# zhing2006/hala-renderer

Measured on AMD Instinct MI355X. Metric: Mrays/s, higher is better.
Workload: dtype f32

## Files before the change

### hala-renderer_amd/_abi.py

```python
import ctypes as C

INVALID_INDEX = 0xFFFFFFFF
MAX_CAMERA_COUNT = 8
MAX_LIGHT_COUNT = 32


class Vertex(C.Structure):
    _fields_ = [("position", C.c_float * 3), ("normal", C.c_float * 3),
                ("tangent", C.c_float * 3), ("tex_coord", C.c_float * 2)]


class GpuCamera(C.Structure):
    _fields_ = [("position", C.c_float * 3), ("_pad0", C.c_float),
                ("right", C.c_float * 3), ("_pad1", C.c_float),
                ("up", C.c_float * 3), ("_pad2", C.c_float),
                ("forward", C.c_float * 3), ("yfov", C.c_float),
                ("focal_distance_or_xmag", C.c_float), ("aperture_or_ymag", C.c_float),
                ("type", C.c_uint32), ("_pad3", C.c_uint32)]


class GpuLight(C.Structure):
    _fields_ = [("intensity", C.c_float * 3), ("_pad0", C.c_float),
                ("position", C.c_float * 3), ("_pad1", C.c_float),
                ("u", C.c_float * 3), ("_pad2", C.c_float),
# ... 51 lines not shown
class MeshDesc(C.Structure):
    _fields_ = [("primitives", C.POINTER(PrimitiveDesc)), ("primitive_count", C.c_uint32)]


class MaterialDesc(C.Structure):
    _fields_ = [("type", C.c_uint32), ("base_color", C.c_float * 3), ("opacity", C.c_float),
                ("emission", C.c_float * 3), ("anisotropic", C.c_float), ("metallic", C.c_float),
                ("roughness", C.c_float), ("subsurface", C.c_float), ("specular_tint", C.c_float),
                ("sheen", C.c_float), ("sheen_tint", C.c_float), ("clearcoat", C.c_float),
                ("clearcoat_roughness", C.c_float), ("clearcoat_tint", C.c_float * 3),
                ("specular_transmission", C.c_float), ("ior", C.c_float),
                ("medium_type", C.c_uint32), ("medium_color", C.c_float * 3),
                ("medium_density", C.c_float), ("medium_anisotropy", C.c_float),
                ("base_color_map_index", C.c_uint32), ("emission_map_index", C.c_uint32),
                ("normal_map_index", C.c_uint32), ("metallic_roughness_map_index", C.c_uint32)]


class LightDesc(C.Structure):
    _fields_ = [("color", C.c_float * 3), ("intensity", C.c_float), ("light_type", C.c_uint32),
                ("param0", C.c_float), ("param1", C.c_float)]


class CameraDesc(C.Structure):
    _fields_ = [("type", C.c_uint32), ("aspect", C.c_float), ("yfov", C.c_float), ("znear", C.c_float),
                ("zfar", C.c_float), ("focal_distance", C.c_float), ("aperture", C.c_float),
                ("xmag", C.c_float), ("ymag", C.c_float)]


class ImageDesc(C.Structure):
    _fields_ = [("format", C.c_uint32), ("width", C.c_uint32), ("height", C.c_uint32),
                ("data", C.c_void_p), ("num_of_bytes", C.c_size_t)]


class IndexPair(C.Structure):
    _fields_ = [("key", C.c_uint32), ("value", C.c_uint32)]


class SceneDesc(C.Structure):
    _fields_ = [("nodes", C.POINTER(NodeDesc)), ("node_count", C.c_uint32),
                ("meshes", C.POINTER(MeshDesc)), ("mesh_count", C.c_uint32),
                ("materials", C.POINTER(MaterialDesc)), ("material_count", C.c_uint32),
                ("lights", C.POINTER(LightDesc)), ("light_count", C.c_uint32),
                ("cameras", C.POINTER(CameraDesc)), ("camera_count", C.c_uint32),
                ("texture2image_mapping", C.POINTER(IndexPair)), ("texture_count", C.c_uint32),
                ("image2data_mapping", C.POINTER(IndexPair)), ("image_count", C.c_uint32),
                ("image_data", C.POINTER(ImageDesc)), ("image_data_count", C.c_uint32)]


class Ray(C.Structure):
    _fields_ = [("origin", C.c_float * 3), ("tmin", C.c_float), ("direction", C.c_float * 3), ("tmax", C.c_float)]


class Hit(C.Structure):
    _fields_ = [("t", C.c_float), ("u", C.c_float), ("v", C.c_float), ("prim", C.c_uint32)]


class RtInfo(C.Structure):
    _fields_ = [("width", C.c_uint32), ("height", C.c_uint32)]


class RtStatistics(C.Structure):
    _fields_ = [("total_frames", C.c_uint64), ("last_gpu_ms", C.c_double), ("rays_last_update", C.c_uint64),
                ("rays_total", C.c_uint64), ("traverse_ms_last_update", C.c_double),
                ("gpu_ms_total", C.c_double), ("traverse_closest_ms_total", C.c_double),
                ("traverse_shadow_ms_total", C.c_double), ("traverse_closest_launches", C.c_uint64),
                ("traverse_shadow_launches", C.c_uint64), ("updates_rendered", C.c_uint64),
                ("rays_closest_total", C.c_uint64), ("rays_shadow_total", C.c_uint64),
                ("nodes_closest_total", C.c_uint64), ("tris_closest_total", C.c_uint64),
                ("nodes_shadow_total", C.c_uint64), ("tris_shadow_total", C.c_uint64),
                ("rays_closest_counted", C.c_uint64), ("rays_shadow_counted", C.c_uint64),
                ("wave_steps_closest_total", C.c_uint64), ("leaf_passes_closest_total", C.c_uint64), ("leaf_lanes_closest_total", C.c_uint64),
                ("wave_steps_shadow_total", C.c_uint64), ("leaf_passes_shadow_total", C.c_uint64), ("leaf_lanes_shadow_total", C.c_uint64),
                ("traverse_primary_ms_total", C.c_double), ("traverse_primary_launches", C.c_uint64),
                ("nodes_primary_total", C.c_uint64), ("tris_primary_total", C.c_uint64), ("rays_primary_counted", C.c_uint64),
                ("rays_primary_total", C.c_uint64),
                ("rays_closest_timed", C.c_uint64), ("rays_primary_timed", C.c_uint64), ("rays_shadow_timed", C.c_uint64),
                ("shade_ms_total", C.c_double), ("shade_launches", C.c_uint64),
                ("traverse_fused_ms_total", C.c_double), ("traverse_fused_launches", C.c_uint64),
                ("rays_fused_closest_timed", C.c_uint64), ("rays_fused_shadow_timed", C.c_uint64)]


class BuildOptions(C.Structure):
    _fields_ = [("builder", C.c_uint32), ("ploc_tail", C.c_uint32), ("ploc_look_every", C.c_uint32),
                ("collapse_look_every", C.c_uint32), ("instancing", C.c_uint32), ("reserved", C.c_uint32 * 3)]


class BvhInfo(C.Structure):
    _fields_ = [("node_count", C.c_uint32), ("triangle_count", C.c_uint32), ("max_depth", C.c_uint32),
                ("lds_node_count", C.c_uint32), ("scene_min", C.c_float * 3), ("scene_max", C.c_float * 3),
                ("node_width", C.c_uint32), ("stored_triangle_count", C.c_uint32), ("instance_node_count", C.c_uint32),
                ("instance_ref_count", C.c_uint32), ("tree_bytes", C.c_uint64)]


class RtProgDescInfo(C.Structure):
    _fields_ = [("raygen_count", C.c_uint32), ("miss_count", C.c_uint32), ("hit_count", C.c_uint32),
                ("callable_count", C.c_uint32), ("push_constant_size", C.c_uint32),
                ("binding_count", C.c_uint32), ("ray_recursion_depth", C.c_uint32)]


class DenoiseParams(C.Structure):
    _fields_ = [("iterations", C.c_uint32), ("sigma_color", C.c_float), ("sigma_albedo", C.c_float),
                ("normal_power", C.c_uint32), ("demodulate", C.c_uint32), ("reserved", C.c_uint32 * 3)]


class AdaptiveParams(C.Structure):
    _fields_ = [("threshold", C.c_float), ("min_samples", C.c_uint32), ("interval", C.c_uint32), ("reserved", C.c_uint32 * 5)]


class AdaptiveStatus(C.Structure):
    _fields_ = [("enabled", C.c_uint32), ("active_blocks", C.c_uint32), ("total_blocks", C.c_uint32), ("active_pixels", C.c_uint32),
                ("samples", C.c_uint32), ("last_snapshot", C.c_uint32), ("reserved", C.c_uint32 * 2)]


class LightGroups(C.Structure):
    _fields_ = [("group_count", C.c_uint32), ("environment_group", C.c_uint32), ("light_count", C.c_uint32),
                ("material_count", C.c_uint32), ("light_group", C.POINTER(C.c_uint32)), ("material_group", C.POINTER(C.c_uint32))]


class CryptomatteDesc(C.Structure):
    _fields_ = [("layer_mask", C.c_uint32), ("material_name_count", C.c_uint32), ("material_names", C.POINTER(C.c_char_p)),
                ("reserved", C.c_uint32 * 2)]


class TemporalParams(C.Structure):
    _fields_ = [("max_history", C.c_float), ("tol", C.c_float), ("min_weight", C.c_float), ("reserved", C.c_uint32 * 5)]


PROTOTYPES = {
    "hala_denoise_default_params": ([C.POINTER(DenoiseParams)], None),
    "hala_rt_denoise": ([C.c_void_p, C.POINTER(DenoiseParams), C.POINTER(C.c_float)], C.c_int),
    "hala_rt_read_denoised": ([C.c_void_p, C.POINTER(C.c_float)], C.c_int),
    "hala_rt_get_denoised_buffer": ([C.c_void_p, C.POINTER(C.c_void_p), C.POINTER(C.c_size_t)], C.c_int),
    "hala_rt_save_denoised": ([C.c_void_p, C.c_char_p], C.c_int),
    "hala_denoise_images": ([C.c_int, C.POINTER(C.c_float), C.POINTER(C.c_float), C.POINTER(C.c_float), C.c_uint32, C.c_uint32,
                             C.POINTER(DenoiseParams), C.POINTER(C.c_float)], C.c_int),
    "hala_adaptive_default_params": ([C.POINTER(AdaptiveParams)], None),
    "hala_rt_set_adaptive_sampling": ([C.c_void_p, C.POINTER(AdaptiveParams)], C.c_int),
    "hala_rt_read_sample_counts": ([C.c_void_p, C.POINTER(C.c_uint32)], C.c_int),
    "hala_rt_get_adaptive_status": ([C.c_void_p, C.POINTER(AdaptiveStatus)], C.c_int),
    "hala_rt_set_views": ([C.c_void_p, C.POINTER(C.c_uint32), C.c_uint32], C.c_int),
    "hala_rt_read_view_image": ([C.c_void_p, C.c_uint32, C.c_int, C.POINTER(C.c_float)], C.c_int),
    "hala_rt_set_aovs": ([C.c_void_p, C.c_uint32], C.c_int),
    "hala_rt_set_light_groups": ([C.c_void_p, C.POINTER(LightGroups)], C.c_int),
    "hala_rt_read_light_group": ([C.c_void_p, C.c_uint32, C.c_uint32, C.POINTER(C.c_float)], C.c_int),
    "hala_rt_relight": ([C.c_void_p, C.c_uint32, C.POINTER(C.c_float), C.c_uint32], C.c_int),
    "hala_rt_read_relit": ([C.c_void_p, C.c_int, C.POINTER(C.c_float)], C.c_int),
    "hala_rt_get_relit_buffer": ([C.c_void_p, C.c_int, C.POINTER(C.c_void_p), C.POINTER(C.c_size_t)], C.c_int),
    "hala_rt_set_cryptomatte": ([C.c_void_p, C.POINTER(CryptomatteDesc)], C.c_int),
    "hala_rt_read_cryptomatte": ([C.c_void_p, C.c_uint32, C.c_uint32, C.POINTER(C.c_float)], C.c_int),
    "hala_rt_read_cryptomatte_records": ([C.c_void_p, C.c_uint32, C.c_uint32, C.POINTER(C.c_uint32)], C.c_int),
    "hala_rt_get_cryptomatte_manifest": ([C.c_void_p, C.c_uint32, C.c_char_p, C.c_size_t, C.POINTER(C.c_size_t)], C.c_int),
    "hala_rt_save_cryptomatte": ([C.c_void_p, C.c_uint32, C.c_char_p], C.c_int),
    "hala_cryptomatte_hash": ([C.c_char_p, C.POINTER(C.c_uint32), C.POINTER(C.c_uint32)], C.c_int),
    "hala_write_exr": ([C.c_char_p, C.c_uint32, C.c_uint32, C.c_uint32, C.POINTER(C.c_char_p), C.POINTER(C.POINTER(C.c_float)), C.c_uint32,
                        C.POINTER(C.c_char_p), C.POINTER(C.c_char_p)], C.c_int),
    "hala_temporal_default_params": ([C.POINTER(TemporalParams)], None),
    "hala_rt_set_temporal": ([C.c_void_p, C.POINTER(TemporalParams)], C.c_int),
    "hala_rt_temporal_capture": ([C.c_void_p], C.c_int),
    "hala_rt_temporal_resolve": ([C.c_void_p, C.POINTER(C.c_float)], C.c_int),
    "hala_rt_read_temporal": ([C.c_void_p, C.c_int, C.POINTER(C.c_float)], C.c_int),
    "hala_rt_get_temporal_buffer": ([C.c_void_p, C.c_int, C.POINTER(C.c_void_p), C.POINTER(C.c_size_t)], C.c_int),
    "hala_rt_denoise_temporal": ([C.c_void_p, C.POINTER(DenoiseParams), C.POINTER(C.c_float)], C.c_int),
}


import numpy as _np

RAY_DTYPE = _np.dtype([("origin", "<f4", 3), ("tmin", "<f4"), ("direction", "<f4", 3), ("tmax", "<f4")])
HIT_DTYPE = _np.dtype([("t", "<f4"), ("u", "<f4"), ("v", "<f4"), ("prim", "<u4")])
VERTEX_DTYPE = _np.dtype([("position", "<f4", 3), ("normal", "<f4", 3), ("tangent", "<f4", 3), ("tex_coord", "<f4", 2)])

EXPORTS = [
    "hala_last_error_message", "hala_rt_create", "hala_rt_destroy",
    "hala_rt_push_general_shader", "hala_rt_push_general_shader_with_file",
    "hala_rt_push_hit_shaders", "hala_rt_push_hit_shaders_with_file",
    "hala_rt_load_blue_noise_texture", "hala_rt_load_blue_noise_pixels", "hala_rt_set_scene", "hala_rt_set_envmap_pixels",
    "hala_rt_set_envmap_file", "hala_rt_set_ground_color", "hala_rt_set_sky_color",
    "hala_rt_set_env_intensity", "hala_rt_set_exposure_value", "hala_rt_commit", "hala_rt_set_build_options", "hala_rt_update", "hala_rt_update_batch",
    "hala_rt_render", "hala_rt_wait_idle", "hala_rt_save_images", "hala_rt_read_image",
    "hala_rt_get_info", "hala_rt_get_statistics", "hala_rt_set_counting", "hala_rt_set_launch_timing_period", "hala_rt_set_pass_fusion", "hala_rt_reset_accumulation", "hala_rt_get_global_uniform",
    "hala_rt_get_packed_cameras", "hala_rt_get_packed_lights", "hala_rt_get_packed_materials",
    "hala_rt_get_packed_primitives", "hala_rt_get_env_distribution", "hala_rt_get_texture_info",
    "hala_rt_read_texture_level", "hala_rt_sample_texture_host", "hala_rt_set_tile_shard",
    "hala_rt_tile_buffer", "hala_rt_get_stream", "hala_rt_scatter_gathered_tiles", "hala_rt_scatter_gathered_tiles_on_stream", "hala_rt_trace_rays",
    "hala_rt_trace_rays_host", "hala_rt_trace_rays_indirect", "hala_rt_get_bvh_info", "hala_rt_download_bvh", "hala_rt_download_instance_refs",
    "hala_rt_update_node_transform", "hala_rt_update_vertices", "hala_rt_update_material", "hala_rt_refit", "hala_envmap_build_distribution",
    "hala_tonemap_pixels", "hala_write_pfm", "hala_rtprog_parse_desc", "hala_version",
    "hala_scene_load_gltf", "hala_scene_get_desc", "hala_scene_free", "hala_load_float_image",
    "hala_rtprog_create", "hala_rtprog_destroy", "hala_rtprog_get_desc_info", "hala_rtprog_bind", "hala_rtprog_push_constants",
    "hala_rtprog_push_constants_f32", "hala_rtprog_trace_rays", "hala_rtprog_trace_rays_indirect",
    "hala_rt_comm_unique_id", "hala_rt_comm_init_rank", "hala_rt_comm_attach", "hala_rt_comm_destroy",
    "hala_rt_tile_allgather", "hala_rt_tile_allgather_begin", "hala_rt_tile_allgather_finish", "hala_rt_get_gathered_buffer",
    "hala_rt_tile_allgather_begin_external", "hala_rt_get_exchange_buffers",
    "hala_denoise_default_params", "hala_rt_denoise", "hala_rt_read_denoised", "hala_rt_get_denoised_buffer", "hala_rt_save_denoised",
    "hala_denoise_images",
    "hala_adaptive_default_params", "hala_rt_set_adaptive_sampling", "hala_rt_read_sample_counts", "hala_rt_get_adaptive_status",
    "hala_rt_set_views", "hala_rt_read_view_image", "hala_rt_set_aovs",
    "hala_rt_set_light_groups", "hala_rt_read_light_group", "hala_rt_relight", "hala_rt_read_relit", "hala_rt_get_relit_buffer",
    "hala_rt_set_cryptomatte", "hala_rt_read_cryptomatte", "hala_rt_read_cryptomatte_records", "hala_rt_get_cryptomatte_manifest",
    "hala_rt_save_cryptomatte", "hala_cryptomatte_hash", "hala_write_exr",
    "hala_temporal_default_params", "hala_rt_set_temporal", "hala_rt_temporal_capture", "hala_rt_temporal_resolve", "hala_rt_read_temporal",
    "hala_rt_get_temporal_buffer", "hala_rt_denoise_temporal",
]
```

### hala-renderer_amd/csrc/hala_types.h

```cpp
#pragma once
#include <hip/hip_vector_types.h>

#include <cstddef>
#include <cstdint>

#include "../../include/halart.h"

static_assert(sizeof(hala_vertex) == 44, "HalaVertex is 44 B (src/scene/vertex.rs:2-9)");
static_assert(sizeof(hala_gpu_camera) == 80, "gpu::HalaCamera is 80 B (src/scene/gpu/camera.rs:10-20)");
static_assert(offsetof(hala_gpu_camera, forward) == 48 && offsetof(hala_gpu_camera, yfov) == 60 && offsetof(hala_gpu_camera, type) == 72, "HalaCamera offsets");
static_assert(sizeof(hala_gpu_light) == 80, "gpu::HalaLight is 80 B (src/scene/gpu/light.rs:7-32)");
static_assert(offsetof(hala_gpu_light, v) == 48 && offsetof(hala_gpu_light, radius) == 60 && offsetof(hala_gpu_light, type) == 68, "HalaLight offsets");
static_assert(sizeof(hala_aabb) == 24, "HalaAABB is 24 B");
static_assert(sizeof(hala_gpu_material) == 144, "gpu::HalaMaterial is 144 B (src/scene/gpu/material.rs:6-48)");
static_assert(offsetof(hala_gpu_material, base_color) == 32 && offsetof(hala_gpu_material, ior) == 112 && offsetof(hala_gpu_material, type) == 140, "HalaMaterial offsets");
static_assert(sizeof(hala_gpu_mesh_data) == 96, "gpu::HalaMeshData is 96 B (src/scene/gpu/mesh.rs:32-39)");
static_assert(offsetof(hala_gpu_mesh_data, material_index) == 64 && offsetof(hala_gpu_mesh_data, vertices) == 72 && offsetof(hala_gpu_mesh_data, indices) == 80, "HalaMeshData offsets");
static_assert(sizeof(hala_global_uniform) == 112, "HalaGlobalUniform is 112 B (src/rt_renderer.rs:44-65)");
static_assert(offsetof(hala_global_uniform, resolution) == 32 && offsetof(hala_global_uniform, frame_index) == 48 && offsetof(hala_global_uniform, env_total_sum) == 68 && offsetof(hala_global_uniform, num_of_lights) == 96, "HalaGlobalUniform offsets");
static_assert(sizeof(hala_ray) == 32 && sizeof(hala_hit) == 16, "ray batch records");

namespace rt {

constexpr uint32_t kAbsent = 0xffffffffu;
constexpr float kTMax = 3.402823466e+38f;
constexpr float kNoNeePdf = 1e18f;

struct alignas(16) BvhNode4 {
  float pmin[3];
  uint32_t exps;
  uint32_t qlo[3];
  uint32_t qhi[3];
  uint32_t pad[2];
  uint32_t ref[4];
};
static_assert(sizeof(BvhNode4) == 64, "BVH4 node is 64 B");
constexpr uint32_t kLeafRef = 0x80000000u;
constexpr uint32_t kInstLeafTag = 0xF0000000u;
constexpr uint32_t kExitRef = 0xfffffffeu;
#if defined(__HIPCC__)
__host__ __device__
#endif
inline bool is_inst_leaf(uint32_t ref) { return (ref & kInstLeafTag) == kInstLeafTag && ref < kExitRef; }
struct alignas(64) InstRef {
  float r0[3], r1[3], r2[3], tr[3];
  uint32_t root;
  uint32_t gid_base;
  uint32_t shade_base;
  uint32_t inst;
};
static_assert(sizeof(InstRef) == 64, "instance reference is 64 B");
struct InstInfo {
  uint32_t first_tri;
  uint32_t shade_base;
  uint32_t instanced;
  uint32_t pad;
};

struct alignas(16) Tri {
  float v0[3]; uint32_t id;
  float e1[3]; uint32_t pad1;
  float e2[3]; uint32_t pad2;
};
static_assert(sizeof(Tri) == 48, "triangle is 48 B");

constexpr uint32_t kHitKindBits = 3;
#if defined(__HIPCC__)
__host__ __device__
#endif
inline uint32_t hit_encode(uint32_t id, uint32_t kind) { return (id << kHitKindBits) | (kind & 7u); }

struct alignas(128) ShadeTri {
  float gcross[3]; uint32_t inst;
  float n0[3];     uint32_t material;
  float n1[3];     uint32_t pad0;
  float n2[3];     uint32_t pad1;
  float uv[3][2];
  float tg[3][3];
  uint32_t pad2;
};
static_assert(sizeof(ShadeTri) == 128, "shading record is 128 B");

constexpr uint32_t kMaxMips = 16;
constexpr uint32_t kTexFloat = 0, kTexSrgb8 = 1, kTexUnorm8 = 2;
struct TexDesc {
  uint32_t width, height, mips, format;
  uint32_t mip_offset[kMaxMips];
};
#if defined(__HIPCC__)
__host__ __device__
#endif
inline uint32_t tex_tiled_index(uint32_t x, uint32_t y, uint32_t w) { return (((y >> 2) * ((w + 3u) >> 2) + (x >> 2)) << 4) + ((y & 3u) << 2) + (x & 3u); }
inline uint32_t tex_tiled_size(uint32_t w, uint32_t h) { return ((w + 3u) >> 2) * ((h + 3u) >> 2) * 16u; }
static_assert(sizeof(TexDesc) == 80, "texture descriptor is 80 B");

struct SceneView {
  const TexDesc* textures;
  const float4* tex_arena;
  const uint32_t* tex_arena8;
  const float* tex_lut;
  uint32_t texture_count;
  uint32_t shade_sort;
  const BvhNode4* nodes;
  const Tri* tris;
  const Tri* tris_any;
  const Tri* tris_by_id;
  const ShadeTri* shade_tris;
  const uint32_t* inst_first_tri;
  const hala_gpu_mesh_data* primitives;
  const hala_gpu_material* materials;
  const uint8_t* material_kind;
  const hala_gpu_light* lights;
  const hala_gpu_camera* cameras;
  const float* env_pixels;
  const float* env_marginal;
  const float* env_conditional;
  uint32_t node_count, tri_count, lds_nodes, lds_tris;
  const InstRef* inst_refs;
  const InstInfo* inst_info;
  uint32_t instance_count;
  uint32_t two_level;
  uint32_t any_translucent;
  uint32_t scatter_media;
  uint32_t simple_materials;
  float ray_eps;
  uint32_t staged;
};

constexpr uint32_t kShadeKindMiss = 0;
constexpr uint32_t kShadeKindFirst = 1;
constexpr uint32_t kShadeKindSpecial = 7;
constexpr uint32_t kShadeKinds = 9;
inline uint8_t shade_kind_of(const hala_gpu_material& m, uint32_t texture_count) {
  if (m.opacity < 1.0f || m.medium_type != 0u) return (uint8_t)kShadeKindSpecial;
  const bool tex = m.base_color_map_index < texture_count || m.normal_map_index < texture_count ||
                   m.metallic_roughness_map_index < texture_count || m.emission_map_index < texture_count;
  if (m.type == 1u && m.specular_transmission > 0.0f) return (uint8_t)(5u + (tex ? 1u : 0u));
  return (uint8_t)(kShadeKindFirst + (m.type == 1u ? 2u : 0u) + (tex ? 1u : 0u));
}

inline uint8_t any_class_of(const hala_gpu_material& m, bool base_map_has_alpha) {
  const bool medium = m.medium_type == 1u || m.medium_type == 2u;
  if (m.opacity == 0.0f) return medium ? 3 : 1;
  if (m.opacity < 1.0f || base_map_has_alpha) return medium ? 4 : 2;
  return 0;
}
constexpr uint32_t kAnyKeyLight = 0xA511E9B3u, kAnyKeyEnv = 0x63D83595u, kAnyKeyBatch = 0x5BD1E995u;

#ifndef RT_PIXEL_BLOCK
#define RT_PIXEL_BLOCK 8
#endif
constexpr uint32_t kPixelBlock = RT_PIXEL_BLOCK;
constexpr uint32_t kMaxViews = HALA_MAX_CAMERA_COUNT;
struct ViewConst {
  uint32_t camera;
  float tan_half, pixel_spread;
  uint32_t pad;
};
static_assert(sizeof(ViewConst) == 16, "view record is 16 B");
struct FrameConst {
  hala_global_uniform u;
  float aspect, tan_half;
  float pixel_spread;
  uint32_t width, height;
  uint32_t tile_size, tiles_x, tiles_y, world, rank, tiles_per_rank, perm_a, perm_b;
  uint32_t blocks_x;
  uint32_t pixel_slots;
  uint32_t samples;
  uint32_t slot_count;
  uint32_t views;
  uint32_t view_pixels;
  const ViewConst* view_table;
  const uint32_t* block_list;
};

constexpr uint32_t kMaxDepth = 64;
#ifndef RT_WORK_SHARDS
#define RT_WORK_SHARDS 16
#endif
constexpr uint32_t kWorkShards = RT_WORK_SHARDS;
constexpr uint32_t kWorkStride = 32;
constexpr uint32_t kWorkBatch = 128;
struct WorkCounters {
  uint32_t c[kWorkShards * kWorkStride];
// ... 60 lines not shown
```

### hala-renderer_amd/csrc/kernels.h

```cpp
#pragma once
#include <hip/hip_runtime.h>

#include <string>
#include <vector>

#include "hala_types.h"

namespace rt {

struct LaunchCfg {
  uint32_t persistent_blocks;
  uint2* spill;
  uint32_t refill;
  size_t smem;
};

enum class TreeForm { Large, Staged, TwoLevel };
inline TreeForm tree_form(const SceneView& sv) { return sv.staged ? TreeForm::Staged : (sv.two_level ? TreeForm::TwoLevel : TreeForm::Large); }

size_t traverse_fixed_lds_bytes(TreeForm tree);
uint32_t traverse_stack_lds_levels(TreeForm tree);
uint32_t traverse_max_leaf(TreeForm tree);
uint32_t traverse_stack_spill_levels();
uint32_t traverse_blocks_per_cu(size_t dynamic_lds_bytes, TreeForm tree);
void launch_trace_batch(const LaunchCfg& lc, const SceneView& sv, const hala_ray* rays, hala_hit* hits, const uint32_t* n_ptr,
                        uint32_t n_imm, WorkCounters* work, Control* ctl, bool any, bool count, bool account, hipStream_t s);
void launch_trace_shadow(const LaunchCfg& lc, const SceneView& sv, const Queues& q, const PathState& ps, Control* ctl, uint32_t depth,
                         uint32_t kind , bool count, hipStream_t s);
bool launch_trace_shadow_then_batch(const LaunchCfg& lc, const SceneView& sv, const Queues& q, const PathState& ps, Control* ctl, uint32_t depth,
                                    uint32_t kinds , bool with_closest, hipStream_t s);
void launch_trace_primary(const LaunchCfg& lc, const SceneView& sv, const FrameConst& fc, hala_hit* hits, WorkCounters* work, Control* ctl,
                          uint32_t n_account , bool count, hipStream_t s);
void launch_shade(const FrameConst& fc, const SceneView& sv, const Queues& q, const PathState& ps, Control* ctl, uint32_t depth, hipStream_t s);
void launch_resolve(const FrameConst& fc, const PathState& ps, float4* accum, float4* albedo, float4* normal, float4* final_img, float4* pos,
                    uint4* ids, float4* group_images, size_t group_stride, hipStream_t s);
struct RelightScales { float s[kMaxLightGroups][3]; };
void launch_relight(const hala_global_uniform& u, const float4* group_images, size_t group_stride, uint32_t group_count, const RelightScales& sc,
                    uint32_t n, float4* linear, float4* toned, hipStream_t s);
void launch_scatter_tiles(const FrameConst& fc, const float4* gathered, float4* full, hipStream_t s);
void launch_sample_texture(const SceneView& sv, uint32_t tex, const float* uvl, uint32_t n, float4* out, hipStream_t s);

void launch_mip_downsample(const float4* src, uint32_t sw, uint32_t sh, float4* dst, uint32_t dw, uint32_t dh, hipStream_t s);
void launch_tile8(const uint32_t* src, uint32_t w, uint32_t h, uint32_t* dst, hipStream_t s);
void launch_mip_downsample8(const uint32_t* src, uint32_t sw, uint32_t sh, uint32_t* dst, uint32_t dw, uint32_t dh, uint32_t format, const float* lut,
                            const float* thr, hipStream_t s);

struct BuildOptions {
  uint32_t builder = 0;
  uint32_t ploc_tail = 0;
  uint32_t ploc_look_every = 0;
  uint32_t collapse_look_every = 0;
};
struct BvhBuffers {
  const hala_gpu_mesh_data* primitives;
  const uint32_t* inst_first_tri;
  uint32_t instance_count;
  uint32_t tri_count;
  const uint32_t* gid_first = nullptr;
  const uint32_t* inst_index = nullptr;
  bool object_space = false;
  Tri* tris_by_id;
  Tri* tris;
  Tri* tris_any = nullptr;
  const uint8_t* material_any_class = nullptr;
  uint32_t material_count = 0;
  const uint8_t* material_kind = nullptr;
  ShadeTri* shade_tris;
  BvhNode4* nodes;
  void* topology = nullptr;
  BuildOptions opt;
  uint32_t node_count;
  uint32_t max_depth;
  uint32_t stack_need;
  float scene_min[3], scene_max[3];
};
std::string bvh_build(BvhBuffers& b, uint32_t leaf_max, hipStream_t s);
std::string bvh_refit(BvhBuffers& b, hipStream_t s);
std::string bvh_relocate(BvhBuffers& b, uint32_t node_offset, uint32_t tri_offset, hipStream_t s);
void bvh_free_topology(void* topology);

struct TlasItem { float mn[3], mx[3]; uint32_t ref, need; };
uint32_t tlas_build(const std::vector<TlasItem>& items, std::vector<BvhNode4>& out, uint32_t* levels, uint32_t* stack_need);

std::string envmap_build_distribution(const float4* d_rgba, uint32_t width, uint32_t height, float* d_total_sum, float* d_marginal,
                                      float* d_conditional, hipStream_t s);

}
```

### hala-renderer_amd/csrc/renderer.hip

```cpp
#include <hip/hip_runtime.h>

#include <algorithm>
#include <cmath>
#include <cstdio>
#include <cstring>
#include <map>
#include <memory>
#include <string>
#include <sys/stat.h>
#include <vector>

#include "adaptive.h"
#include "cryptomatte.h"
#include "denoise.h"
#include "dyn_api.h"
#include "hala_types.h"
#include "host_image.h"
#include "host_scene.h"
#include "host_util.h"
#include "kernels.h"
#include "temporal.h"

namespace rt { std::string decode_image_file_rgba8(const char* path, uint32_t* w, uint32_t* h, std::vector<uint8_t>* rgba); }

using namespace rt;

namespace {

constexpr uint32_t kLeafMax = 4;
constexpr uint32_t kLeafMaxStaged = 4;
constexpr size_t kLdsStageBudget = 40 * 1024;
constexpr uint32_t kRefillThreshold = 24;
constexpr int kStatRing = 16;
constexpr uint32_t kMaxSampleBatch = 16;

float h_sin_poly(float a) {
  float a2 = a * a;
  float p = -2.50521083854417187751e-8f;
  p = std::fmaf(p, a2, 2.75573192239858906526e-6f);
  p = std::fmaf(p, a2, -1.98412698412698412698e-4f);
  p = std::fmaf(p, a2, 8.33333333333333333333e-3f);
  p = std::fmaf(p, a2, -1.66666666666666666667e-1f);
  p = std::fmaf(p, a2, 1.0f);
  return a * p;
}
float h_cos_poly(float a) {
  float a2 = a * a;
  float p = 2.08767569878680989792e-9f;
  p = std::fmaf(p, a2, -2.75573192239858906526e-7f);
  p = std::fmaf(p, a2, 2.48015873015873015873e-5f);
  p = std::fmaf(p, a2, -1.38888888888888888889e-3f);
  p = std::fmaf(p, a2, 4.16666666666666666667e-2f);
  p = std::fmaf(p, a2, -0.5f);
  p = std::fmaf(p, a2, 1.0f);
  return p;
}
void h_sincos_rad(float a, float* s, float* c) {
  float t = a * 0.15915494309189533577f;
  t = t - std::floor(t);
  if (t >= 1.0f) t = 0.0f;
  float x = t * 4.0f;
  int q = (int)x;
  float f = x - (float)q;
  float ang = f * 1.57079632679489661923f;
  float sa = h_sin_poly(ang), ca = h_cos_poly(ang);
  switch (q & 3) {
    case 0: *s = sa; *c = ca; break;
    case 1: *s = ca; *c = -sa; break;
    case 2: *s = -sa; *c = -ca; break;
    default: *s = -ca; *c = sa; break;
  }
}

uint32_t gcd_u32(uint32_t a, uint32_t b) { while (b) { uint32_t t = a % b; a = b; b = t; } return a; }
uint32_t mod_inverse(uint32_t a, uint32_t n) {
  long long t = 0, nt = 1, r = n, nr = a % n;
  while (nr != 0) { long long q = r / nr; long long tmp = t - q * nt; t = nt; nt = tmp; tmp = r - q * nr; r = nr; nr = tmp; }
  if (t < 0) t += n;
  return (uint32_t)t;
}

struct TraceEvents {
  std::vector<hipEvent_t> ev;
  size_t used = 0;
  hipEvent_t frame_begin = nullptr, frame_end = nullptr;
  bool pending = false, counted = false;
  uint32_t samples = 1;
  uint32_t primary_pixels = 0;
  uint32_t shadow_launches = 0;
  unsigned long long fused_mask = 0, traced_mask = 0;
  QueueSizes* host_sizes = nullptr;
  Totals* host_totals = nullptr;
};

}

struct hala_rt_renderer {
  std::string name;
  uint32_t width = 0, height = 0;
  int device = 0;
  uint32_t max_depth = 0, rr_depth = 0;
  bool enable_tonemap = false, enable_aces = false, use_simple_aces = false;
  uint64_t max_frames = 0;
  hipStream_t stream = nullptr;
  uint32_t cu_count = 256;

  float ground[4] = {1.0f, 1.0f, 1.0f, 1.0f};
  float sky[4] = {0.5f, 0.7f, 1.0f, 1.0f};
  float env_intensity = 1.0f, exposure = 1.0f, env_rotation = 0.0f;

  uint32_t n_raygen = 0, n_miss = 0, n_callable = 0, n_hit = 0;
  DeviceArray<uint8_t> blue_noise;
  uint32_t blue_w = 0, blue_h = 0;

  bool has_scene = false, committed = false;
  HostScene hs;
  DeviceArray<hala_vertex> d_vertices;
  DeviceArray<uint32_t> d_indices;
  std::vector<size_t> prim_vertex_offset, prim_index_offset;
  DeviceArray<hala_gpu_camera> d_cameras;
  DeviceArray<hala_gpu_light> d_lights;
  DeviceArray<hala_gpu_material> d_materials;
  DeviceArray<uint8_t> d_material_kind;
  std::vector<uint8_t> material_kind;
  bool shade_sort = false, simple_materials = false, scatter_media = false;
  DeviceArray<hala_gpu_mesh_data> d_instances;
  DeviceArray<uint32_t> d_inst_first_tri;
  DeviceArray<float4> d_tex_arena;
  DeviceArray<uint32_t> d_tex_arena8;
  DeviceArray<float> d_srgb_lut, d_srgb_thr;
  DeviceArray<TexDesc> d_textures;
  std::vector<TexDesc> host_textures;

  BvhBuffers bvh{};
  struct Blas {
    BvhBuffers b{};
    uint32_t node_off = 0, tri_off = 0, node_cap = 0;
    bool object_space = false;
    uint32_t prim = 0;
    std::vector<uint32_t> insts;
    DeviceArray<hala_gpu_mesh_data> d_md;
    DeviceArray<uint32_t> d_first, d_gid, d_inst;
    ~Blas() { if (b.topology) bvh_free_topology(b.topology); }
  };
  std::vector<std::unique_ptr<Blas>> blas;
  bool two_level = false;
  uint32_t instancing_mode = 0;
  std::vector<uint8_t> inst_instanced;
  std::vector<int32_t> prim_blas;
  uint32_t tlas_capacity = 0, tlas_nodes = 0, stored_tris = 0;
  std::vector<InstRef> inst_refs;
  DeviceArray<InstRef> d_inst_refs;
  DeviceArray<InstInfo> d_inst_info;
  DeviceArray<Tri> d_tris_by_id, d_tris;
  DeviceArray<Tri> d_tris_any;
  DeviceArray<ShadeTri> d_shade_tris;
  DeviceArray<BvhNode4> d_nodes;
  uint32_t lds_nodes = 0, lds_tris = 0;
  bool staged = false;
  uint32_t leaf_max_built = 0;
  float ray_eps = 0.0f;
  DeviceArray<uint2> d_spill;
  LaunchCfg lcfg{};
  uint32_t fuse_mode = 1;

  bool has_env = false;
  uint32_t env_w = 0, env_h = 0;
  DeviceArray<float4> d_env;
  DeviceArray<float> d_env_total, d_marginal, d_conditional;
  float env_total_sum = 0.0f;

  uint32_t real_pixels = 0;
  uint32_t rank = 0, world = 1, tile_size = 32, tiles_x = 0, tiles_y = 0, tiles_per_rank = 0, perm_a_inv = 0, perm_b = 7;
  uint32_t slot_count = 0;
  uint32_t blocks_x = 0;
  size_t image_pixels() const { return world <= 1 ? (size_t)width * height : (size_t)slot_count; }
  uint32_t batch_capacity = 1;
  std::vector<uint32_t> views{0u};
  DeviceArray<ViewConst> d_views;
  std::vector<ViewConst> views_uploaded;
  uint32_t view_count() const { return (uint32_t)views.size(); }
  size_t image_alloc() const { return (size_t)slot_count + (size_t)(view_count() - 1) * image_pixels(); }

  DeviceArray<float4> img_local[6];
  DeviceArray<float4> img_full[6];
  bool full_valid[6] = {false, false, false, false, false, false};
  uint32_t aov_mask = 0;
  bool has_image(int which) const { return which >= 0 && (which < 4 || (which < 6 && ((aov_mask >> (which - 4)) & 1u))); }
  DeviceArray<float4> ps_aov_pos;
  DeviceArray<uint4> ps_aov_ids;
  DeviceArray<uint32_t> d_inst_node, d_light_node;
  uint32_t group_count = 0, env_group = 0;
  std::vector<uint32_t> light_group, material_group;
  DeviceArray<uint32_t> d_light_group, d_material_group;
  DeviceArray<P3> ps_groups;
  DeviceArray<float4> group_img;
  DeviceArray<float4> relit[2];
  bool relit_valid = false;
  uint32_t crypto_mask = 0;
  std::vector<std::string> crypto_material_names;
  DeviceArray<uint4> crypto_rec;
  std::vector<uint32_t> crypto_object, crypto_asset, crypto_material;
  DeviceArray<uint32_t> d_crypto_object, d_crypto_asset, d_crypto_material;
  bool crypto_tables = false;
  bool crypto_ready = false;
  size_t crypto_quads() const { return 4 * (size_t)__builtin_popcount(crypto_mask) * view_count() * slot_count; }
  bool wants_ids() const { return (aov_mask & 2u) || crypto_mask; }
  CryptoTables crypto_view() const {
    return CryptoTables{d_crypto_object.ptr, d_crypto_asset.ptr, d_crypto_material.ptr, (uint32_t)crypto_object.size(), (uint32_t)crypto_material.size(),
                        crypto_mask, slot_count};
  }
  DenoiseBuffers denoise;
  bool denoised = false;
  AdaptiveState adaptive;
  TemporalState temporal;
  DeviceArray<P3> ps_lr, ps_le, ps_alb, ps_nrm;
  DeviceArray<hala_ray> q_rays[2];
  DeviceArray<float4> q_state[2];
  DeviceArray<hala_hit> q_hits;
  DeviceArray<uint32_t> q_perm;
  DeviceArray<ShadowEntry> q_shadow[2];
  DeviceArray<Control> d_ctl;
  DeviceArray<WorkCounters> d_batch_work;

  uint64_t total_frames = 0;
  bool counting = false;
  hala_global_uniform last_uniform{};
  TraceEvents ring[kStatRing];
  int ring_pos = 0;
  bool vertices_dirty = false;
  bool materials_dirty_any = false;
  bool materials_dirty_any_refit = false;
  bool any_invisible = false;
  bool any_translucent = false;
  DeviceArray<uint8_t> d_material_any_class;
  std::vector<uint8_t> material_any_class;
  uint32_t launch_event_period = 0;
  unsigned long long update_counter = 0;
  hala_rt_statistics stats{};
  hipEvent_t scratch_event = nullptr;
  hipStream_t scratch_stream = nullptr;
  hipEvent_t batch_done = nullptr;
  ncclComm_t comm = nullptr;
  bool comm_owned = false;
  int comm_rank = 0, comm_world = 1;
  hipStream_t gather_stream = nullptr;
  DeviceArray<float4> gather_stage[6], gather_recv[6];
  hipEvent_t ev_rendered = nullptr, ev_staged = nullptr, ev_gathered = nullptr;
  uint32_t gather_pending = 0;
  int scratch_acquire(hipStream_t s) {
    if (scratch_event && scratch_stream != s) RT_HIP(hipStreamWaitEvent(s, scratch_event, 0));
    return HALA_OK;
  }
  hipStream_t tail_stream = nullptr;
  hipEvent_t ev_shaded = nullptr;
  hipEvent_t tail_done = nullptr;
  bool tail_open = false;
  uint32_t ctl_pos = 0;
  DeviceArray<uint2> d_spill_tail;
  int join_tail() {
    if (tail_open) RT_HIP(hipStreamWaitEvent(stream, tail_done, 0));
    tail_open = false;
    return HALA_OK;
  }

  ~hala_rt_renderer() {
    if (device >= 0) (void)hipSetDevice(device);
    if (stream) (void)hipStreamSynchronize(stream);
    if (tail_stream) (void)hipStreamSynchronize(tail_stream);
    for (auto& t : ring) {
      for (auto e : t.ev) (void)hipEventDestroy(e);
      if (t.frame_begin) (void)hipEventDestroy(t.frame_begin);
      if (t.frame_end) (void)hipEventDestroy(t.frame_end);
      if (t.host_totals) (void)hipHostFree(t.host_totals);
      if (t.host_sizes) (void)hipHostFree(t.host_sizes);
    }
    if (batch_done) (void)hipEventDestroy(batch_done);
    if (gather_stream) { (void)hipStreamSynchronize(gather_stream); (void)hipStreamDestroy(gather_stream); }
    for (hipEvent_t e : {ev_rendered, ev_staged, ev_gathered}) if (e) (void)hipEventDestroy(e);
    if (comm && comm_owned) { if (const RcclApi* api = rccl_api(nullptr)) (void)api->CommDestroy(comm); }
    for (auto& i : img_local) i.release();
    for (auto& i : img_full) i.release();
    if (bvh.topology) bvh_free_topology(bvh.topology);
    blas.clear();
    if (ev_shaded) (void)hipEventDestroy(ev_shaded);
    if (tail_stream) (void)hipStreamDestroy(tail_stream);
    if (stream) (void)hipStreamDestroy(stream);
  }

  SceneView view() const {
    SceneView sv{};
    sv.nodes = d_nodes.ptr; sv.tris = d_tris.ptr; sv.tris_any = any_invisible ? d_tris_any.ptr : d_tris.ptr; sv.tris_by_id = d_tris_by_id.ptr; sv.shade_tris = d_shade_tris.ptr;
    sv.inst_first_tri = d_inst_first_tri.ptr; sv.primitives = d_instances.ptr; sv.materials = d_materials.ptr; sv.material_kind = d_material_kind.ptr;
    sv.lights = d_lights.ptr; sv.cameras = d_cameras.ptr;
    sv.textures = d_textures.ptr; sv.tex_arena = d_tex_arena.ptr; sv.tex_arena8 = d_tex_arena8.ptr; sv.tex_lut = d_srgb_lut.ptr; sv.texture_count = (uint32_t)host_textures.size(); sv.shade_sort = shade_sort ? 1u : 0u; sv.simple_materials = simple_materials ? 1u : 0u; sv.scatter_media = scatter_media ? 1u : 0u; sv.any_translucent = any_translucent ? 1u : 0u;
    sv.env_pixels = reinterpret_cast<const float*>(d_env.ptr); sv.env_marginal = d_marginal.ptr; sv.env_conditional = d_conditional.ptr;
    sv.node_count = bvh.node_count; sv.tri_count = bvh.tri_count; sv.lds_nodes = lds_nodes; sv.lds_tris = lds_tris;
    sv.inst_refs = d_inst_refs.ptr; sv.inst_info = d_inst_info.ptr; sv.instance_count = (uint32_t)hs.instances.size(); sv.two_level = two_level ? 1u : 0u;
    sv.ray_eps = ray_eps;
    sv.staged = staged ? 1u : 0u;
    return sv;
  }
  Queues queues() const {
    Queues q{};
    q.rays[0] = q_rays[0].ptr; q.rays[1] = q_rays[1].ptr; q.state[0] = q_state[0].ptr; q.state[1] = q_state[1].ptr;
    q.hits = q_hits.ptr; q.perm = q_perm.ptr; q.shadow[0] = q_shadow[0].ptr; q.shadow[1] = q_shadow[1].ptr;
    return q;
  }
  PathState path_state() const {
    return PathState{ps_lr.ptr, ps_le.ptr, ps_alb.ptr, ps_nrm.ptr, (aov_mask & 1u) ? ps_aov_pos.ptr : nullptr, wants_ids() ? ps_aov_ids.ptr : nullptr,
                     d_inst_node.ptr, d_light_node.ptr,
                     group_count ? ps_groups.ptr : nullptr, group_count ? d_light_group.ptr : nullptr, group_count ? d_material_group.ptr : nullptr,
                     group_count, group_count ? (uint32_t)((size_t)slot_count * batch_capacity) : 0u, env_group};
  }

  ViewConst view_const(uint32_t cam, float height) const {
    ViewConst v{};
    float sn = 0.0f, cs = 1.0f;
    if (cam < hs.cameras.size()) h_sincos_rad(0.5f * hs.cameras[cam].yfov, &sn, &cs);
    v.camera = cam;
    v.tan_half = sn / cs;
    v.pixel_spread = 2.0f * v.tan_half / height;
    return v;
  }
  FrameConst frame_const(const hala_global_uniform& u, uint32_t samples = 1) const {
    FrameConst fc{};
    fc.u = u;
    fc.aspect = u.resolution[0] / u.resolution[1];
    const ViewConst v0 = view_const(views[0], u.resolution[1]);
    fc.tan_half = v0.tan_half;
    fc.pixel_spread = v0.pixel_spread;
    fc.views = view_count();
    fc.view_pixels = (uint32_t)image_pixels();
    fc.view_table = fc.views > 1u ? d_views.ptr : nullptr;
    fc.width = width; fc.height = height;
    fc.tile_size = tile_size; fc.tiles_x = tiles_x; fc.tiles_y = tiles_y; fc.world = world; fc.rank = rank; fc.blocks_x = blocks_x;
    fc.tiles_per_rank = tiles_per_rank; fc.perm_a = perm_a_inv; fc.perm_b = perm_b;
    fc.pixel_slots = slot_count; fc.samples = samples; fc.slot_count = slot_count * samples * fc.views;
    if (adaptive.enabled) {
      fc.block_list = adaptive.lists[adaptive.cur].ptr;
      fc.pixel_slots = adaptive.active_blocks * kPixelBlock * kPixelBlock;
      fc.slot_count = fc.pixel_slots * samples;
    }
    return fc;
  }

  void reset_accumulation() {
    total_frames = 0;
    for (bool& v : full_valid) v = false;
    adaptive.restart(width * height);
    crypto_ready = false;
  }
  uint32_t rendered_frames() const { return (uint32_t)std::min(total_frames, max_frames); }

  void resolve_slot(TraceEvents& t) {
    if (!t.pending) return;
    (void)hipEventSynchronize(t.frame_end);
    float ms = 0.0f;
    if (hipEventElapsedTime(&ms, t.frame_begin, t.frame_end) == hipSuccess) { stats.last_gpu_ms = ms; stats.gpu_ms_total += ms; }
    double tr[3] = {0.0, 0.0, 0.0}, sh = 0.0;
    unsigned long long rays[3] = {0, 0, 0}, launches[3] = {0, 0, 0};
    const QueueSizes* qs = t.host_sizes;
    for (size_t k = 0, depth = 0; k + 3 < t.used; k += 4, ++depth) {
      float m = 0.0f;
      const bool own_closest = depth == 0 || !((t.traced_mask >> depth) & 1ull);
      if (own_closest && hipEventElapsedTime(&m, t.ev[k], t.ev[k + 1]) == hipSuccess) {
        const unsigned long long n = depth == 0 ? (unsigned long long)t.primary_pixels * t.samples : qs->n_active[depth];
        tr[0] += m; rays[0] += n; launches[0] += 1;
        if (depth == 0) { stats.traverse_primary_ms_total += m; stats.traverse_primary_launches += 1; stats.rays_primary_timed += n; }
      }
      if (hipEventElapsedTime(&m, t.ev[k + 1], t.ev[k + 2]) == hipSuccess) sh += m;
      if (hipEventElapsedTime(&m, t.ev[k + 2], t.ev[k + 3]) == hipSuccess) {
        const unsigned long long ns = (unsigned long long)qs->n_shadow[0][depth] + qs->n_shadow[1][depth];
        if ((t.fused_mask >> depth) & 1ull) {
          tr[2] += m; launches[2] += 1;
          stats.rays_fused_shadow_timed += ns;
          if ((t.traced_mask >> (depth + 1)) & 1ull) stats.rays_fused_closest_timed += qs->n_active[depth + 1];
        } else { tr[1] += m; rays[1] += ns; }
// ... 192 lines not shown
    hs.instances[i].indices = reinterpret_cast<uint64_t>(r->d_indices.ptr + r->prim_index_offset[p]);
  }
  RT_HIP(r->d_cameras.upload(hs.cameras.data(), hs.cameras.size(), r->stream));
  RT_HIP(r->d_lights.upload(hs.lights.data(), hs.lights.size(), r->stream));
  RT_HIP(r->d_materials.upload(hs.gpu_materials.data(), hs.gpu_materials.size(), r->stream));
  {
    std::vector<uint8_t> kind(hs.gpu_materials.size());
    for (size_t i = 0; i < kind.size(); ++i) kind[i] = shade_kind_of(hs.gpu_materials[i], (uint32_t)hs.texture_image.size());
    RT_HIP(r->d_material_kind.upload(kind.data(), kind.size(), r->stream));
    r->material_kind = kind;
    uint32_t seen = 0;
    for (uint8_t k : kind) seen |= 1u << k;
    r->shade_sort = (seen & (seen - 1u)) != 0u;
    r->scatter_media = false;
    for (const auto& m : hs.gpu_materials) r->scatter_media = r->scatter_media || m.medium_type == 2u;
    r->simple_materials = seen == (1u << kShadeKindFirst);
  }
  RT_HIP(r->d_instances.upload(hs.instances.data(), hs.instances.size(), r->stream));
  RT_HIP(r->d_inst_first_tri.upload(hs.inst_first_tri.data(), hs.inst_first_tri.size(), r->stream));
  RT_HIP(r->d_inst_node.upload(hs.instance_node.data(), hs.instance_node.size(), r->stream));
  RT_HIP(r->d_light_node.upload(hs.light_node.data(), hs.light_node.size(), r->stream));
  RT_HIP(hipStreamSynchronize(r->stream));
  return HALA_OK;
}

int upload_textures(hala_rt_renderer* r) {
  const HostScene& hs = r->hs;
  std::vector<TexDesc> img_desc(hs.images.size());
  size_t total_f = 0, total_8 = 0, largest_8 = 0;
  for (size_t k = 0; k < hs.images.size(); ++k) {
    TexDesc& td = img_desc[k];
    memset(&td, 0, sizeof(td));
    td.width = hs.images[k].width; td.height = hs.images[k].height; td.format = hs.images[k].format;
    uint32_t m = std::max(td.width, td.height), p2 = 1, lg = 0;
    while (p2 < m) { p2 <<= 1; ++lg; }
    td.mips = std::min<uint32_t>(lg + 1, kMaxMips);
    size_t& total = td.format == kTexFloat ? total_f : total_8;
    for (uint32_t l = 0; l < td.mips; ++l) {
      if (total > 0xffffffffull) RT_FAIL("The texture arena exceeds 2^32 texels.");
      td.mip_offset[l] = (uint32_t)total;
      const uint32_t lw = std::max(1u, td.width >> l), lh = std::max(1u, td.height >> l);
      total += td.format == kTexFloat ? (size_t)lw * lh : (size_t)tex_tiled_size(lw, lh);
    }
    if (td.format != kTexFloat) largest_8 = std::max(largest_8, (size_t)td.width * td.height);
  }
  RT_HIP(r->d_tex_arena.resize(total_f));
  RT_HIP(r->d_tex_arena8.resize(total_8));
  if (total_8) RT_HIP(hipMemsetAsync(r->d_tex_arena8.ptr, 0, total_8 * 4, r->stream));
  const float* lut = srgb_decode_lut();
  float thr[256];
  for (int k = 0; k < 255; ++k) thr[k] = (lut[k] + lut[k + 1]) * 0.5f;
  thr[255] = 3.402823466e+38f;
  float lut512[512];
  for (int k = 0; k < 256; ++k) { lut512[k] = lut[k]; lut512[256 + k] = (float)k / 255.0f; }
  RT_HIP(r->d_srgb_lut.upload(lut512, 512, r->stream));
  RT_HIP(r->d_srgb_thr.upload(thr, 256, r->stream));
  DeviceArray<uint32_t> staging;
  RT_HIP(staging.resize(largest_8));
  for (size_t k = 0; k < hs.images.size(); ++k) {
    const TexDesc& td = img_desc[k];
    if (td.format == kTexFloat) {
      RT_HIP(hipMemcpyAsync(r->d_tex_arena.ptr + td.mip_offset[0], hs.images[k].rgba.data(), (size_t)td.width * td.height * 16, hipMemcpyHostToDevice, r->stream));
      for (uint32_t l = 1; l < td.mips; ++l)
        launch_mip_downsample(r->d_tex_arena.ptr + td.mip_offset[l - 1], std::max(1u, td.width >> (l - 1)), std::max(1u, td.height >> (l - 1)),
                              r->d_tex_arena.ptr + td.mip_offset[l], std::max(1u, td.width >> l), std::max(1u, td.height >> l), r->stream);
    } else {
      RT_HIP(hipMemcpyAsync(staging.ptr, hs.images[k].rgba8.data(), (size_t)td.width * td.height * 4, hipMemcpyHostToDevice, r->stream));
      launch_tile8(staging.ptr, td.width, td.height, r->d_tex_arena8.ptr + td.mip_offset[0], r->stream);
      for (uint32_t l = 1; l < td.mips; ++l)
        launch_mip_downsample8(r->d_tex_arena8.ptr + td.mip_offset[l - 1], std::max(1u, td.width >> (l - 1)), std::max(1u, td.height >> (l - 1)),
                               r->d_tex_arena8.ptr + td.mip_offset[l], std::max(1u, td.width >> l), std::max(1u, td.height >> l), td.format,
                               r->d_srgb_lut.ptr, r->d_srgb_thr.ptr, r->stream);
    }
  }
  std::vector<TexDesc> tex(hs.texture_image.size());
  for (size_t i = 0; i < tex.size(); ++i) tex[i] = img_desc[hs.texture_image[i]];
  RT_HIP(r->d_textures.upload(tex.data(), tex.size(), r->stream));
  RT_HIP(hipStreamSynchronize(r->stream));
  RT_HIP(hipGetLastError());
  r->host_textures = tex;
  return HALA_OK;
}

int configure_traversal(hala_rt_renderer* r) {
  const size_t nb = (size_t)r->bvh.node_count * 64, tb = (size_t)r->bvh.tri_count * 48;
  r->staged = !r->two_level && nb + tb <= kLdsStageBudget;
  r->lds_nodes = r->staged ? r->bvh.node_count : 0u;
  r->lds_tris = r->staged ? r->bvh.tri_count : 0u;
  const TreeForm tree = tree_form(r->view());
  if (r->leaf_max_built > traverse_max_leaf(tree)) RT_FAIL("The BVH was built with larger leaves than the traversal variant for its size accepts.");
  const size_t smem = (size_t)r->lds_nodes * 64 + (size_t)r->lds_tris * 48 + traverse_fixed_lds_bytes(tree);
  const uint32_t per_cu = traverse_blocks_per_cu(smem, tree);
  if (per_cu == 0) RT_FAIL("The traversal kernel does not fit on a compute unit with the requested LDS staging.");
  r->lcfg.persistent_blocks = r->cu_count * std::min(per_cu, 8u);
  r->lcfg.smem = smem;
  r->lcfg.spill = nullptr;
  r->lcfg.refill = r->staged ? 64u : kRefillThreshold;
  if (r->two_level || r->bvh.stack_need > traverse_stack_lds_levels(tree)) {
    if (r->two_level || r->bvh.stack_need > traverse_stack_lds_levels(tree) + traverse_stack_spill_levels()) {
      std::vector<BvhNode4> nodes(r->bvh.node_count);
      RT_HIP(hipMemcpy(nodes.data(), r->d_nodes.ptr, nodes.size() * sizeof(BvhNode4), hipMemcpyDeviceToHost));
      std::vector<uint32_t> need(nodes.size(), 0u);
      for (size_t i = nodes.size(); i-- > 0;) {
        uint32_t inner = 0, deepest = 0;
        for (uint32_t ref : nodes[i].ref) {
          if (ref == kAbsent) continue;
          if (is_inst_leaf(ref)) {
            const uint32_t k = ref & 0x0fffffffu;
            ++inner;
            if (k < r->inst_refs.size() && r->inst_refs[k].root < need.size()) deepest = std::max(deepest, 4u + need[r->inst_refs[k].root]);
            continue;
          }
          if (ref & kLeafRef) continue;
          ++inner;
          if (ref < need.size()) deepest = std::max(deepest, need[ref]);
        }
        need[i] = inner ? inner - 1u + deepest : 0u;
      }
      r->bvh.stack_need = need.empty() ? 1u : std::max(1u, need[0]);
    }
    if (r->bvh.stack_need > traverse_stack_lds_levels(tree) + traverse_stack_spill_levels())
      RT_FAIL("The BVH is deeper than the traversal stack supports (" + std::to_string(r->bvh.max_depth) + " levels, " + std::to_string(r->bvh.stack_need) + " stack entries).");
    RT_HIP(r->d_spill.resize((size_t)r->lcfg.persistent_blocks * 256 * traverse_stack_spill_levels()));
    RT_HIP(r->d_spill_tail.resize(r->d_spill.count));
    r->lcfg.spill = r->d_spill.ptr;
  }
  const float ex = r->bvh.scene_max[0] - r->bvh.scene_min[0], ey = r->bvh.scene_max[1] - r->bvh.scene_min[1], ez = r->bvh.scene_max[2] - r->bvh.scene_min[2];
  r->ray_eps = std::sqrt(std::fmaf(ez, ez, std::fmaf(ey, ey, ex * ex))) * 1e-5f;
  return HALA_OK;
}

int attach_any_triangles(hala_rt_renderer* r) {
  const HostScene& hs = r->hs;
  std::vector<uint8_t> cls(hs.gpu_materials.size());
  r->any_invisible = false; r->any_translucent = false;
  for (size_t i = 0; i < cls.size(); ++i) {
    const hala_gpu_material& m = hs.gpu_materials[i];
    const bool cutout = m.base_color_map_index < hs.texture_image.size() && hs.images[hs.texture_image[m.base_color_map_index]].has_alpha;
    cls[i] = any_class_of(m, cutout);
    r->any_invisible = r->any_invisible || cls[i] != 0;
    r->any_translucent = r->any_translucent || cls[i] >= 2;
  }
  r->material_any_class = cls;
  RT_HIP(r->d_material_any_class.upload(cls.data(), cls.size(), r->stream));
  if (r->any_invisible) RT_HIP(r->d_tris_any.resize(r->two_level ? r->stored_tris : r->hs.triangle_count));
  r->bvh.tris_any = r->any_invisible ? r->d_tris_any.ptr : nullptr;
  r->bvh.material_any_class = r->d_material_any_class.ptr;
  r->bvh.material_kind = r->d_material_kind.ptr;
  r->bvh.material_count = (uint32_t)r->hs.gpu_materials.size();
  return HALA_OK;
}

static float h_dot3(const float* a, const float* b) { return std::fmaf(a[2], b[2], std::fmaf(a[1], b[1], a[0] * b[0])); }
static void h_cross3(const float* a, const float* b, float* o) {
  o[0] = std::fmaf(a[1], b[2], -(a[2] * b[1])); o[1] = std::fmaf(a[2], b[0], -(a[0] * b[2])); o[2] = std::fmaf(a[0], b[1], -(a[1] * b[0]));
}
static bool world_to_object(const float* m, InstRef* o) {
  const float c0[3] = {m[0], m[1], m[2]}, c1[3] = {m[4], m[5], m[6]}, c2[3] = {m[8], m[9], m[10]};
  float k0[3], k1[3], k2[3];
  h_cross3(c1, c2, k0); h_cross3(c2, c0, k1); h_cross3(c0, c1, k2);
  const float det = h_dot3(c0, k0);
  if (!(det != 0.0f) || !std::isfinite(det)) return false;
  const float inv = 1.0f / det;
  for (int k = 0; k < 3; ++k) { o->r0[k] = k0[k] * inv; o->r1[k] = k1[k] * inv; o->r2[k] = k2[k] * inv; o->tr[k] = m[12 + k]; }
  for (int k = 0; k < 3; ++k)
    if (!std::isfinite(o->r0[k]) || !std::isfinite(o->r1[k]) || !std::isfinite(o->r2[k]) || !std::isfinite(o->tr[k])) return false;
// ... 304 lines not shown
  return HALA_OK;
}

int hala_rt_load_blue_noise_pixels(hala_rt_renderer* r, const uint8_t* rgba8, uint32_t width, uint32_t height);
int hala_rt_load_blue_noise_texture(hala_rt_renderer* r, const char* path) {
  if (!r) RT_FAIL("The renderer handle is null!");
  if (!path || !*path || file_stem(path).empty()) RT_FAIL("The file name is none!");
  uint32_t w = 0, h = 0;
  std::vector<uint8_t> px;
  std::string e;
  try { e = rt::decode_image_file_rgba8(path, &w, &h, &px); }
  catch (const std::exception& ex) { e = std::string("Failed to open image \"") + path + "\": " + ex.what(); }
  if (!e.empty()) RT_FAIL(e);
  return hala_rt_load_blue_noise_pixels(r, px.data(), w, h);
}
int hala_rt_load_blue_noise_pixels(hala_rt_renderer* r, const uint8_t* rgba8, uint32_t width, uint32_t height) {
  if (ensure_device(r) != HALA_OK) return HALA_ERR;
  if (!rgba8 || !width || !height) RT_FAIL("The blue noise texture is empty!");
  RT_HIP(r->blue_noise.upload(rgba8, (size_t)width * height * 4, r->stream));
  RT_HIP(hipStreamSynchronize(r->stream));
  r->blue_w = width; r->blue_h = height;
  return HALA_OK;
}

int hala_rt_set_scene(hala_rt_renderer* r, const hala_scene_desc* scene) {
  RtRange range("halart::set_scene");
  if (ensure_device(r) != HALA_OK) return HALA_ERR;
  RT_HIP(hipStreamSynchronize(r->stream));
  r->has_scene = false; r->committed = false;
  r->temporal.drop_history();
  const std::string e = r->hs.assign(scene);
  if (!e.empty()) RT_FAIL(e);
  if (upload_packed(r) != HALA_OK) return HALA_ERR;
  if (upload_textures(r) != HALA_OK) return HALA_ERR;
  r->has_scene = true;
  return HALA_OK;
}

int hala_rt_set_envmap_pixels(hala_rt_renderer* r, const float* pixels, uint32_t channels, uint32_t width, uint32_t height, float rotation_degrees) {
  if (ensure_device(r) != HALA_OK) return HALA_ERR;
  RT_HIP(hipStreamSynchronize(r->stream));
  return install_envmap(r, pixels, channels, width, height, rotation_degrees, nullptr, nullptr, nullptr);
}

int hala_rt_set_envmap_file(hala_rt_renderer* r, const char* path, float rotation_degrees) {
  if (ensure_device(r) != HALA_OK) return HALA_ERR;
  if (!path || !*path) RT_FAIL("The file name is none!");
  HostImage img;
  const std::string e = load_float_image(path, &img);
  if (!e.empty()) RT_FAIL(e);
  RT_HIP(hipStreamSynchronize(r->stream));
  const std::string cache = "./out/" + file_stem(path) + ".dist_cache";
  const size_t W = img.width, H = img.height;
  std::vector<float> blob(1 + H + W * H);
  FILE* f = fopen(cache.c_str(), "rb");
  if (f) {
    const size_t got = fread(blob.data(), 4, blob.size(), f);
    fclose(f);
    if (got != blob.size()) RT_FAIL("Failed to read from file.");
    return install_envmap(r, img.pixels.data(), img.channels, img.width, img.height, rotation_degrees, &blob[0], &blob[1], &blob[1 + H]);
  }
  if (install_envmap(r, img.pixels.data(), img.channels, img.width, img.height, rotation_degrees, nullptr, nullptr, nullptr) != HALA_OK) return HALA_ERR;
  blob[0] = r->env_total_sum;
  RT_HIP(hipMemcpy(&blob[1], r->d_marginal.ptr, H * 4, hipMemcpyDeviceToHost));
  RT_HIP(hipMemcpy(&blob[1 + H], r->d_conditional.ptr, W * H * 4, hipMemcpyDeviceToHost));
  f = fopen(cache.c_str(), "wb");
  if (!f) RT_FAIL("Failed to create file \"" + cache + "\".");
  const size_t put = fwrite(blob.data(), 4, blob.size(), f);
  if (fclose(f) != 0 || put != blob.size()) RT_FAIL("Failed to write to file.");
  return HALA_OK;
}

void hala_rt_set_ground_color(hala_rt_renderer* r, const float rgba[4]) { if (r && rgba) memcpy(r->ground, rgba, 16); }
void hala_rt_set_sky_color(hala_rt_renderer* r, const float rgba[4]) { if (r && rgba) memcpy(r->sky, rgba, 16); }
void hala_rt_set_env_intensity(hala_rt_renderer* r, float v) { if (r) r->env_intensity = v; }
void hala_rt_set_exposure_value(hala_rt_renderer* r, float v) { if (r) r->exposure = v; }

int hala_rt_commit(hala_rt_renderer* r) {
  RtRange range("halart::commit");
  if (ensure_device(r) != HALA_OK) return HALA_ERR;
  if (!r->has_scene) RT_FAIL("The scene in GPU is none!");
  if (r->hs.cameras.empty()) RT_FAIL("The scene has no camera.");
  if (r->hs.instances.empty()) RT_FAIL("The scene has no mesh primitive.");
  if (build_bvh(r) != HALA_OK) return HALA_ERR;
  r->committed = true;
  r->crypto_tables = false;
  r->temporal.drop_history();
  r->reset_accumulation();
  return HALA_OK;
}

int hala_rt_set_build_options(hala_rt_renderer* r, const hala_rt_build_options* o) {
  if (!r) RT_FAIL("The renderer handle is null!");
  if (!o) RT_FAIL("The build options are null!");
  if (o->builder > 3u || o->ploc_tail > 2u || o->instancing > 2u) RT_FAIL("Invalid build options.");
  for (uint32_t v : o->reserved) if (v != 0u) RT_FAIL("Invalid build options (reserved fields must be 0).");
  r->instancing_mode = o->instancing;
  r->bvh.opt.builder = o->builder; r->bvh.opt.ploc_tail = o->ploc_tail;
  r->bvh.opt.ploc_look_every = o->ploc_look_every; r->bvh.opt.collapse_look_every = o->collapse_look_every;
  return HALA_OK;
}

static int update_impl(hala_rt_renderer* r, uint32_t frames) {
  RtRange range("halart::update");
  if (ensure_device(r, false) != HALA_OK) return HALA_ERR;
  if (!r->committed) RT_FAIL("The pipeline is none!");
  const uint32_t V = r->view_count();
  for (uint32_t v = 0; v < V; ++v)
    if (r->views[v] >= r->hs.cameras.size())
      RT_FAIL("hala_rt_update: view " + std::to_string(v) + " renders camera " + std::to_string(r->views[v]) + ", but the committed scene has " +
              std::to_string(r->hs.cameras.size()) + " camera(s) (hala_rt_set_views).");
  if (r->group_count && (r->hs.lights.size() > r->light_group.size() || r->hs.gpu_materials.size() > r->material_group.size()))
    RT_FAIL("hala_rt_update: the light groups cover " + std::to_string(r->light_group.size()) + " light(s) and " + std::to_string(r->material_group.size()) +
            " material(s), but the committed scene has " + std::to_string(r->hs.lights.size()) + " and " + std::to_string(r->hs.gpu_materials.size()) +
            " (hala_rt_set_light_groups).");
  const uint64_t first = r->total_frames;
  r->total_frames += frames;
  if (first >= r->max_frames) return HALA_OK;
  const uint32_t samples = (uint32_t)std::min<uint64_t>(frames, r->max_frames - first);
  if (samples * V > r->batch_capacity) {
    if (r->join_tail() != HALA_OK) return HALA_ERR;
    RT_HIP(hipStreamSynchronize(r->stream));
    if (alloc_wavefront(r, samples * V) != HALA_OK) return HALA_ERR;
  }
  if (r->crypto_mask && crypto_prepare(r) != HALA_OK) return HALA_ERR;
  if (V > 1u) {
    std::vector<ViewConst> table(V);
    for (uint32_t v = 0; v < V; ++v) table[v] = r->view_const(r->views[v], (float)r->height);
    if (table.size() != r->views_uploaded.size() || memcmp(table.data(), r->views_uploaded.data(), V * sizeof(ViewConst)) != 0) {
      if (r->join_tail() != HALA_OK) return HALA_ERR;
      RT_HIP(hipStreamSynchronize(r->stream));
      RT_HIP(r->d_views.upload(table.data(), V, r->stream));
      RT_HIP(hipStreamSynchronize(r->stream));
      r->views_uploaded = table;
    }
  }
  hala_global_uniform u{};
  memcpy(u.ground_color, r->ground, 16); memcpy(u.sky_color, r->sky, 16);
  u.resolution[0] = (float)r->width; u.resolution[1] = (float)r->height;
  u.max_depth = r->max_depth; u.rr_depth = r->rr_depth;
  u.frame_index = (uint32_t)first;
  u.camera_index = r->views[0];
  u.env_type = r->has_env ? 1u : 0u;
  u.env_map_width = r->has_env ? r->env_w : 0; u.env_map_height = r->has_env ? r->env_h : 0;
  u.env_total_sum = r->has_env ? r->env_total_sum : 0.0f;
  u.env_rotation = r->env_rotation / 360.0f;
  u.env_intensity = r->env_intensity; u.exposure_value = r->exposure;
  u.enable_tonemap = r->enable_tonemap; u.enable_aces = r->enable_aces; u.use_simple_aces = r->use_simple_aces;
  u.num_of_lights = (uint32_t)r->hs.lights.size();
  r->last_uniform = u;
  r->last_uniform.frame_index = (uint32_t)(first + samples - 1);
  AdaptiveState& ad = r->adaptive;
  if (ad.enabled && first == 0 && (r->join_tail() != HALA_OK || adaptive_begin(ad, r->stream) != hipSuccess)) RT_FAIL("hala_rt_update: the adaptive sampling state could not be reset.");
  if (ad.enabled && ad.active_blocks == 0) {
    for (int k = 0; k < kStatRing; ++k) r->resolve_slot(r->ring[(r->ring_pos + k) % kStatRing]);
    r->stats.rays_last_update = 0;
    return HALA_OK;
  }
  const uint32_t primary_pixels = (ad.enabled ? ad.active_pixels : r->real_pixels) * V;

  TraceEvents& te = r->ring[r->ring_pos];
  r->ring_pos = (r->ring_pos + 1) % kStatRing;
  r->resolve_slot(te);
  if (!te.frame_begin) { RT_HIP(hipEventCreate(&te.frame_begin)); RT_HIP(hipEventCreate(&te.frame_end)); RT_HIP(hipHostMalloc(reinterpret_cast<void**>(&te.host_totals), sizeof(Totals), hipHostMallocDefault)); }
  te.used = 0; te.counted = r->counting; te.shadow_launches = 0; te.fused_mask = 0; te.traced_mask = 0;

  te.samples = samples;
  te.primary_pixels = primary_pixels;
  const FrameConst fc = r->frame_const(u, samples);
  const SceneView sv = r->view();
  const Queues q = r->queues();
  const PathState ps = r->path_state();
  Control* ctl = r->d_ctl.ptr + r->ctl_pos;
  r->ctl_pos ^= 1u;
  const hipStream_t s = r->stream;
  const bool timed = r->launch_event_period == 1u || (r->launch_event_period > 1u && (r->update_counter % r->launch_event_period) == 0u);
  r->update_counter++;
  const bool split_tail = !timed && !r->counting;
  if (!split_tail && r->join_tail() != HALA_OK) return HALA_ERR;
  if (!r->tail_open && r->scratch_acquire(s) != HALA_OK) return HALA_ERR;
// ... 737 lines not shown
  if (e == hipSuccess && gpu_ms) e = hipEventRecord(ev[1], r->stream);
  if (e == hipSuccess && gpu_ms) e = hipEventSynchronize(ev[1]);
  if (e == hipSuccess && gpu_ms) e = hipEventElapsedTime(gpu_ms, ev[0], ev[1]);
  for (hipEvent_t x : ev) if (x) (void)hipEventDestroy(x);
  if (e != hipSuccess) RT_FAIL(std::string("hala_rt_denoise_temporal: ") + hipGetErrorString(e));
  r->denoised = true;
  return HALA_OK;
}

int hala_rt_set_launch_timing_period(hala_rt_renderer* r, uint32_t period) {
  if (!r) RT_FAIL("The renderer handle is null!");
  r->launch_event_period = period;
  r->update_counter = 0;
  return HALA_OK;
}
int hala_rt_set_pass_fusion(hala_rt_renderer* r, uint32_t mode) {
  if (!r) RT_FAIL("The renderer handle is null!");
  if (mode > 2u) RT_FAIL("Invalid pass fusion mode.");
  r->fuse_mode = mode;
  return HALA_OK;
}
int hala_rt_set_counting(hala_rt_renderer* r, int enable) {
  if (!r) RT_FAIL("The renderer handle is null!");
  r->counting = enable != 0;
  return HALA_OK;
}
int hala_rt_get_global_uniform(hala_rt_renderer* r, hala_global_uniform* out) {
  if (!r || !out) RT_FAIL("The renderer handle is null!");
  *out = r->last_uniform;
  return HALA_OK;
}

#define RT_READBACK(dev, T, dst, cap, cnt)                                                               \
  do {                                                                                                     \
    *(cnt) = (uint32_t)(dev).count;                                                                        \
    const size_t _n = std::min<size_t>((cap), (dev).count);                                                \
    if ((dst) && _n) RT_HIP(hipMemcpy((dst), (dev).ptr, _n * sizeof(T), hipMemcpyDeviceToHost));           \
  } while (0)

int hala_rt_get_packed_cameras(hala_rt_renderer* r, hala_gpu_camera* dst, uint32_t capacity, uint32_t* count) {
  if (ensure_device(r) != HALA_OK) return HALA_ERR;
  if (!r->has_scene || !count) RT_FAIL("The scene in GPU is none!");
  RT_READBACK(r->d_cameras, hala_gpu_camera, dst, capacity, count);
  return HALA_OK;
}
int hala_rt_get_packed_lights(hala_rt_renderer* r, hala_gpu_light* dst, hala_aabb* bb, uint32_t capacity, uint32_t* count) {
  if (ensure_device(r) != HALA_OK) return HALA_ERR;
  if (!r->has_scene || !count) RT_FAIL("The scene in GPU is none!");
  RT_READBACK(r->d_lights, hala_gpu_light, dst, capacity, count);
  if (bb) memcpy(bb, r->hs.light_aabbs.data(), std::min<size_t>(capacity, r->hs.light_aabbs.size()) * sizeof(hala_aabb));
  return HALA_OK;
}
int hala_rt_get_packed_materials(hala_rt_renderer* r, hala_gpu_material* dst, uint32_t capacity, uint32_t* count) {
  if (ensure_device(r) != HALA_OK) return HALA_ERR;
  if (!r->has_scene || !count) RT_FAIL("The scene in GPU is none!");
  RT_READBACK(r->d_materials, hala_gpu_material, dst, capacity, count);
  return HALA_OK;
}
int hala_rt_get_packed_primitives(hala_rt_renderer* r, hala_gpu_mesh_data* dst, float* t3x4, uint32_t capacity, uint32_t* count) {
  if (ensure_device(r) != HALA_OK) return HALA_ERR;
  if (!r->has_scene || !count) RT_FAIL("The scene in GPU is none!");
  RT_READBACK(r->d_instances, hala_gpu_mesh_data, dst, capacity, count);
  if (t3x4) memcpy(t3x4, r->hs.instance_3x4.data(), std::min<size_t>(capacity, r->hs.instances.size()) * 12 * sizeof(float));
  return HALA_OK;
}
int hala_rt_get_env_distribution(hala_rt_renderer* r, float* total_sum, float* marginal, float* conditional) {
  if (ensure_device(r) != HALA_OK) return HALA_ERR;
  if (!r->has_env) RT_FAIL("The environment map is none!");
  if (total_sum) *total_sum = r->env_total_sum;
  if (marginal) RT_HIP(hipMemcpy(marginal, r->d_marginal.ptr, (size_t)r->env_h * 4, hipMemcpyDeviceToHost));
  if (conditional) RT_HIP(hipMemcpy(conditional, r->d_conditional.ptr, (size_t)r->env_w * r->env_h * 4, hipMemcpyDeviceToHost));
  return HALA_OK;
}

int hala_rt_get_texture_info(hala_rt_renderer* r, uint32_t texture, uint32_t* width, uint32_t* height, uint32_t* mips) {
  if (!r) RT_FAIL("The renderer handle is null!");
  if (!r->has_scene || texture >= r->host_textures.size()) RT_FAIL("The texture does not exist.");
  const TexDesc& td = r->host_textures[texture];
  if (width) *width = td.width;
  if (height) *height = td.height;
  if (mips) *mips = td.mips;
  return HALA_OK;
}
int hala_rt_read_texture_level(hala_rt_renderer* r, uint32_t texture, uint32_t level, float* dst_rgba32f) {
  if (ensure_device(r) != HALA_OK) return HALA_ERR;
  if (!r->has_scene || texture >= r->host_textures.size() || !dst_rgba32f) RT_FAIL("The texture does not exist.");
  const TexDesc& td = r->host_textures[texture];
  if (level >= td.mips) RT_FAIL("The mip level does not exist.");
  const uint32_t lw = std::max(1u, td.width >> level), lh = std::max(1u, td.height >> level);
  const size_t n = (size_t)lw * lh;
  if (td.format == kTexFloat) {
    RT_HIP(hipMemcpy(dst_rgba32f, r->d_tex_arena.ptr + td.mip_offset[level], n * 16, hipMemcpyDeviceToHost));
    return HALA_OK;
  }
  std::vector<uint32_t> tiled(tex_tiled_size(lw, lh));
  RT_HIP(hipMemcpy(tiled.data(), r->d_tex_arena8.ptr + td.mip_offset[level], tiled.size() * 4, hipMemcpyDeviceToHost));
  const float* lut = srgb_decode_lut();
  for (uint32_t y = 0; y < lh; ++y)
    for (uint32_t x = 0; x < lw; ++x) {
      const uint32_t t = tiled[tex_tiled_index(x, y, lw)];
      float* o = dst_rgba32f + ((size_t)y * lw + x) * 4;
      for (int c = 0; c < 3; ++c) { const uint32_t b = (t >> (8 * c)) & 0xffu; o[c] = td.format == kTexSrgb8 ? lut[b] : (float)b / 255.0f; }
      o[3] = (float)(t >> 24) / 255.0f;
    }
  return HALA_OK;
}
int hala_rt_sample_texture_host(hala_rt_renderer* r, uint32_t texture, const float* uv_lod, uint32_t count, float* dst_rgba32f) {
  if (ensure_device(r) != HALA_OK) return HALA_ERR;
  if (!r->has_scene || texture >= r->host_textures.size()) RT_FAIL("The texture does not exist.");
  if (!count) return HALA_OK;
  if (!uv_lod || !dst_rgba32f) RT_FAIL("Invalid argument.");
  DeviceArray<float> d_in;
  DeviceArray<float4> d_out;
  RT_HIP(d_in.upload(uv_lod, (size_t)count * 3, r->stream));
  RT_HIP(d_out.resize(count));
  launch_sample_texture(r->view(), texture, d_in.ptr, count, d_out.ptr, r->stream);
  RT_HIP(hipMemcpyAsync(dst_rgba32f, d_out.ptr, (size_t)count * 16, hipMemcpyDeviceToHost, r->stream));
  RT_HIP(hipStreamSynchronize(r->stream));
  RT_HIP(hipGetLastError());
  return HALA_OK;
}

int hala_rt_tile_allgather_finish(hala_rt_renderer* r);
int hala_rt_set_tile_shard(hala_rt_renderer* r, uint32_t rank, uint32_t world, uint32_t tile_size) {
  if (ensure_device(r) != HALA_OK) return HALA_ERR;
  if (world == 0 || rank >= world) RT_FAIL("Invalid rank / world size.");
  if (tile_size == 0 || tile_size > 256) RT_FAIL("Invalid tile size.");
  if (world > 1 && r->adaptive.enabled) RT_FAIL("Adaptive sampling is on: a sharded frame cannot use it (hala_rt_set_adaptive_sampling(r, NULL) first).");
  if (world > 1 && r->view_count() > 1u) RT_FAIL("The renderer has several views: a sharded frame renders one (hala_rt_set_views with one camera first).");
  if (world > 1 && r->group_count) RT_FAIL("Light groups are on: a sharded frame cannot use them (hala_rt_set_light_groups(r, NULL) first).");
  if (world > 1 && r->crypto_mask) RT_FAIL("Cryptomatte is on: a sharded frame cannot use it (hala_rt_set_cryptomatte(r, NULL) first).");
  if (world > 1 && r->temporal.enabled) RT_FAIL("Temporal reprojection is on: a sharded frame cannot use it (hala_rt_set_temporal(r, NULL) first).");
  if (r->gather_pending && hala_rt_tile_allgather_finish(r) != HALA_OK) return HALA_ERR;
  if (r->comm && ((uint32_t)r->comm_rank != rank || (uint32_t)r->comm_world != world))
    RT_FAIL("The renderer holds a communicator for rank " + std::to_string(r->comm_rank) + " of " + std::to_string(r->comm_world) +
            ": call hala_rt_comm_destroy before changing the tile shard.");
  RT_HIP(hipStreamSynchronize(r->stream));
  if (r->gather_stream) RT_HIP(hipStreamSynchronize(r->gather_stream));
  r->rank = rank; r->world = world; r->tile_size = tile_size;
  r->temporal.drop_history();
  compute_tiling(r);
  if (alloc_frame_buffers(r) != HALA_OK) return HALA_ERR;
  RT_HIP(hipStreamSynchronize(r->stream));
  r->reset_accumulation();
  return HALA_OK;
}
int hala_rt_tile_buffer(hala_rt_renderer* r, int which, void** d_ptr, size_t* bytes) {
  if (!r || !r->has_image(which) || !d_ptr || !bytes) RT_FAIL("Invalid argument.");
  *d_ptr = r->img_local[which].ptr;
  *bytes = r->image_pixels() * sizeof(float4);
  return HALA_OK;
}
int hala_rt_get_stream(hala_rt_renderer* r, void** hip_stream) {
  if (!hip_stream) RT_FAIL("Invalid argument.");
  if (ensure_device(r) != HALA_OK) return HALA_ERR;
  *hip_stream = static_cast<void*>(r->stream);
  return HALA_OK;
}
int hala_rt_scatter_gathered_tiles_on_stream(hala_rt_renderer* r, int which, const void* d_gathered, size_t bytes, void* hip_stream) {
  if (ensure_device(r) != HALA_OK) return HALA_ERR;
  if (!r->has_image(which) || !d_gathered) RT_FAIL("Invalid argument.");
  if (r->world <= 1) RT_FAIL("The renderer is not sharded.");
  if (bytes != r->image_pixels() * r->world * sizeof(float4)) RT_FAIL("The gathered buffer has the wrong size.");
  RT_HIP(r->img_full[which].resize((size_t)r->width * r->height));
  hala_global_uniform u = r->last_uniform;
  const FrameConst fc = r->frame_const(u);
// ... 199 lines not shown
  RT_HIP(hipStreamSynchronize(r->stream));
  return HALA_OK;
}

int hala_rt_get_bvh_info(hala_rt_renderer* r, hala_bvh_info* out) {
  if (!r || !out) RT_FAIL("The renderer handle is null!");
  if (!r->committed) RT_FAIL("The top level acceleration structure is none!");
  out->node_count = r->bvh.node_count; out->triangle_count = r->hs.triangle_count; out->max_depth = r->bvh.max_depth; out->lds_node_count = r->lds_nodes;
  out->node_width = 4u;
  out->stored_triangle_count = r->stored_tris; out->instance_node_count = r->two_level ? r->tlas_nodes : 0u;
  out->instance_ref_count = r->two_level ? (uint32_t)r->inst_refs.size() : 0u;
  out->tree_bytes = (uint64_t)r->d_nodes.bytes() + r->d_tris.bytes() + r->d_tris_any.bytes() + r->d_shade_tris.bytes() + r->d_inst_refs.bytes() + r->d_inst_info.bytes();
  memcpy(out->scene_min, r->bvh.scene_min, 12); memcpy(out->scene_max, r->bvh.scene_max, 12);
  return HALA_OK;
}
int hala_rt_download_bvh(hala_rt_renderer* r, void* nodes_64B, void* triangles_48B) {
  if (ensure_device(r) != HALA_OK) return HALA_ERR;
  if (!r->committed) RT_FAIL("The top level acceleration structure is none!");
  RT_HIP(hipStreamSynchronize(r->stream));
  if (nodes_64B) RT_HIP(hipMemcpy(nodes_64B, r->d_nodes.ptr, (size_t)r->bvh.node_count * 64, hipMemcpyDeviceToHost));
  if (triangles_48B && r->bvh.tri_count) {
    RT_HIP(hipMemcpy(triangles_48B, r->d_tris.ptr, (size_t)r->bvh.tri_count * 48, hipMemcpyDeviceToHost));
    Tri* t = static_cast<Tri*>(triangles_48B);
    for (uint32_t i = 0; i < r->bvh.tri_count; ++i) t[i].pad2 = 0u;
  }
  return HALA_OK;
}

int hala_rt_download_instance_refs(hala_rt_renderer* r, void* refs_64B, uint32_t capacity, uint32_t* count) {
  if (!r || !count) RT_FAIL("Invalid argument.");
  if (!r->committed) RT_FAIL("The top level acceleration structure is none!");
  *count = r->two_level ? (uint32_t)r->inst_refs.size() : 0u;
  if (refs_64B && r->two_level) memcpy(refs_64B, r->inst_refs.data(), std::min<size_t>(capacity, r->inst_refs.size()) * sizeof(InstRef));
  return HALA_OK;
}
int hala_rt_update_node_transform(hala_rt_renderer* r, uint32_t node_index, const float local_transform[16]) {
  if (!r || !local_transform) RT_FAIL("Invalid argument.");
  if (!r->committed) RT_FAIL("The top level acceleration structure is none!");
  if (node_index >= r->hs.nodes.size()) RT_FAIL("The node does not exist.");
  memcpy(r->hs.nodes[node_index].local.m, local_transform, 64);
  return HALA_OK;
}
int hala_rt_update_vertices(hala_rt_renderer* r, uint32_t mesh_index, uint32_t primitive_index, const hala_vertex* vertices, uint32_t vertex_count) {
  if (!r || !vertices) RT_FAIL("Invalid argument.");
  if (ensure_device(r) != HALA_OK) return HALA_ERR;
  if (!r->committed) RT_FAIL("The top level acceleration structure is none!");
  if (mesh_index + 1u >= r->hs.mesh_first_prim.size()) RT_FAIL("The mesh does not exist.");
  const uint32_t first = r->hs.mesh_first_prim[mesh_index], end = r->hs.mesh_first_prim[mesh_index + 1u];
  if (primitive_index >= end - first) RT_FAIL("The primitive does not exist.");
  HostPrimitive& p = r->hs.prims[first + primitive_index];
  if (vertex_count != p.vertices.size()) RT_FAIL("The vertex count differs from the primitive's (" + std::to_string(p.vertices.size()) + "): refit keeps the topology, use set_scene + commit.");
  for (uint32_t k = 0; k < vertex_count; ++k)
    if (!std::isfinite(vertices[k].position[0]) || !std::isfinite(vertices[k].position[1]) || !std::isfinite(vertices[k].position[2])) RT_FAIL("Vertex position is not finite.");
  memcpy(p.vertices.data(), vertices, (size_t)vertex_count * sizeof(hala_vertex));
  RT_HIP(hipStreamSynchronize(r->stream));
  r->vertices_dirty = true;
  if (r->temporal.enabled)
    for (size_t i = 0; i < r->hs.instance_prim.size() && i < r->temporal.inst_marked.size(); ++i)
      if (r->hs.instance_prim[i] == first + primitive_index) { r->temporal.inst_marked[i] = 1; r->temporal.table_dirty = true; }
  if (vertex_count) RT_HIP(hipMemcpyAsync(r->d_vertices.ptr + r->prim_vertex_offset[first + primitive_index], p.vertices.data(), (size_t)vertex_count * sizeof(hala_vertex), hipMemcpyHostToDevice, r->stream));
  return HALA_OK;
}
int hala_rt_update_material(hala_rt_renderer* r, uint32_t material_index, const hala_material_desc* material) {
  if (!r || !material) RT_FAIL("Invalid argument.");
  if (!r->committed) RT_FAIL("The top level acceleration structure is none!");
  if (material_index >= r->hs.materials.size()) RT_FAIL("The material does not exist.");
  if (material->type > 1u) RT_FAIL("Invalid material type.");
  if (r->hs.materials[material_index].opacity == 0.0f || material->opacity == 0.0f) r->materials_dirty_any = true;
  r->hs.materials[material_index] = *material;
  if (r->temporal.enabled && material_index < r->temporal.mat_marked.size()) { r->temporal.mat_marked[material_index] = 1; r->temporal.table_dirty = true; }
  return HALA_OK;
}
int hala_rt_refit(hala_rt_renderer* r) {
  RtRange range("halart::refit");
  if (ensure_device(r) != HALA_OK) return HALA_ERR;
  if (!r->committed) RT_FAIL("The top level acceleration structure is none!");
  RT_HIP(hipStreamSynchronize(r->stream));
  const std::vector<hala_gpu_mesh_data> before = r->hs.instances;
  const std::vector<uint8_t> kinds_before = r->material_kind;
  r->hs.update_node_hierarchies();
  const std::string e = r->hs.pack();
  if (!e.empty()) RT_FAIL(e);
  if (upload_packed(r, false) != HALA_OK) return HALA_ERR;
  r->bvh.primitives = r->d_instances.ptr; r->bvh.inst_first_tri = r->d_inst_first_tri.ptr;
  const bool had_invisible = r->any_invisible;
  const std::vector<uint8_t> classes_before = r->material_any_class;
  if (attach_any_triangles(r) != HALA_OK) return HALA_ERR;
  if (classes_before != r->material_any_class) r->materials_dirty_any = true;
  bool geometry_moved = r->vertices_dirty || r->materials_dirty_any || had_invisible != r->any_invisible || before.size() != r->hs.instances.size() ||
                        kinds_before != r->material_kind;
  r->materials_dirty_any_refit = r->materials_dirty_any;
  r->materials_dirty_any = false;
  for (size_t i = 0; i < before.size() && !geometry_moved; ++i) geometry_moved = memcmp(before[i].transform, r->hs.instances[i].transform, 64) != 0;
  std::vector<uint8_t> flags;
  classify_instances(r, &flags);
  if (flags != r->inst_instanced) {
    if (build_bvh(r) != HALA_OK) return HALA_ERR;
    r->vertices_dirty = false;
  } else if (r->two_level) {
    const bool content = r->vertices_dirty || r->materials_dirty_any_refit || had_invisible != r->any_invisible || kinds_before != r->material_kind;
    r->bvh.tris_any = r->any_invisible ? r->d_tris_any.ptr : nullptr;
    for (auto& bl : r->blas) {
      bool moved = content;
      if (!bl->object_space)
        for (uint32_t i : bl->insts) moved = moved || memcmp(before[i].transform, r->hs.instances[i].transform, 64) != 0;
      if (moved && blas_build_or_refit(r, *bl, true) != HALA_OK) return HALA_ERR;
    }
    if (build_instance_levels(r) != HALA_OK) return HALA_ERR;
    if (configure_traversal(r) != HALA_OK) return HALA_ERR;
    r->vertices_dirty = false;
  } else if (geometry_moved) {
    const std::string e2 = bvh_refit(r->bvh, r->stream);
    if (!e2.empty()) RT_FAIL(e2);
    if (configure_traversal(r) != HALA_OK) return HALA_ERR;
    r->vertices_dirty = false;
  }
  r->crypto_tables = false;
  r->temporal.table_dirty = true;
  r->reset_accumulation();
  return HALA_OK;
}

int hala_envmap_build_distribution(int device_ordinal, const float* rgba32f, uint32_t width, uint32_t height, float* total_sum, float* marginal, float* conditional) {
  if (!rgba32f || !total_sum || !marginal || !conditional || !width || !height) RT_FAIL("Invalid argument.");
  int count = 0;
  if (hipGetDeviceCount(&count) != hipSuccess || count <= 0) RT_FAIL("No HIP device is available: libhalart has no CPU path.");
  RT_HIP(hipSetDevice(device_ordinal));
  DeviceArray<float4> d_px;
  DeviceArray<float> d_total, d_m, d_c;
  const size_t n = (size_t)width * height;
  RT_HIP(d_px.upload(reinterpret_cast<const float4*>(rgba32f), n, nullptr));
  RT_HIP(d_total.resize(1)); RT_HIP(d_m.resize(height)); RT_HIP(d_c.resize(n));
  const std::string e = envmap_build_distribution(d_px.ptr, width, height, d_total.ptr, d_m.ptr, d_c.ptr, nullptr);
  if (!e.empty()) RT_FAIL(e);
  RT_HIP(hipMemcpy(total_sum, d_total.ptr, 4, hipMemcpyDeviceToHost));
  RT_HIP(hipMemcpy(marginal, d_m.ptr, (size_t)height * 4, hipMemcpyDeviceToHost));
  RT_HIP(hipMemcpy(conditional, d_c.ptr, n * 4, hipMemcpyDeviceToHost));
  return HALA_OK;
}

void hala_tonemap_pixels(float* rgba32f, size_t pixel_count, int enable_tonemap, int enable_aces, int use_simple_aces) {
  if (rgba32f) tonemap_pixels(rgba32f, pixel_count, enable_tonemap, enable_aces, use_simple_aces);
}
int hala_cryptomatte_hash(const char* name, uint32_t* raw, uint32_t* id) {
  if (!name) RT_FAIL("The name is null!");
  const uint32_t h = murmur3_32(name, strlen(name), 0u);
  if (raw) *raw = h;
  if (id) *id = crypto_id(h);
  return HALA_OK;
}
int hala_write_exr(const char* path, uint32_t width, uint32_t height, uint32_t channel_count, const char* const* channel_names,
                   const float* const* planes, uint32_t attribute_count, const char* const* attr_names, const char* const* attr_values) {
  const std::string e = write_exr(path, width, height, channel_count, channel_names, planes, attribute_count, attr_names, attr_values);
  if (!e.empty()) RT_FAIL(e);
  return HALA_OK;
}
int hala_write_pfm(const char* path, const float* rgba32f, uint32_t width, uint32_t height) {
  if (!path || !rgba32f) RT_FAIL("Invalid argument.");
  const std::string e = write_pfm(path, rgba32f, width, height);
  if (!e.empty()) RT_FAIL(e);
  return HALA_OK;
}

int hala_load_float_image(const char* path, uint32_t* width, uint32_t* height, uint32_t* channels, float* dst, size_t capacity_floats) {
  if (!path || !width || !height || !channels) RT_FAIL("Invalid argument.");
  HostImage img;
// ... 118 lines not shown
```

### hala-renderer_amd/csrc/shading.h

```cpp
#pragma once
#include <hip/hip_runtime.h>

#include "hala_types.h"
#include "rt_math.h"

namespace rt {

RT_DI bool slot_to_pixel(const FrameConst& fc, uint32_t slot, uint32_t* px, uint32_t* py) {
  if (fc.world <= 1u) {
    if (kPixelBlock == 0u) {
      *py = slot / fc.width;
      *px = slot - *py * fc.width;
      return true;
    }
    constexpr uint32_t kB = kPixelBlock ? kPixelBlock : 1u, kB2 = kB * kB;
    uint32_t blk = slot / kB2;
    const uint32_t within = slot - blk * kB2;
    if (fc.block_list) blk = fc.block_list[blk];
    const uint32_t ly = within / kB, lx = within - ly * kB;
    const uint32_t by = blk / fc.blocks_x, bx = blk - by * fc.blocks_x;
    *px = bx * kB + lx;
    *py = by * kB + ly;
    return *px < fc.width && *py < fc.height;
  }
// ... 359 lines not shown
    }
    s.dist = kTMax;
    s.le = inten;
    s.valid = true;
  } else if (l.type == 3u) {
    f3 u = ld3(l.u), v = ld3(l.v);
    f3 pt = madd3(v, r2, madd3(u, r1, pos));
    f3 n = normalize3(cross3(u, v));
    f3 to = pt - P;
    float d2 = dot3(to, to);
    if (!(d2 > 0.0f)) return s;
    float dist = sqrtf(d2);
    s.wi = to * (1.0f / dist);
    float cosl = -dot3(s.wi, n);
    if (!(cosl > 0.0f)) return s;
    s.dist = dist; s.le = inten; s.pdf = d2 / (l.area * cosl); s.delta = false; s.valid = true;
  } else if (l.type == 4u) {
    float z = 1.0f - 2.0f * r1;
    float rr = sqrtf(maxf(0.0f, 1.0f - z * z));
    float sp, cp;
    sincos_2pi(r2, &sp, &cp);
    f3 nl = mk3(rr * cp, rr * sp, z);
    f3 pt = madd3(nl, l.radius, pos);
    f3 to = pt - P;
    float d2 = dot3(to, to);
    if (!(d2 > 0.0f)) return s;
    float dist = sqrtf(d2);
    s.wi = to * (1.0f / dist);
    float cosl = -dot3(s.wi, nl);
    if (!(cosl > 0.0f)) return s;
    s.dist = dist; s.le = inten; s.pdf = d2 / (l.area * cosl); s.delta = false; s.valid = true;
  }
  return s;
}
RT_DI float intersect_light(const hala_gpu_light& l, f3 o, f3 d, float* pdf) {
  f3 pos = ld3(l.position);
  if (l.type == 3u) {
    f3 u = ld3(l.u), v = ld3(l.v);
    f3 n = normalize3(cross3(u, v));
    float dn = dot3(d, n);
    if (!(dn < 0.0f)) return -1.0f;
    float t = dot3(pos - o, n) / dn;
    if (!(t > 0.0f)) return -1.0f;
    f3 hp = madd3(d, t, o) - pos;
    float a = dot3(hp, u) / dot3(u, u), b = dot3(hp, v) / dot3(v, v);
    if (!(a >= 0.0f && a <= 1.0f && b >= 0.0f && b <= 1.0f)) return -1.0f;
    *pdf = (t * t) / (l.area * (-dn));
    return t;
  }
  if (l.type == 4u) {
    f3 oc = o - pos;
    float b = dot3(oc, d);
    float c = dot3(oc, oc) - l.radius * l.radius;
    float disc = b * b - c;
    if (!(disc > 0.0f)) return -1.0f;
    float t = -b - sqrtf(disc);
    if (!(t > 0.0f)) return -1.0f;
    f3 nl = (madd3(d, t, o) - pos) * (1.0f / l.radius);
    float cosl = -dot3(d, nl);
    if (!(cosl > 0.0f)) return -1.0f;
    *pdf = (t * t) / (l.area * cosl);
    return t;
  }
  return -1.0f;
}

RT_DI f3 transform_normal(const float* m, f3 n) {
  f3 c0 = mk3(m[0], m[1], m[2]), c1 = mk3(m[4], m[5], m[6]), c2 = mk3(m[8], m[9], m[10]);
  f3 k0 = cross3(c1, c2), k1 = cross3(c2, c0), k2 = cross3(c0, c1);
  float det = dot3(c0, k0);
  f3 r = mk3(__fmaf_rn(k2.x, n.z, __fmaf_rn(k1.x, n.y, k0.x * n.x)), __fmaf_rn(k2.y, n.z, __fmaf_rn(k1.y, n.y, k0.y * n.x)),
             __fmaf_rn(k2.z, n.z, __fmaf_rn(k1.z, n.y, k0.z * n.x)));
  return det < 0.0f ? -r : r;
}

RT_DI float log2_approx(float x) {
  const uint32_t b = __float_as_uint(x);
  const float e = (float)((int)((b >> 23) & 255u) - 127);
  const float m = __uint_as_float((b & 0x007fffffu) | 0x3f800000u);
  return e + (m - 1.0f);
}
constexpr uint32_t kTexLutEntries = 512;
template <typename LUT>
RT_DI float4 tex8_fetch(LUT lut, const uint32_t* base, uint32_t format, int x, int y, int w) {
  const uint32_t t = base[tex_tiled_index((uint32_t)x, (uint32_t)y, (uint32_t)w)];
  const uint32_t o = format == kTexSrgb8 ? 0u : 256u;
  return make_float4(lut[o + (t & 0xffu)], lut[o + ((t >> 8) & 0xffu)], lut[o + ((t >> 16) & 0xffu)], lut[256u + (t >> 24)]);
}
template <typename LUT>
RT_DI float4 tex_bilinear(const SceneView& sv, LUT lut, const TexDesc& td, uint32_t level, float u, float v) {
  const int w = max((int)(td.width >> level), 1), h = max((int)(td.height >> level), 1);
  const float x = u * (float)w - 0.5f, y = v * (float)h - 0.5f;
  const float x0 = floorf(x), y0 = floorf(y);
  const float fx = x - x0, fy = y - y0;
  const int ix0 = wrapi((int)x0, w), iy0 = wrapi((int)y0, h);
  const int ix1 = wrap_next(ix0, w), iy1 = wrap_next(iy0, h);
  float4 c00, c10, c01, c11;
  if (td.format == kTexFloat) {
    const float4* base = sv.tex_arena + td.mip_offset[level];
    c00 = base[(size_t)iy0 * w + ix0]; c10 = base[(size_t)iy0 * w + ix1];
    c01 = base[(size_t)iy1 * w + ix0]; c11 = base[(size_t)iy1 * w + ix1];
  } else {
    const uint32_t* base = sv.tex_arena8 + td.mip_offset[level];
    c00 = tex8_fetch(lut, base, td.format, ix0, iy0, w); c10 = tex8_fetch(lut, base, td.format, ix1, iy0, w);
    c01 = tex8_fetch(lut, base, td.format, ix0, iy1, w); c11 = tex8_fetch(lut, base, td.format, ix1, iy1, w);
  }
  const float gx = 1.0f - fx, gy = 1.0f - fy;
  float4 r;
  r.x = (c00.x * gx + c10.x * fx) * gy + (c01.x * gx + c11.x * fx) * fy;
  r.y = (c00.y * gx + c10.y * fx) * gy + (c01.y * gx + c11.y * fx) * fy;
  r.z = (c00.z * gx + c10.z * fx) * gy + (c01.z * gx + c11.z * fx) * fy;
  r.w = (c00.w * gx + c10.w * fx) * gy + (c01.w * gx + c11.w * fx) * fy;
  return r;
}
template <typename LUT>
RT_DI float4 tex_sample(const SceneView& sv, LUT lut, uint32_t tex, float u, float v, float lod) {
  const TexDesc& td = sv.textures[tex];
  const float top = (float)(td.mips - 1u);
  lod = lod < 0.0f ? 0.0f : (lod > top ? top : lod);
  const float l0 = floorf(lod);
  const float fl = lod - l0;
  const uint32_t level = (uint32_t)l0;
  float4 a = tex_bilinear(sv, lut, td, level, u, v);
  if (fl > 0.0f && level + 1u < td.mips) {
    const float4 b = tex_bilinear(sv, lut, td, level + 1u, u, v);
    const float g = 1.0f - fl;
    a.x = a.x * g + b.x * fl; a.y = a.y * g + b.y * fl; a.z = a.z * g + b.z * fl; a.w = a.w * g + b.w * fl;
  }
  return a;
}
RT_DI float tex_lod(const SceneView& sv, uint32_t tex, float lod_base) {
  const TexDesc& td = sv.textures[tex];
  return lod_base + 0.5f * log2_approx((float)td.width * (float)td.height);
}

RT_DI uint32_t instance_of(const SceneView& sv, uint32_t gid) {
  uint32_t lo = 0, hi = sv.instance_count;
  while (hi - lo > 1u) {
    const uint32_t mid = (lo + hi) >> 1;
    if (sv.inst_info[mid].first_tri <= gid) lo = mid; else hi = mid;
  }
  return lo;
}
RT_DI uint32_t hit_record_of(const SceneView& sv, uint32_t gid, uint32_t shade_base_flagged, uint32_t local) {
  if (shade_base_flagged >> 31) return (shade_base_flagged & 0x7fffffffu) + local;
  const InstInfo ii = sv.inst_info[instance_of(sv, gid)];
  return ii.shade_base + (gid - ii.first_tri);
}
RT_DI float hit_alpha(const SceneView& sv, uint32_t prim, float u, float v) {
  const float4* sp = reinterpret_cast<const float4*>(sv.shade_tris + prim);
  const uint32_t material = __float_as_uint(sp[1].w);
  const hala_gpu_material& m = sv.materials[material];
  float alpha = m.opacity;
  const uint32_t tex = m.base_color_map_index;
  if (tex < sv.texture_count) {
    const float4 s4 = sp[4], s5 = sp[5];
    const float w0 = 1.0f - u - v;
    const float tu = __fmaf_rn(s5.x, v, __fmaf_rn(s4.z, u, s4.x * w0));
    const float tv = __fmaf_rn(s5.y, v, __fmaf_rn(s4.w, u, s4.y * w0));
    alpha = alpha * tex_bilinear(sv, sv.tex_lut, sv.textures[tex], 0u, tu, tv).w;
  }
  return alpha;
}
RT_DI bool any_hit_event(const SceneView& sv, uint32_t key, uint32_t prim, uint32_t rec, uint32_t flag, float t, float det, float u, float v, uint32_t q[3]) {
  q[0] = q[1] = q[2] = 0u;
  if (flag & 1u) {
    const float x = (float)(pcg_hash(key + prim * 0x9E3779B1u) >> 8) * (1.0f / 16777216.0f);
    if (x < hit_alpha(sv, rec, u, v)) return true;
  }
  if (flag & 2u) {
    const uint32_t material = __float_as_uint(reinterpret_cast<const float4*>(sv.shade_tris + rec)[1].w);
    const hala_gpu_material& m = sv.materials[material];
#pragma unroll
    for (int c = 0; c < 3; ++c) {
      const float sigma = m.medium_type == 1u ? m.medium_density * (1.0f - m.medium_color[c]) : m.medium_density;
      const uint32_t v32 = (uint32_t)(int32_t)floorf(minf(t * sigma, 4096.0f) * 65536.0f + 0.5f);
      q[c] = det < 0.0f ? v32 : 0u - v32;
    }
  }
  return false;
}
RT_DI f3 any_transmittance(const uint32_t tau[3]) {
  float r[3];
#pragma unroll
  for (int c = 0; c < 3; ++c) {
    const int32_t qv = (int32_t)tau[c];
    r[c] = qv > 0 ? exp_neg_poly(-((float)qv * (1.0f / 65536.0f))) : 1.0f;
  }
  return mk3(r[0], r[1], r[2]);
}

struct Surface {
  f3 P, ns, ng;
  MatView mat;
  f3 absorb, glow;
  float sigma, hg;
  f3 scol;
  uint32_t inst, material;
};
RT_DI f3 transform_vector(const float* m, f3 p) {
  return mk3(__fmaf_rn(m[8], p.z, __fmaf_rn(m[4], p.y, m[0] * p.x)), __fmaf_rn(m[9], p.z, __fmaf_rn(m[5], p.y, m[1] * p.x)),
             __fmaf_rn(m[10], p.z, __fmaf_rn(m[6], p.y, m[2] * p.x)));
}
template <bool SIMPLE, typename LUT>
RT_DI Surface make_surface(const SceneView& sv, LUT lut, float pixel_spread, f3 o, f3 d, float t, float u, float v, uint32_t prim) {
  Surface sf;
  uint32_t rec = prim, inst_tl = 0;
  bool instanced = false;
  if (sv.two_level) {
    inst_tl = instance_of(sv, prim);
    const InstInfo ii = sv.inst_info[inst_tl];
    rec = ii.shade_base + (prim - ii.first_tri);
    instanced = ii.instanced != 0u;
  }
  const float4* sp = reinterpret_cast<const float4*>(sv.shade_tris + rec);
  const float4 s0 = sp[0], s1 = sp[1], s2 = sp[2], s3 = sp[3];
  const uint32_t inst = sv.two_level ? inst_tl : __float_as_uint(s0.w), material = __float_as_uint(s1.w);
  const hala_gpu_mesh_data& md = sv.primitives[inst];
  sf.inst = inst; sf.material = material;
  float w0 = 1.0f - u - v;
  f3 nl = madd3(mk3(s3.x, s3.y, s3.z), v, madd3(mk3(s2.x, s2.y, s2.z), u, mk3(s1.x, s1.y, s1.z) * w0));
  sf.ns = normalize3(transform_normal(md.transform, nl));
  f3 gcross = mk3(s0.x, s0.y, s0.z);
  if (instanced) gcross = transform_normal(md.transform, gcross);
  sf.ng = normalize3(gcross);
  sf.P = madd3(d, t, o);
  const hala_gpu_material& m = sv.materials[material];
  sf.mat.base = ld3(m.base_color);
  sf.mat.emission = ld3(m.emission);
  sf.mat.ax = m.ax; sf.mat.ay = m.ay; sf.mat.type = SIMPLE ? 0u : m.type;
  sf.mat.metallic = m.metallic; sf.mat.roughness = m.roughness; sf.mat.specular_tint = m.specular_tint;
  sf.mat.sheen = m.sheen; sf.mat.sheen_tint = m.sheen_tint; sf.mat.clearcoat = m.clearcoat;
  sf.mat.clearcoat_roughness = m.clearcoat_roughness; sf.mat.ior = m.ior;
  sf.mat.trans = 0.0f; sf.mat.eta = m.ior; sf.mat.opacity = SIMPLE ? 1.0f : m.opacity;
  const uint32_t nt = sv.texture_count;
  const bool has_base = !SIMPLE && m.base_color_map_index < nt, has_nrm = !SIMPLE && m.normal_map_index < nt;
  const bool has_mr = !SIMPLE && m.metallic_roughness_map_index < nt, has_em = !SIMPLE && m.emission_map_index < nt;
  if (has_base || has_nrm || has_mr || has_em) {
    const float4 s4 = sp[4], s5 = sp[5], s6 = sp[6], s7 = sp[7];
    struct VA { float tex_coord[2]; };
    const VA a = {{s4.x, s4.y}}, b = {{s4.z, s4.w}}, c = {{s5.x, s5.y}};
    const float tu = __fmaf_rn(c.tex_coord[0], v, __fmaf_rn(b.tex_coord[0], u, a.tex_coord[0] * w0));
    const float tv = __fmaf_rn(c.tex_coord[1], v, __fmaf_rn(b.tex_coord[1], u, a.tex_coord[1] * w0));
    const float du1 = b.tex_coord[0] - a.tex_coord[0], dv1 = b.tex_coord[1] - a.tex_coord[1];
    const float du2 = c.tex_coord[0] - a.tex_coord[0], dv2 = c.tex_coord[1] - a.tex_coord[1];
    const float uv_area = fabsf(du1 * dv2 - dv1 * du2);
    const float world_area = sqrtf(dot3(gcross, gcross));
    const float cosi = maxf(fabsf(dot3(d, sf.ng)), 0.1f);
    const float foot = t * pixel_spread / cosi;
    const float ratio = foot * foot * uv_area / world_area;
    const float lod_base = (ratio > 0.0f && ratio < 3.0e38f) ? 0.5f * log2_approx(ratio) : 0.0f;
    if (has_base) {
      const float4 s = tex_sample(sv, lut, m.base_color_map_index, tu, tv, tex_lod(sv, m.base_color_map_index, lod_base));
      sf.mat.base = sf.mat.base * mk3(s.x, s.y, s.z);
      sf.mat.opacity = sf.mat.opacity * s.w;
    }
    if (has_em) {
      const float4 s = tex_sample(sv, lut, m.emission_map_index, tu, tv, tex_lod(sv, m.emission_map_index, lod_base));
      sf.mat.emission = sf.mat.emission * mk3(s.x, s.y, s.z);
    }
    if (has_mr) {
      const float4 s = tex_sample(sv, lut, m.metallic_roughness_map_index, tu, tv, tex_lod(sv, m.metallic_roughness_map_index, lod_base));
      sf.mat.metallic = sf.mat.metallic * s.z;
      if (m.type == 1u) {
        const float rl = sqrtf(m.roughness) * s.y;
        const float r2 = rl * rl;
        const float aspect = sqrtf(1.0f - clampf(m.anisotropic, 0.0f, 1.0f) * 0.9f);
        sf.mat.roughness = r2;
        sf.mat.ax = maxf(0.001f, r2 / aspect);
        sf.mat.ay = maxf(0.001f, r2 * aspect);
      }
    }
    if (has_nrm) {
      const float4 s = tex_sample(sv, lut, m.normal_map_index, tu, tv, tex_lod(sv, m.normal_map_index, lod_base));
      const f3 tl = madd3(mk3(s7.x, s7.y, s7.z), v, madd3(mk3(s6.y, s6.z, s6.w), u, mk3(s5.z, s5.w, s6.x) * w0));
      f3 tw = transform_vector(md.transform, tl);
      tw = tw - sf.ns * dot3(sf.ns, tw);
      const float tl2 = dot3(tw, tw);
      if (tl2 > 0.0f) {
        tw = tw * (1.0f / sqrtf(tl2));
        const f3 bw = cross3(sf.ns, tw);
        const f3 nts = mk3(s.x * 2.0f - 1.0f, s.y * 2.0f - 1.0f, s.z * 2.0f - 1.0f);
        const f3 nn = to_world(nts, tw, bw, sf.ns);
        const float nn2 = dot3(nn, nn);
        if (nn2 > 0.0f) sf.ns = nn * (1.0f / sqrtf(nn2));
      }
    }
  }
  if (!SIMPLE && m.type == 1u) sf.mat.trans = m.specular_transmission * (1.0f - sf.mat.metallic);
  if (dot3(sf.ns, sf.ng) < 0.0f) sf.ng = -sf.ng;
  sf.absorb = splat3(1.0f); sf.glow = splat3(0.0f);
  sf.sigma = 0.0f; sf.hg = 0.0f; sf.scol = splat3(1.0f);
  if (dot3(sf.ng, d) > 0.0f) {
    sf.ns = -sf.ns; sf.ng = -sf.ng;
    sf.mat.eta = 1.0f / sf.mat.ior;
    const float dt = m.medium_density * t;
    if (SIMPLE) {
    } else if (m.medium_type == 1u)
      sf.absorb = mk3(exp_neg_poly(-(dt * (1.0f - m.medium_color[0]))), exp_neg_poly(-(dt * (1.0f - m.medium_color[1]))),
                      exp_neg_poly(-(dt * (1.0f - m.medium_color[2]))));
    else if (m.medium_type == 3u)
      sf.glow = mk3(m.medium_color[0] * dt, m.medium_color[1] * dt, m.medium_color[2] * dt);
    else if (m.medium_type == 2u) {
      sf.sigma = m.medium_density; sf.hg = m.medium_anisotropy; sf.scol = mk3(m.medium_color[0], m.medium_color[1], m.medium_color[2]);
    }
  }
  return sf;
}

RT_DI float fold_mean(float mean_old, float x, uint32_t frame_index) {
  if (frame_index == 0u) return x;
  return (mean_old * (float)frame_index + x) / (float)(frame_index + 1u);
}

RT_DI f3 clamp01(f3 c) { return mk3(clampf(c.x, 0.0f, 1.0f), clampf(c.y, 0.0f, 1.0f), clampf(c.z, 0.0f, 1.0f)); }
RT_DI f3 mat3_mul(f3 c0, f3 c1, f3 c2, f3 v) {
  return mk3(c0.x * v.x + c1.x * v.y + c2.x * v.z, c0.y * v.x + c1.y * v.y + c2.y * v.z, c0.z * v.x + c1.z * v.y + c2.z * v.z);
}
RT_DI f3 tonemap_select(f3 color, uint32_t enable_tonemap, uint32_t enable_aces, uint32_t use_simple_aces) {
  if (!enable_tonemap) return color;
  if (enable_aces) {
    if (use_simple_aces) {
      const float A = 2.51f, B = 0.03f, Y = 2.43f, D = 0.59f, E = 0.14f;
      f3 num = color * (color * A + splat3(B));
      f3 den = color * (color * Y + splat3(D)) + splat3(E);
      return clamp01(mk3(num.x / den.x, num.y / den.y, num.z / den.z));
    }
    f3 c = mat3_mul(mk3(0.59719f, 0.07600f, 0.02840f), mk3(0.35458f, 0.90834f, 0.13383f), mk3(0.04823f, 0.01566f, 0.83777f), color);
    f3 a = c * (c + splat3(0.0245786f)) - splat3(0.000090537f);
    f3 b = c * (c * 0.983729f + splat3(0.432951f)) + splat3(0.238081f);
    c = mk3(a.x / b.x, a.y / b.y, a.z / b.z);
    c = mat3_mul(mk3(1.60475f, -0.10208f, -0.00327f), mk3(-0.53108f, 1.10813f, -0.07276f), mk3(-0.07367f, -0.00605f, 1.07602f), c);
    return clamp01(c);
  }
  float dd = 1.0f + luminance(color) / 1.5f;
  f3 n = color * 1.0f;
  return mk3(n.x / dd, n.y / dd, n.z / dd);
}

}
```

### hala-renderer_amd/csrc/texture.hip

```cpp
#include <hip/hip_runtime.h>

#include "kernels.h"
#include "rt_math.h"

namespace rt {

__global__ void __launch_bounds__(256) k_mip_downsample(const float4* __restrict__ src, uint32_t sw, uint32_t sh, float4* __restrict__ dst,
                                                         uint32_t dw, uint32_t dh) {
  const uint32_t i = blockIdx.x * blockDim.x + threadIdx.x;
  if (i >= dw * dh) return;
  const uint32_t y = i / dw, x = i - y * dw;
  const uint32_t x0 = min(2u * x, sw - 1u), x1 = min(2u * x + 1u, sw - 1u);
  const uint32_t y0 = min(2u * y, sh - 1u), y1 = min(2u * y + 1u, sh - 1u);
  const float4 a = src[(size_t)y0 * sw + x0], b = src[(size_t)y0 * sw + x1];
  const float4 c = src[(size_t)y1 * sw + x0], d = src[(size_t)y1 * sw + x1];
  float4 r;
  r.x = ((a.x + b.x) + (c.x + d.x)) * 0.25f;
  r.y = ((a.y + b.y) + (c.y + d.y)) * 0.25f;
  r.z = ((a.z + b.z) + (c.z + d.z)) * 0.25f;
  r.w = ((a.w + b.w) + (c.w + d.w)) * 0.25f;
  dst[i] = r;
}

__global__ void __launch_bounds__(256) k_tile8(const uint32_t* __restrict__ src, uint32_t w, uint32_t h, uint32_t* __restrict__ dst) {
  const uint32_t i = blockIdx.x * blockDim.x + threadIdx.x;
  if (i >= w * h) return;
  const uint32_t y = i / w, x = i - y * w;
  dst[tex_tiled_index(x, y, w)] = src[i];
}
RT_DI float4 tex8_decode(uint32_t t, uint32_t format, const float* __restrict__ lut) {
  const uint32_t r = t & 0xffu, g = (t >> 8) & 0xffu, b = (t >> 16) & 0xffu, a = t >> 24;
  if (format == kTexSrgb8) return make_float4(lut[r], lut[g], lut[b], (float)a / 255.0f);
  return make_float4((float)r / 255.0f, (float)g / 255.0f, (float)b / 255.0f, (float)a / 255.0f);
}
RT_DI uint32_t tex8_encode_unorm(float x) { const float v = floorf(x * 255.0f + 0.5f); return (uint32_t)(v < 0.0f ? 0.0f : (v > 255.0f ? 255.0f : v)); }
RT_DI uint32_t tex8_encode_srgb(float x, const float* __restrict__ thr) {
  uint32_t lo = 0, hi = 255;
  while (lo < hi) {
    const uint32_t mid = (lo + hi) >> 1;
    if (thr[mid] < x) lo = mid + 1u; else hi = mid;
  }
  return lo;
}
__global__ void __launch_bounds__(256) k_mip_downsample8(const uint32_t* __restrict__ src, uint32_t sw, uint32_t sh, uint32_t* __restrict__ dst, uint32_t dw,
                                                          uint32_t dh, uint32_t format, const float* __restrict__ lut, const float* __restrict__ thr) {
  const uint32_t i = blockIdx.x * blockDim.x + threadIdx.x;
  if (i >= dw * dh) return;
  const uint32_t y = i / dw, x = i - y * dw;
  const uint32_t x0 = min(2u * x, sw - 1u), x1 = min(2u * x + 1u, sw - 1u);
  const uint32_t y0 = min(2u * y, sh - 1u), y1 = min(2u * y + 1u, sh - 1u);
  const float4 a = tex8_decode(src[tex_tiled_index(x0, y0, sw)], format, lut), b = tex8_decode(src[tex_tiled_index(x1, y0, sw)], format, lut);
  const float4 c = tex8_decode(src[tex_tiled_index(x0, y1, sw)], format, lut), d = tex8_decode(src[tex_tiled_index(x1, y1, sw)], format, lut);
  const float r4[4] = {((a.x + b.x) + (c.x + d.x)) * 0.25f, ((a.y + b.y) + (c.y + d.y)) * 0.25f, ((a.z + b.z) + (c.z + d.z)) * 0.25f,
                       ((a.w + b.w) + (c.w + d.w)) * 0.25f};
  uint32_t out = tex8_encode_unorm(r4[3]) << 24;
#pragma unroll
  for (int k = 0; k < 3; ++k) out |= (format == kTexSrgb8 ? tex8_encode_srgb(r4[k], thr) : tex8_encode_unorm(r4[k])) << (8 * k);
  dst[tex_tiled_index(x, y, dw)] = out;
}
void launch_tile8(const uint32_t* src, uint32_t w, uint32_t h, uint32_t* dst, hipStream_t s) {
  hipLaunchKernelGGL(k_tile8, dim3((w * h + 255u) / 256u), dim3(256), 0, s, src, w, h, dst);
}
void launch_mip_downsample8(const uint32_t* src, uint32_t sw, uint32_t sh, uint32_t* dst, uint32_t dw, uint32_t dh, uint32_t format, const float* lut,
                            const float* thr, hipStream_t s) {
  hipLaunchKernelGGL(k_mip_downsample8, dim3((dw * dh + 255u) / 256u), dim3(256), 0, s, src, sw, sh, dst, dw, dh, format, lut, thr);
}

void launch_mip_downsample(const float4* src, uint32_t sw, uint32_t sh, float4* dst, uint32_t dw, uint32_t dh, hipStream_t s) {
  const uint32_t n = dw * dh;
  hipLaunchKernelGGL(k_mip_downsample, dim3((n + 255u) / 256u), dim3(256), 0, s, src, sw, sh, dst, dw, dh);
}

}
```

### hala-renderer_amd/renderer.py

```python
import ctypes as C
import os

import numpy as np

from . import _abi as A


class HalaRenderer:

    RAYGEN, MISS, CALLABLE = 0, 1, 2

    def __init__(self, name, width, height, max_depth, rr_depth, enable_tonemap, enable_aces, use_simple_aces,
                 max_frames, device_ordinal=0):
        from . import check, load_library
        self._lib = load_library()
        self._check = check
        self._h = C.c_void_p()
        check(self._lib.hala_rt_create(name.encode(), C.c_uint32(width), C.c_uint32(height), C.c_int(device_ordinal),
                                       C.c_uint32(max_depth), C.c_uint32(rr_depth), C.c_int(bool(enable_tonemap)),
                                       C.c_int(bool(enable_aces)), C.c_int(bool(use_simple_aces)),
                                       C.c_uint64(max_frames), C.byref(self._h)))
        self.width, self.height = width, height

    def close(self):
        if getattr(self, "_h", None) is not None and self._h:
            self._lib.hala_rt_destroy(self._h)
            self._h = None

    def __del__(self):
        try:
            self.close()
        except Exception:
            pass

    def __enter__(self):
        return self

    def __exit__(self, *exc):
        self.close()

    def push_general_shader(self, code: bytes, stage, group_type=None, debug_name=""):
        self._check(self._lib.hala_rt_push_general_shader(self._h, code, C.c_size_t(len(code)), C.c_int(stage), debug_name.encode()))

    def push_general_shader_with_file(self, file_path, stage, group_type=None, debug_name=""):
        self._check(self._lib.hala_rt_push_general_shader_with_file(self._h, os.fsencode(file_path), C.c_int(stage), debug_name.encode()))

    def push_hit_shaders(self, closest_code=None, any_hit_code=None, intersection_code=None, debug_name=""):
        def arg(b):
            return (b, C.c_size_t(len(b))) if b else (None, C.c_size_t(0))
        c, a, i = arg(closest_code), arg(any_hit_code), arg(intersection_code)
        self._check(self._lib.hala_rt_push_hit_shaders(self._h, c[0], c[1], a[0], a[1], i[0], i[1], debug_name.encode()))

    def push_hit_shaders_with_file(self, closest_hit_path=None, any_hit_path=None, intersection_path=None, debug_name=""):
        enc = lambda p: os.fsencode(p) if p else None
        self._check(self._lib.hala_rt_push_hit_shaders_with_file(self._h, enc(closest_hit_path), enc(any_hit_path), enc(intersection_path), debug_name.encode()))

    def load_blue_noise_texture(self, path_or_rgba8):
        if isinstance(path_or_rgba8, (str, bytes, os.PathLike)):
            self._check(self._lib.hala_rt_load_blue_noise_texture(self._h, os.fsencode(path_or_rgba8)))
            return
        px = np.ascontiguousarray(path_or_rgba8, dtype=np.uint8)
        self._check(self._lib.hala_rt_load_blue_noise_pixels(self._h, px.ctypes.data_as(C.POINTER(C.c_uint8)), C.c_uint32(px.shape[1]), C.c_uint32(px.shape[0])))

    def set_scene(self, scene_in_cpu):
        if hasattr(scene_in_cpu, "desc_ptr"):
            self._check(self._lib.hala_rt_set_scene(self._h, scene_in_cpu.desc_ptr()))
            return
        holder = scene_in_cpu.to_desc()
        self._check(self._lib.hala_rt_set_scene(self._h, holder.ptr()))
        self._scene = scene_in_cpu

    def set_envmap(self, path_or_pixels, rotation=0.0):
        if isinstance(path_or_pixels, (str, bytes, os.PathLike)):
            self._check(self._lib.hala_rt_set_envmap_file(self._h, os.fsencode(path_or_pixels), C.c_float(rotation)))
            return
        px = np.ascontiguousarray(path_or_pixels, dtype=np.float32)
        h, w, ch = px.shape
        self._check(self._lib.hala_rt_set_envmap_pixels(self._h, px.ctypes.data_as(C.POINTER(C.c_float)), C.c_uint32(ch), C.c_uint32(w), C.c_uint32(h), C.c_float(rotation)))

    def set_ground_color(self, color):
        self._lib.hala_rt_set_ground_color(self._h, (C.c_float * 4)(*color))

    def set_sky_color(self, color):
        self._lib.hala_rt_set_sky_color(self._h, (C.c_float * 4)(*color))

    def set_env_intensity(self, intensity):
        self._lib.hala_rt_set_env_intensity(self._h, C.c_float(intensity))

    def set_exposure_value(self, exposure_value):
        self._lib.hala_rt_set_exposure_value(self._h, C.c_float(exposure_value))

    def commit(self):
        self._check(self._lib.hala_rt_commit(self._h))

    BUILDERS = {None: 0, "auto": 0, "sah": 1, "ploc": 2, "lbvh": 3}

    def set_build_options(self, builder=None, ploc_tail=0, ploc_look_every=0, collapse_look_every=0, instancing=None):
        o = A.BuildOptions(builder=self.BUILDERS[builder], ploc_tail=ploc_tail, ploc_look_every=ploc_look_every, collapse_look_every=collapse_look_every,
                           instancing=0 if instancing is None else (2 if instancing else 1))
        self._check(self._lib.hala_rt_set_build_options(self._h, C.byref(o)))

    def update(self, delta_time=0.0, width=None, height=None, ui_fn=None):
        self._check(self._lib.hala_rt_update(self._h, C.c_double(delta_time), C.c_uint32(width or self.width), C.c_uint32(height or self.height)))

    def update_batch(self, frames: int):
        self._check(self._lib.hala_rt_update_batch(self._h, C.c_uint32(frames)))

    def render(self):
        self._check(self._lib.hala_rt_render(self._h))

    def wait_idle(self):
        self._check(self._lib.hala_rt_wait_idle(self._h))

    def save_images(self, path):
        self._check(self._lib.hala_rt_save_images(self._h, os.fsencode(path)))

    def info(self):
        i = A.RtInfo()
        self._check(self._lib.hala_rt_get_info(self._h, C.byref(i)))
        return i

    def statistics(self):
        s = A.RtStatistics()
        self._check(self._lib.hala_rt_get_statistics(self._h, C.byref(s)))
        return s

    def reset_accumulation(self):
        self._check(self._lib.hala_rt_reset_accumulation(self._h))

    def set_counting(self, enable: bool):
        self._check(self._lib.hala_rt_set_counting(self._h, C.c_int(bool(enable))))

    def set_pass_fusion(self, mode):
        self._check(self._lib.hala_rt_set_pass_fusion(self._h, C.c_uint32(mode)))

    def set_launch_timing_period(self, period):
        self._check(self._lib.hala_rt_set_launch_timing_period(self._h, C.c_uint32(period)))

    ACCUM, ALBEDO, NORMAL, FINAL, POSITION, IDS = 0, 1, 2, 3, 4, 5
    IMAGE_NAMES = ("accum", "albedo", "normal", "final", "position", "ids")

    def read_image(self, which=0, view=0) -> np.ndarray:
        if isinstance(which, str):
            which = self.IMAGE_NAMES.index(which)
        out = np.empty((self.height, self.width, 4), dtype=np.float32)
        dst = out.ctypes.data_as(C.POINTER(C.c_float))
        if view == 0:
            self._check(self._lib.hala_rt_read_image(self._h, C.c_int(which), dst))
        else:
            self._check(self._lib.hala_rt_read_view_image(self._h, C.c_uint32(view), C.c_int(which), dst))
        return out

    def set_views(self, cameras):
        idx = [int(c) for c in cameras]
        arr = (C.c_uint32 * max(len(idx), 1))(*idx)
        self._check(self._lib.hala_rt_set_views(self._h, arr, C.c_uint32(len(idx))))

    def set_aovs(self, position=False, ids=False):
        self._check(self._lib.hala_rt_set_aovs(self._h, C.c_uint32((1 if position else 0) | (2 if ids else 0))))

    def read_ids(self, view=0) -> np.ndarray:
        return self.read_image(self.IDS, view=view).view(np.uint32)

    def set_light_groups(self, lights=None, environment=0, materials=None, group_count=None):
        if lights is None and materials is None and group_count is None and environment == 0:
            self._check(self._lib.hala_rt_set_light_groups(self._h, None))
            self.light_group_count = 0
            return
        n_lights = len(self.packed_lights()[0])
        if isinstance(lights, dict):
            scene = getattr(self, "_scene", None)
            if scene is None or not hasattr(scene, "nodes"):
                raise ValueError("set_light_groups: a dict of light node names needs the HalaScene given to set_scene")
            from .scene import INVALID
            names = [nd.name for nd in scene.nodes if nd.light_index != INVALID]
            unknown = set(lights) - set(names)
            if unknown:
                raise ValueError(f"set_light_groups: no light node named {sorted(unknown)}")
            lg = [int(lights.get(nm, 0)) for nm in names[:n_lights]]
        else:
            lg = [int(x) for x in (lights if lights is not None else [0] * n_lights)]
        used = max(lg + [int(environment)]) + 1
# ... 102 lines not shown
        p = temporal_default_params(max_history=max_history, tol=tol, min_weight=min_weight)
        self._check(self._lib.hala_rt_set_temporal(self._h, C.byref(p)))

    def temporal_capture(self):
        self._check(self._lib.hala_rt_temporal_capture(self._h))

    def temporal_resolve(self, timed=False):
        ms = C.c_float(0.0)
        self._check(self._lib.hala_rt_temporal_resolve(self._h, C.byref(ms) if timed else None))
        return ms.value if timed else None

    def read_temporal(self, which=0) -> np.ndarray:
        if isinstance(which, str):
            which = ("temporal", "motion").index(which)
        out = np.empty((self.height, self.width, 4), dtype=np.float32)
        self._check(self._lib.hala_rt_read_temporal(self._h, C.c_int(which), out.ctypes.data_as(C.POINTER(C.c_float))))
        return out

    def temporal_buffer(self, which=0):
        p = C.c_void_p(); n = C.c_size_t()
        self._check(self._lib.hala_rt_get_temporal_buffer(self._h, C.c_int(which), C.byref(p), C.byref(n)))
        return p.value, n.value

    def denoise_temporal(self, iterations=None, sigma_color=None, sigma_albedo=None, normal_power=None, demodulate=True, timed=False):
        p = denoise_default_params(iterations=iterations, sigma_color=sigma_color, sigma_albedo=sigma_albedo,
                                   normal_power=normal_power, demodulate=demodulate)
        ms = C.c_float(0.0)
        self._check(self._lib.hala_rt_denoise_temporal(self._h, C.byref(p), C.byref(ms) if timed else None))
        return ms.value if timed else None

    def set_adaptive_sampling(self, threshold, min_samples=None, interval=None):
        if threshold is None:
            self._check(self._lib.hala_rt_set_adaptive_sampling(self._h, None))
            return
        p = adaptive_default_params(threshold=threshold, min_samples=min_samples, interval=interval)
        self._check(self._lib.hala_rt_set_adaptive_sampling(self._h, C.byref(p)))

    def read_sample_counts(self) -> np.ndarray:
        out = np.empty((self.height, self.width), dtype=np.uint32)
        self._check(self._lib.hala_rt_read_sample_counts(self._h, out.ctypes.data_as(C.POINTER(C.c_uint32))))
        return out

    def adaptive_status(self) -> A.AdaptiveStatus:
        s = A.AdaptiveStatus()
        self._check(self._lib.hala_rt_get_adaptive_status(self._h, C.byref(s)))
        return s

    def global_uniform(self) -> A.GlobalUniform:
        u = A.GlobalUniform()
        self._check(self._lib.hala_rt_get_global_uniform(self._h, C.byref(u)))
        return u

    def packed_cameras(self):
        buf = (A.GpuCamera * A.MAX_CAMERA_COUNT)(); n = C.c_uint32()
        self._check(self._lib.hala_rt_get_packed_cameras(self._h, buf, C.c_uint32(A.MAX_CAMERA_COUNT), C.byref(n)))
        return list(buf[:n.value])

    def packed_lights(self):
        buf = (A.GpuLight * A.MAX_LIGHT_COUNT)(); bb = (A.Aabb * A.MAX_LIGHT_COUNT)(); n = C.c_uint32()
        self._check(self._lib.hala_rt_get_packed_lights(self._h, buf, bb, C.c_uint32(A.MAX_LIGHT_COUNT), C.byref(n)))
        return list(buf[:n.value]), list(bb[:n.value])

    def packed_materials(self, capacity=4096):
        buf = (A.GpuMaterial * capacity)(); n = C.c_uint32()
        self._check(self._lib.hala_rt_get_packed_materials(self._h, buf, C.c_uint32(capacity), C.byref(n)))
        return list(buf[:min(n.value, capacity)])

    def packed_primitives(self, capacity=65536):
        buf = (A.GpuMeshData * capacity)(); t = np.zeros((capacity, 12), dtype=np.float32); n = C.c_uint32()
        self._check(self._lib.hala_rt_get_packed_primitives(self._h, buf, t.ctypes.data_as(C.POINTER(C.c_float)), C.c_uint32(capacity), C.byref(n)))
        k = min(n.value, capacity)
        return list(buf[:k]), t[:k]

    def env_distribution(self, width, height):
        total = C.c_float(); marg = np.empty(height, dtype=np.float32); cond = np.empty((height, width), dtype=np.float32)
        self._check(self._lib.hala_rt_get_env_distribution(self._h, C.byref(total), marg.ctypes.data_as(C.POINTER(C.c_float)), cond.ctypes.data_as(C.POINTER(C.c_float))))
        return total.value, marg, cond

    def texture_info(self, texture):
        w, h, m = C.c_uint32(), C.c_uint32(), C.c_uint32()
        self._check(self._lib.hala_rt_get_texture_info(self._h, C.c_uint32(texture), C.byref(w), C.byref(h), C.byref(m)))
        return w.value, h.value, m.value

    def read_texture_level(self, texture, level):
        w, h, _ = self.texture_info(texture)
        lw, lh = max(1, w >> level), max(1, h >> level)
        out = np.empty((lh, lw, 4), dtype=np.float32)
        self._check(self._lib.hala_rt_read_texture_level(self._h, C.c_uint32(texture), C.c_uint32(level), out.ctypes.data_as(C.POINTER(C.c_float))))
        return out

    def sample_texture(self, texture, uv_lod):
        q = np.ascontiguousarray(uv_lod, dtype=np.float32).reshape(-1, 3)
        out = np.empty((q.shape[0], 4), dtype=np.float32)
        self._check(self._lib.hala_rt_sample_texture_host(self._h, C.c_uint32(texture), q.ctypes.data_as(C.POINTER(C.c_float)), C.c_uint32(q.shape[0]),
                                                          out.ctypes.data_as(C.POINTER(C.c_float))))
        return out

    def trace_rays_host(self, rays: np.ndarray, mode=0, count_steps=False):
        rays = np.ascontiguousarray(rays, dtype=A.RAY_DTYPE)
        hits = np.empty(rays.shape[0], dtype=A.HIT_DTYPE)
        ctr = (C.c_uint64 * 2)(0, 0)
        self._check(self._lib.hala_rt_trace_rays_host(self._h, C.c_void_p(rays.ctypes.data), C.c_void_p(hits.ctypes.data), C.c_uint32(rays.shape[0]), C.c_int(mode), ctr if count_steps else None))
        return (hits, (ctr[0], ctr[1])) if count_steps else hits

    def trace_rays(self, d_rays: int, d_hits: int, count: int, mode=0, d_counters: int = 0, stream: int = 0):
        self._check(self._lib.hala_rt_trace_rays(self._h, C.c_void_p(d_rays), C.c_void_p(d_hits), C.c_uint32(count), C.c_int(mode), C.c_void_p(d_counters), C.c_void_p(stream)))

    def bvh_info(self) -> A.BvhInfo:
        i = A.BvhInfo()
        self._check(self._lib.hala_rt_get_bvh_info(self._h, C.byref(i)))
        return i

    def download_bvh(self):
        i = self.bvh_info()
        nodes = np.empty(i.node_count * 16, dtype=np.uint32)
        tris = np.empty(max(i.stored_triangle_count, 1) * 12, dtype=np.uint32)
        self._check(self._lib.hala_rt_download_bvh(self._h, C.c_void_p(nodes.ctypes.data), C.c_void_p(tris.ctypes.data)))
        return nodes, tris[: i.stored_triangle_count * 12]

    def download_instance_refs(self):
        n = C.c_uint32(0)
        self._check(self._lib.hala_rt_download_instance_refs(self._h, None, C.c_uint32(0), C.byref(n)))
        refs = np.empty((max(n.value, 1), 16), dtype=np.uint32)
        self._check(self._lib.hala_rt_download_instance_refs(self._h, C.c_void_p(refs.ctypes.data), C.c_uint32(n.value), C.byref(n)))
        return refs[: n.value]

    def update_node_transform(self, node_index, local_transform):
        m = np.asarray(local_transform, dtype=np.float32)
        self._check(self._lib.hala_rt_update_node_transform(self._h, C.c_uint32(node_index), (C.c_float * 16)(*m.T.reshape(-1).tolist())))

    def update_vertices(self, mesh_index, primitive_index, vertices):
        v = np.ascontiguousarray(vertices, dtype=A.VERTEX_DTYPE)
        self._check(self._lib.hala_rt_update_vertices(self._h, C.c_uint32(mesh_index), C.c_uint32(primitive_index), C.c_void_p(v.ctypes.data), C.c_uint32(v.shape[0])))

    def update_material(self, material_index, material):
        from .scene import fill_material_desc
        d = A.MaterialDesc()
        fill_material_desc(d, material)
        self._check(self._lib.hala_rt_update_material(self._h, C.c_uint32(material_index), C.byref(d)))

    def refit(self):
        self._check(self._lib.hala_rt_refit(self._h))

    def set_tile_shard(self, rank, world, tile_size=32):
        self._check(self._lib.hala_rt_set_tile_shard(self._h, C.c_uint32(rank), C.c_uint32(world), C.c_uint32(tile_size)))

    def stream_handle(self):
        p = C.c_void_p()
        self._check(self._lib.hala_rt_get_stream(self._h, C.byref(p)))
        return p.value or 0

    def tile_buffer(self, which=0):
        p = C.c_void_p(); n = C.c_size_t()
        self._check(self._lib.hala_rt_tile_buffer(self._h, C.c_int(which), C.byref(p), C.byref(n)))
        return p.value, n.value

    @staticmethod
    def comm_unique_id() -> bytes:
        from . import check, load_library
        buf = (C.c_uint8 * 128)()
        check(load_library().hala_rt_comm_unique_id(buf))
        return bytes(buf)

    def comm_init_rank(self, unique_id: bytes, rank: int, world: int):
        self._check(self._lib.hala_rt_comm_init_rank(self._h, (C.c_uint8 * 128)(*unique_id), C.c_uint32(rank), C.c_uint32(world)))

# ... 108 lines not shown
```

### include/halart.h

```cpp
#ifndef HALART_H
#define HALART_H

#include <stddef.h>
#include <stdint.h>

#ifdef __cplusplus
extern "C" {
#endif

#define HALA_OK 0
#define HALA_ERR 1

#define HALA_INVALID_INDEX 0xffffffffu
#define HALA_MAX_CAMERA_COUNT 8
#define HALA_MAX_LIGHT_COUNT 32


typedef struct hala_vertex {
  float position[3];
  float normal[3];
  float tangent[3];
  float tex_coord[2];
} hala_vertex;

// ... 152 lines not shown
  float znear;
  float zfar;
  float focal_distance;
  float aperture;
  float xmag;
  float ymag;
} hala_camera_desc;

#define HALA_FORMAT_R8G8B8A8_UNORM 0
#define HALA_FORMAT_R8G8B8A8_SRGB 1
#define HALA_FORMAT_R32G32B32A32_SFLOAT 2
#define HALA_FORMAT_B8G8R8A8_UNORM 3
typedef struct hala_image_desc {
  uint32_t format;
  uint32_t width;
  uint32_t height;
  const void* data;
  size_t num_of_bytes;
} hala_image_desc;

typedef struct hala_index_pair {
  uint32_t key;
  uint32_t value;
} hala_index_pair;

typedef struct hala_scene_desc {
  const hala_node_desc* nodes;         uint32_t node_count;
  const hala_mesh_desc* meshes;        uint32_t mesh_count;
  const hala_material_desc* materials; uint32_t material_count;
  const hala_light_desc* lights;       uint32_t light_count;
  const hala_camera_desc* cameras;     uint32_t camera_count;
  const hala_index_pair* texture2image_mapping; uint32_t texture_count;
  const hala_index_pair* image2data_mapping;    uint32_t image_count;
  const hala_image_desc* image_data;   uint32_t image_data_count;
} hala_scene_desc;

typedef struct hala_scene hala_scene;
int hala_scene_load_gltf(const char* path, hala_scene** out);
const hala_scene_desc* hala_scene_get_desc(const hala_scene* scene);
void hala_scene_free(hala_scene* scene);

const char* hala_last_error_message(void);

typedef struct hala_rt_renderer hala_rt_renderer;

int hala_rt_create(const char* name, uint32_t width, uint32_t height, int device_ordinal,
                   uint32_t max_depth, uint32_t rr_depth, int enable_tonemap, int enable_aces,
                   int use_simple_aces, uint64_t max_frames, hala_rt_renderer** out);
void hala_rt_destroy(hala_rt_renderer* r);

int hala_rt_push_general_shader(hala_rt_renderer* r, const void* code, size_t code_size, int stage,
                                const char* debug_name);
int hala_rt_push_general_shader_with_file(hala_rt_renderer* r, const char* file_path, int stage,
                                          const char* debug_name);
int hala_rt_push_hit_shaders(hala_rt_renderer* r, const void* closest_hit, size_t closest_hit_size,
                             const void* any_hit, size_t any_hit_size, const void* intersection,
                             size_t intersection_size, const char* debug_name);
int hala_rt_push_hit_shaders_with_file(hala_rt_renderer* r, const char* closest_hit_path,
                                       const char* any_hit_path, const char* intersection_path,
                                       const char* debug_name);

int hala_rt_load_blue_noise_texture(hala_rt_renderer* r, const char* path);
int hala_rt_load_blue_noise_pixels(hala_rt_renderer* r, const uint8_t* rgba8, uint32_t width,
                                   uint32_t height);

int hala_rt_set_scene(hala_rt_renderer* r, const hala_scene_desc* scene);

int hala_rt_set_envmap_pixels(hala_rt_renderer* r, const float* pixels, uint32_t channels,
                              uint32_t width, uint32_t height, float rotation_degrees);
int hala_rt_set_envmap_file(hala_rt_renderer* r, const char* path, float rotation_degrees);

void hala_rt_set_ground_color(hala_rt_renderer* r, const float rgba[4]);
void hala_rt_set_sky_color(hala_rt_renderer* r, const float rgba[4]);
void hala_rt_set_env_intensity(hala_rt_renderer* r, float intensity);
void hala_rt_set_exposure_value(hala_rt_renderer* r, float exposure_value);

int hala_rt_commit(hala_rt_renderer* r);
typedef struct hala_rt_build_options {
  uint32_t builder;
  uint32_t ploc_tail;
  uint32_t ploc_look_every;
  uint32_t collapse_look_every;
  uint32_t instancing;
  uint32_t reserved[3];
} hala_rt_build_options;
int hala_rt_set_build_options(hala_rt_renderer* r, const hala_rt_build_options* options);

int hala_rt_update(hala_rt_renderer* r, double delta_time, uint32_t width, uint32_t height);
int hala_rt_update_batch(hala_rt_renderer* r, uint32_t frames);
int hala_rt_render(hala_rt_renderer* r);
int hala_rt_wait_idle(hala_rt_renderer* r);

int hala_rt_save_images(hala_rt_renderer* r, const char* path);

int hala_rt_read_image(hala_rt_renderer* r, int which, float* dst_rgba32f);

int hala_rt_set_views(hala_rt_renderer* r, const uint32_t* camera_indices, uint32_t count);
int hala_rt_read_view_image(hala_rt_renderer* r, uint32_t view, int which, float* dst_rgba32f);

int hala_rt_set_aovs(hala_rt_renderer* r, uint32_t mask);

typedef struct hala_light_groups {
  uint32_t group_count;
  uint32_t environment_group;
  uint32_t light_count;
  uint32_t material_count;
  const uint32_t* light_group;
  const uint32_t* material_group;
} hala_light_groups;
int hala_rt_set_light_groups(hala_rt_renderer* r, const hala_light_groups* g);
int hala_rt_read_light_group(hala_rt_renderer* r, uint32_t view, uint32_t group, float* dst_rgba32f);
int hala_rt_relight(hala_rt_renderer* r, uint32_t view, const float* rgb_scales, uint32_t group_count);
int hala_rt_read_relit(hala_rt_renderer* r, int which, float* dst_rgba32f);
int hala_rt_get_relit_buffer(hala_rt_renderer* r, int which, void** d_ptr, size_t* bytes);

typedef struct hala_cryptomatte_desc {
  uint32_t layer_mask;
  uint32_t material_name_count;
  const char* const* material_names;
  uint32_t reserved[2];
} hala_cryptomatte_desc;
int hala_rt_set_cryptomatte(hala_rt_renderer* r, const hala_cryptomatte_desc* d);
int hala_rt_read_cryptomatte(hala_rt_renderer* r, uint32_t view, uint32_t layer, float* dst);
int hala_rt_read_cryptomatte_records(hala_rt_renderer* r, uint32_t view, uint32_t layer, uint32_t* dst);
int hala_rt_get_cryptomatte_manifest(hala_rt_renderer* r, uint32_t layer, char* dst, size_t capacity, size_t* length);
int hala_rt_save_cryptomatte(hala_rt_renderer* r, uint32_t view, const char* path);

typedef struct hala_rt_info {
  uint32_t width;
  uint32_t height;
} hala_rt_info;
typedef struct hala_rt_statistics {
  uint64_t total_frames;
  double last_gpu_ms;
  uint64_t rays_last_update;
  uint64_t rays_total;
  double traverse_ms_last_update;
  double gpu_ms_total;
  double traverse_closest_ms_total;
  double traverse_shadow_ms_total;
  uint64_t traverse_closest_launches;
  uint64_t traverse_shadow_launches;
  uint64_t updates_rendered;
  uint64_t rays_closest_total;
  uint64_t rays_shadow_total;
  uint64_t nodes_closest_total, tris_closest_total, nodes_shadow_total, tris_shadow_total;
  uint64_t rays_closest_counted, rays_shadow_counted;
  uint64_t wave_steps_closest_total, leaf_passes_closest_total, leaf_lanes_closest_total;
  uint64_t wave_steps_shadow_total, leaf_passes_shadow_total, leaf_lanes_shadow_total;
  double traverse_primary_ms_total;
  uint64_t traverse_primary_launches;
  uint64_t nodes_primary_total, tris_primary_total, rays_primary_counted;
  uint64_t rays_primary_total;
  uint64_t rays_closest_timed, rays_primary_timed, rays_shadow_timed;
  double shade_ms_total;
  uint64_t shade_launches;
  double traverse_fused_ms_total;
  uint64_t traverse_fused_launches;
  uint64_t rays_fused_closest_timed, rays_fused_shadow_timed;
} hala_rt_statistics;
int hala_rt_get_info(hala_rt_renderer* r, hala_rt_info* out);
int hala_rt_get_statistics(hala_rt_renderer* r, hala_rt_statistics* out);
int hala_rt_reset_accumulation(hala_rt_renderer* r);
int hala_rt_set_counting(hala_rt_renderer* r, int enable);
int hala_rt_set_launch_timing_period(hala_rt_renderer* r, uint32_t period);
int hala_rt_set_pass_fusion(hala_rt_renderer* r, uint32_t mode);
int hala_rt_get_global_uniform(hala_rt_renderer* r, hala_global_uniform* out);

int hala_rt_get_packed_cameras(hala_rt_renderer* r, hala_gpu_camera* dst, uint32_t capacity, uint32_t* count);
int hala_rt_get_packed_lights(hala_rt_renderer* r, hala_gpu_light* dst, hala_aabb* dst_aabbs, uint32_t capacity, uint32_t* count);
int hala_rt_get_packed_materials(hala_rt_renderer* r, hala_gpu_material* dst, uint32_t capacity, uint32_t* count);
int hala_rt_get_packed_primitives(hala_rt_renderer* r, hala_gpu_mesh_data* dst, float* dst_instance_3x4, uint32_t capacity, uint32_t* count);
int hala_rt_get_env_distribution(hala_rt_renderer* r, float* total_sum, float* marginal, float* conditional);

int hala_rt_get_texture_info(hala_rt_renderer* r, uint32_t texture, uint32_t* width, uint32_t* height, uint32_t* mips);
int hala_rt_read_texture_level(hala_rt_renderer* r, uint32_t texture, uint32_t level, float* dst_rgba32f);
int hala_rt_sample_texture_host(hala_rt_renderer* r, uint32_t texture, const float* uv_lod, uint32_t count, float* dst_rgba32f);

int hala_rt_set_tile_shard(hala_rt_renderer* r, uint32_t rank, uint32_t world, uint32_t tile_size);
int hala_rt_tile_buffer(hala_rt_renderer* r, int which, void** d_ptr, size_t* bytes);
int hala_rt_get_stream(hala_rt_renderer* r, void** hip_stream);
int hala_rt_scatter_gathered_tiles(hala_rt_renderer* r, int which, const void* d_gathered, size_t bytes);

#define HALA_COMM_UNIQUE_ID_BYTES 128
int hala_rt_comm_unique_id(void* out_128_bytes);
int hala_rt_comm_init_rank(hala_rt_renderer* r, const void* unique_id_128_bytes, uint32_t rank, uint32_t world);
int hala_rt_comm_attach(hala_rt_renderer* r, void* nccl_comm);
int hala_rt_comm_destroy(hala_rt_renderer* r);
int hala_rt_tile_allgather(hala_rt_renderer* r, uint32_t aov_mask);
int hala_rt_tile_allgather_begin(hala_rt_renderer* r, uint32_t aov_mask);
int hala_rt_tile_allgather_finish(hala_rt_renderer* r);
int hala_rt_get_gathered_buffer(hala_rt_renderer* r, int which, void** d_ptr, size_t* bytes);
int hala_rt_tile_allgather_begin_external(hala_rt_renderer* r, uint32_t aov_mask);
int hala_rt_get_exchange_buffers(hala_rt_renderer* r, int which, void** d_staged, size_t* staged_bytes, void** d_receive, size_t* receive_bytes,
                                 void** hip_stream);
int hala_rt_scatter_gathered_tiles_on_stream(hala_rt_renderer* r, int which, const void* d_gathered, size_t bytes, void* hip_stream);

typedef struct hala_ray {
  float origin[3];
  float tmin;
  float direction[3];
  float tmax;
} hala_ray;

typedef struct hala_hit {
  float t;
  float u;
  float v;
  uint32_t prim;
} hala_hit;

int hala_rt_trace_rays(hala_rt_renderer* r, const hala_ray* d_rays, hala_hit* d_hits, uint32_t count,
                       int mode, uint64_t* d_counters, void* hip_stream);
int hala_rt_trace_rays_indirect(hala_rt_renderer* r, const hala_ray* d_rays, hala_hit* d_hits,
                                const uint32_t* d_indirect, int mode, void* hip_stream);
int hala_rt_trace_rays_host(hala_rt_renderer* r, const hala_ray* rays, hala_hit* hits, uint32_t count,
                            int mode, uint64_t counters[2]);

typedef struct hala_bvh_info {
  uint32_t node_count;
  uint32_t triangle_count;
  uint32_t max_depth;
  uint32_t lds_node_count;
  float scene_min[3];
  float scene_max[3];
  uint32_t node_width;
  uint32_t stored_triangle_count;
  uint32_t instance_node_count;
  uint32_t instance_ref_count;
  uint64_t tree_bytes;
} hala_bvh_info;
int hala_rt_get_bvh_info(hala_rt_renderer* r, hala_bvh_info* out);
int hala_rt_download_bvh(hala_rt_renderer* r, void* nodes_64B, void* triangles_48B);
int hala_rt_download_instance_refs(hala_rt_renderer* r, void* refs_64B, uint32_t capacity, uint32_t* count);
int hala_rt_update_node_transform(hala_rt_renderer* r, uint32_t node_index, const float local_transform[16]);
int hala_rt_update_vertices(hala_rt_renderer* r, uint32_t mesh_index, uint32_t primitive_index, const hala_vertex* vertices,
                            uint32_t vertex_count);
int hala_rt_update_material(hala_rt_renderer* r, uint32_t material_index, const hala_material_desc* material);
int hala_rt_refit(hala_rt_renderer* r);

typedef struct hala_denoise_params {
  uint32_t iterations;
  float sigma_color;
  float sigma_albedo;
  uint32_t normal_power;
  uint32_t demodulate;
  uint32_t reserved[3];
} hala_denoise_params;
void hala_denoise_default_params(hala_denoise_params* out);
int hala_rt_denoise(hala_rt_renderer* r, const hala_denoise_params* p, float* gpu_ms);
int hala_rt_read_denoised(hala_rt_renderer* r, float* dst_rgba32f);
int hala_rt_get_denoised_buffer(hala_rt_renderer* r, void** d_ptr, size_t* bytes);
int hala_rt_save_denoised(hala_rt_renderer* r, const char* path);
int hala_denoise_images(int device_ordinal, const float* color, const float* albedo, const float* normal, uint32_t width,
                        uint32_t height, const hala_denoise_params* p, float* dst);

typedef struct hala_adaptive_status {
  uint32_t enabled, active_blocks, total_blocks, active_pixels;
  uint32_t samples;
// ... 68 lines not shown
```

### rust/hala-renderer-halart/src/lib.rs

```rust
#![allow(non_camel_case_types)]

use std::ffi::{CStr, CString};
use std::os::raw::{c_char, c_int, c_void};
use std::path::Path;

pub mod sys {
  use super::*;

  #[repr(C)] pub struct hala_rt_renderer { _private: [u8; 0] }

  #[repr(C)] #[derive(Clone, Copy)]
  pub struct hala_vertex { pub position: [f32; 3], pub normal: [f32; 3], pub tangent: [f32; 3], pub tex_coord: [f32; 2] }

  #[repr(C)] pub struct hala_node_desc {
    pub name: *const c_char, pub parent: i32, pub local_transform: [f32; 16],
    pub mesh_index: u32, pub camera_index: u32, pub light_index: u32,
  }
  #[repr(C)] pub struct hala_primitive_desc {
    pub indices: *const u32, pub index_count: u32, pub vertices: *const hala_vertex, pub vertex_count: u32, pub material_index: u32,
  }
  #[repr(C)] pub struct hala_mesh_desc { pub primitives: *const hala_primitive_desc, pub primitive_count: u32 }
  #[repr(C)] pub struct hala_material_desc {
    pub type_: u32, pub base_color: [f32; 3], pub opacity: f32, pub emission: [f32; 3], pub anisotropic: f32, pub metallic: f32,
    pub roughness: f32, pub subsurface: f32, pub specular_tint: f32, pub sheen: f32, pub sheen_tint: f32, pub clearcoat: f32,
    pub clearcoat_roughness: f32, pub clearcoat_tint: [f32; 3], pub specular_transmission: f32, pub ior: f32,
    pub medium_type: u32, pub medium_color: [f32; 3], pub medium_density: f32, pub medium_anisotropy: f32,
    pub base_color_map_index: u32, pub emission_map_index: u32, pub normal_map_index: u32, pub metallic_roughness_map_index: u32,
  }
  #[repr(C)] pub struct hala_light_desc { pub color: [f32; 3], pub intensity: f32, pub light_type: u32, pub param0: f32, pub param1: f32 }
  #[repr(C)] pub struct hala_camera_desc {
    pub type_: u32, pub aspect: f32, pub yfov: f32, pub znear: f32, pub zfar: f32, pub focal_distance: f32, pub aperture: f32, pub xmag: f32, pub ymag: f32,
  }
  #[repr(C)] pub struct hala_light_groups {
    pub group_count: u32, pub environment_group: u32, pub light_count: u32, pub material_count: u32,
    pub light_group: *const u32, pub material_group: *const u32,
  }
  #[repr(C)] pub struct hala_cryptomatte_desc {
    pub layer_mask: u32, pub material_name_count: u32, pub material_names: *const *const c_char, pub reserved: [u32; 2],
  }
  #[repr(C)] pub struct hala_image_desc { pub format: u32, pub width: u32, pub height: u32, pub data: *const c_void, pub num_of_bytes: usize }
  #[repr(C)] pub struct hala_index_pair { pub key: u32, pub value: u32 }
  #[repr(C)] pub struct hala_scene_desc {
    pub nodes: *const hala_node_desc, pub node_count: u32,
    pub meshes: *const hala_mesh_desc, pub mesh_count: u32,
    pub materials: *const hala_material_desc, pub material_count: u32,
    pub lights: *const hala_light_desc, pub light_count: u32,
    pub cameras: *const hala_camera_desc, pub camera_count: u32,
    pub texture2image_mapping: *const hala_index_pair, pub texture_count: u32,
    pub image2data_mapping: *const hala_index_pair, pub image_count: u32,
    pub image_data: *const hala_image_desc, pub image_data_count: u32,
  }
  #[repr(C)] #[derive(Clone, Copy)] pub struct hala_ray { pub origin: [f32; 3], pub tmin: f32, pub direction: [f32; 3], pub tmax: f32 }
  #[repr(C)] #[derive(Clone, Copy)] pub struct hala_hit { pub t: f32, pub u: f32, pub v: f32, pub prim: u32 }
  #[repr(C)] #[derive(Default)] pub struct hala_rt_info { pub width: u32, pub height: u32 }

  #[repr(C)] #[derive(Default, Clone, Copy)]
  pub struct hala_rt_build_options { pub builder: u32, pub ploc_tail: u32, pub ploc_look_every: u32, pub collapse_look_every: u32, pub instancing: u32, pub reserved: [u32; 3] }
  #[repr(C)] pub struct hala_scene { _private: [u8; 0] }
  #[repr(C)] pub struct hala_rtprog { _private: [u8; 0] }
  extern "C" {
    pub fn hala_last_error_message() -> *const c_char;
    pub fn hala_rt_create(name: *const c_char, width: u32, height: u32, device_ordinal: c_int, max_depth: u32, rr_depth: u32,
                          enable_tonemap: c_int, enable_aces: c_int, use_simple_aces: c_int, max_frames: u64, out: *mut *mut hala_rt_renderer) -> c_int;
    pub fn hala_rt_destroy(r: *mut hala_rt_renderer);
    pub fn hala_rt_push_general_shader(r: *mut hala_rt_renderer, code: *const c_void, code_size: usize, stage: c_int, debug_name: *const c_char) -> c_int;
    pub fn hala_rt_push_general_shader_with_file(r: *mut hala_rt_renderer, file_path: *const c_char, stage: c_int, debug_name: *const c_char) -> c_int;
    pub fn hala_rt_push_hit_shaders_with_file(r: *mut hala_rt_renderer, closest: *const c_char, any: *const c_char, isect: *const c_char, debug_name: *const c_char) -> c_int;
    pub fn hala_rt_load_blue_noise_pixels(r: *mut hala_rt_renderer, rgba8: *const u8, width: u32, height: u32) -> c_int;
    pub fn hala_rt_set_scene(r: *mut hala_rt_renderer, scene: *const hala_scene_desc) -> c_int;
    pub fn hala_rt_set_envmap_file(r: *mut hala_rt_renderer, path: *const c_char, rotation_degrees: f32) -> c_int;
    pub fn hala_rt_set_envmap_pixels(r: *mut hala_rt_renderer, pixels: *const f32, channels: u32, width: u32, height: u32, rotation_degrees: f32) -> c_int;
    pub fn hala_rt_set_ground_color(r: *mut hala_rt_renderer, rgba: *const f32);
    pub fn hala_rt_set_sky_color(r: *mut hala_rt_renderer, rgba: *const f32);
    pub fn hala_rt_set_env_intensity(r: *mut hala_rt_renderer, intensity: f32);
    pub fn hala_rt_set_exposure_value(r: *mut hala_rt_renderer, exposure_value: f32);
    pub fn hala_rt_commit(r: *mut hala_rt_renderer) -> c_int;
    pub fn hala_rt_update(r: *mut hala_rt_renderer, delta_time: f64, width: u32, height: u32) -> c_int;
    pub fn hala_rt_update_batch(r: *mut hala_rt_renderer, frames: u32) -> c_int;
    pub fn hala_rt_render(r: *mut hala_rt_renderer) -> c_int;
    pub fn hala_rt_wait_idle(r: *mut hala_rt_renderer) -> c_int;
    pub fn hala_rt_save_images(r: *mut hala_rt_renderer, path: *const c_char) -> c_int;
    pub fn hala_rt_get_info(r: *mut hala_rt_renderer, out: *mut hala_rt_info) -> c_int;
    pub fn hala_rt_trace_rays(r: *mut hala_rt_renderer, d_rays: *const hala_ray, d_hits: *mut hala_hit, count: u32, mode: c_int,
                              d_counters: *mut u64, hip_stream: *mut c_void) -> c_int;
    pub fn hala_rt_trace_rays_indirect(r: *mut hala_rt_renderer, d_rays: *const hala_ray, d_hits: *mut hala_hit, d_indirect: *const u32,
                                       mode: c_int, hip_stream: *mut c_void) -> c_int;
    pub fn hala_rt_update_node_transform(r: *mut hala_rt_renderer, node_index: u32, local_transform: *const f32) -> c_int;
    pub fn hala_rt_update_material(r: *mut hala_rt_renderer, material_index: u32, material: *const hala_material_desc) -> c_int;
    pub fn hala_rt_update_vertices(r: *mut hala_rt_renderer, mesh_index: u32, primitive_index: u32, vertices: *const hala_vertex, vertex_count: u32) -> c_int;
    pub fn hala_rt_refit(r: *mut hala_rt_renderer) -> c_int;
    pub fn hala_rt_load_blue_noise_texture(r: *mut hala_rt_renderer, path: *const c_char) -> c_int;
    pub fn hala_rt_set_tile_shard(r: *mut hala_rt_renderer, rank: u32, world: u32, tile_size: u32) -> c_int;
    pub fn hala_rt_comm_unique_id(out_128_bytes: *mut u8) -> c_int;
    pub fn hala_rt_comm_init_rank(r: *mut hala_rt_renderer, unique_id_128_bytes: *const u8, rank: u32, world: u32) -> c_int;
    pub fn hala_rt_comm_attach(r: *mut hala_rt_renderer, nccl_comm: *mut c_void) -> c_int;
    pub fn hala_rt_comm_destroy(r: *mut hala_rt_renderer) -> c_int;
    pub fn hala_rt_tile_allgather(r: *mut hala_rt_renderer, aov_mask: u32) -> c_int;
    pub fn hala_rt_tile_allgather_begin(r: *mut hala_rt_renderer, aov_mask: u32) -> c_int;
    pub fn hala_rt_tile_allgather_finish(r: *mut hala_rt_renderer) -> c_int;
    pub fn hala_rtprog_create(r: *mut hala_rt_renderer, desc_json: *const c_char, debug_name: *const c_char, out: *mut *mut hala_rtprog) -> c_int;
    pub fn hala_rtprog_destroy(p: *mut hala_rtprog);
    pub fn hala_rtprog_bind(p: *mut hala_rtprog, d_rays: *const hala_ray, d_hits: *mut hala_hit) -> c_int;
    pub fn hala_rtprog_push_constants(p: *mut hala_rtprog, offset: u32, data: *const c_void, len: usize) -> c_int;
    pub fn hala_rtprog_push_constants_f32(p: *mut hala_rtprog, offset: u32, data: *const f32, count: usize) -> c_int;
    pub fn hala_rtprog_trace_rays(p: *mut hala_rtprog, width: u32, height: u32, depth: u32, hip_stream: *mut c_void) -> c_int;
    pub fn hala_rtprog_trace_rays_indirect(p: *mut hala_rtprog, d_indirect: *const u32, hip_stream: *mut c_void) -> c_int;
    pub fn hala_rt_tile_buffer(r: *mut hala_rt_renderer, which: c_int, d_ptr: *mut *mut c_void, bytes: *mut usize) -> c_int;
    pub fn hala_rt_scatter_gathered_tiles(r: *mut hala_rt_renderer, which: c_int, d_gathered: *const c_void, bytes: usize) -> c_int;
    pub fn hala_rt_scatter_gathered_tiles_on_stream(r: *mut hala_rt_renderer, which: c_int, d_gathered: *const c_void, bytes: usize, hip_stream: *mut c_void) -> c_int;
    pub fn hala_rt_get_stream(r: *mut hala_rt_renderer, hip_stream: *mut *mut c_void) -> c_int;
    pub fn hala_rt_set_launch_timing_period(r: *mut hala_rt_renderer, period: u32) -> c_int;
    pub fn hala_rt_set_pass_fusion(r: *mut hala_rt_renderer, mode: u32) -> c_int;
    pub fn hala_rt_set_build_options(r: *mut hala_rt_renderer, options: *const hala_rt_build_options) -> c_int;
    pub fn hala_rt_tile_allgather_begin_external(r: *mut hala_rt_renderer, aov_mask: u32) -> c_int;
    pub fn hala_rt_get_exchange_buffers(r: *mut hala_rt_renderer, which: c_int, d_staged: *mut *mut c_void, staged_bytes: *mut usize,
                                        d_receive: *mut *mut c_void, receive_bytes: *mut usize, hip_stream: *mut *mut c_void) -> c_int;
    pub fn hala_rt_set_aovs(r: *mut hala_rt_renderer, mask: u32) -> c_int;
    pub fn hala_rt_set_light_groups(r: *mut hala_rt_renderer, g: *const hala_light_groups) -> c_int;
    pub fn hala_rt_read_light_group(r: *mut hala_rt_renderer, view: u32, group: u32, dst_rgba32f: *mut f32) -> c_int;
    pub fn hala_rt_relight(r: *mut hala_rt_renderer, view: u32, rgb_scales: *const f32, group_count: u32) -> c_int;
    pub fn hala_rt_read_relit(r: *mut hala_rt_renderer, which: c_int, dst_rgba32f: *mut f32) -> c_int;
    pub fn hala_rt_get_relit_buffer(r: *mut hala_rt_renderer, which: c_int, d_ptr: *mut *mut c_void, bytes: *mut usize) -> c_int;
    pub fn hala_rt_set_cryptomatte(r: *mut hala_rt_renderer, d: *const hala_cryptomatte_desc) -> c_int;
    pub fn hala_rt_read_cryptomatte(r: *mut hala_rt_renderer, view: u32, layer: u32, dst: *mut f32) -> c_int;
    pub fn hala_rt_read_cryptomatte_records(r: *mut hala_rt_renderer, view: u32, layer: u32, dst: *mut u32) -> c_int;
    pub fn hala_rt_get_cryptomatte_manifest(r: *mut hala_rt_renderer, layer: u32, dst: *mut c_char, capacity: usize, length: *mut usize) -> c_int;
    pub fn hala_rt_save_cryptomatte(r: *mut hala_rt_renderer, view: u32, path: *const c_char) -> c_int;
    pub fn hala_cryptomatte_hash(name: *const c_char, raw: *mut u32, id: *mut u32) -> c_int;
    pub fn hala_write_exr(path: *const c_char, width: u32, height: u32, channel_count: u32, channel_names: *const *const c_char,
                          planes: *const *const f32, attribute_count: u32, attr_names: *const *const c_char, attr_values: *const *const c_char) -> c_int;
    pub fn hala_scene_load_gltf(path: *const c_char, out: *mut *mut hala_scene) -> c_int;
    pub fn hala_scene_get_desc(scene: *const hala_scene) -> *const hala_scene_desc;
    pub fn hala_scene_free(scene: *mut hala_scene);
    pub fn hala_load_float_image(path: *const c_char, width: *mut u32, height: *mut u32, channels: *mut u32, dst: *mut f32, capacity_floats: usize) -> c_int;
  }
}

#[derive(thiserror::Error, Debug)]
#[error("{msg}")]
pub struct HalaRendererError { msg: String }
// ... 156 lines not shown
```

Measured before the change: 5304.

## Interleave same-size material texture maps into bundled uint4 texels for shading

Materials whose base color, normal, metallic-roughness and emission maps share dimensions and 8-bit formats get their maps interleaved into one 2x2-tiled uint4 arena, so a single bilinear fetch covers all maps. LOD selection and the address math are shared across the maps. The aim is fewer scattered memory transactions and less texture addressing work in shading. It costs extra device memory for duplicated texture data and a build-time interleave pass, and a 16-byte fetch is wasted on lanes whose maps are absent.

Result: faster. 5509 (median of 6 runs) (+3.9%).

```diff
diff --git a/hala-renderer_amd/_abi.py b/hala-renderer_amd/_abi.py
--- a/hala-renderer_amd/_abi.py
+++ b/hala-renderer_amd/_abi.py
@@ -157,7 +157,12 @@
 
 class BuildOptions(C.Structure):
     _fields_ = [("builder", C.c_uint32), ("ploc_tail", C.c_uint32), ("ploc_look_every", C.c_uint32),
-                ("collapse_look_every", C.c_uint32), ("instancing", C.c_uint32), ("reserved", C.c_uint32 * 3)]
+                ("collapse_look_every", C.c_uint32), ("instancing", C.c_uint32), ("texture_bundles", C.c_uint32), ("reserved", C.c_uint32 * 2)]
+
+
+class TextureBundleInfo(C.Structure):
+    _fields_ = [("bundle_count", C.c_uint32), ("bundled_materials", C.c_uint32), ("unbundled_textured_materials", C.c_uint32),
+                ("reserved", C.c_uint32), ("bundle_bytes", C.c_uint64)]
 
 
 class BvhInfo(C.Structure):
@@ -229,6 +234,7 @@
     "hala_cryptomatte_hash": ([C.c_char_p, C.POINTER(C.c_uint32), C.POINTER(C.c_uint32)], C.c_int),
     "hala_write_exr": ([C.c_char_p, C.c_uint32, C.c_uint32, C.c_uint32, C.POINTER(C.c_char_p), C.POINTER(C.POINTER(C.c_float)), C.c_uint32,
                         C.POINTER(C.c_char_p), C.POINTER(C.c_char_p)], C.c_int),
+    "hala_rt_texture_bundle_info": ([C.c_void_p, C.POINTER(TextureBundleInfo)], C.c_int),
     "hala_temporal_default_params": ([C.POINTER(TemporalParams)], None),
     "hala_rt_set_temporal": ([C.c_void_p, C.POINTER(TemporalParams)], C.c_int),
     "hala_rt_temporal_capture": ([C.c_void_p], C.c_int),
@@ -276,4 +282,5 @@
     "hala_rt_save_cryptomatte", "hala_cryptomatte_hash", "hala_write_exr",
     "hala_temporal_default_params", "hala_rt_set_temporal", "hala_rt_temporal_capture", "hala_rt_temporal_resolve", "hala_rt_read_temporal",
     "hala_rt_get_temporal_buffer", "hala_rt_denoise_temporal",
+    "hala_rt_texture_bundle_info",
 ]
diff --git a/hala-renderer_amd/csrc/hala_types.h b/hala-renderer_amd/csrc/hala_types.h
--- a/hala-renderer_amd/csrc/hala_types.h
+++ b/hala-renderer_amd/csrc/hala_types.h
@@ -93,6 +93,18 @@
 inline uint32_t tex_tiled_index(uint32_t x, uint32_t y, uint32_t w) { return (((y >> 2) * ((w + 3u) >> 2) + (x >> 2)) << 4) + ((y & 3u) << 2) + (x & 3u); }
 inline uint32_t tex_tiled_size(uint32_t w, uint32_t h) { return ((w + 3u) >> 2) * ((h + 3u) >> 2) * 16u; }
 static_assert(sizeof(TexDesc) == 80, "texture descriptor is 80 B");
+constexpr uint32_t kBundleLanes = 4;
+struct BundleDesc {
+  uint32_t width, height, mips;
+  uint32_t formats;
+  uint32_t mip_offset[kMaxMips];
+};
+static_assert(sizeof(BundleDesc) == 80, "bundle descriptor is 80 B");
+#if defined(__HIPCC__)
+__host__ __device__
+#endif
+inline uint32_t bundle_texel_index(uint32_t x, uint32_t y, uint32_t w) { return (((y >> 1) * ((w + 1u) >> 1) + (x >> 1)) << 2) + ((y & 1u) << 1) + (x & 1u); }
+inline uint32_t bundle_level_lines(uint32_t w, uint32_t h) { return ((w + 1u) >> 1) * ((h + 1u) >> 1); }
 
 struct SceneView {
   const TexDesc* textures;
@@ -100,6 +112,9 @@
   const uint32_t* tex_arena8;
   const float* tex_lut;
   uint32_t texture_count;
+  const BundleDesc* bundles;
+  const uint4* bundle_arena;
+  const uint32_t* material_bundle;
   uint32_t shade_sort;
   const BvhNode4* nodes;
   const Tri* tris;
diff --git a/hala-renderer_amd/csrc/kernels.h b/hala-renderer_amd/csrc/kernels.h
--- a/hala-renderer_amd/csrc/kernels.h
+++ b/hala-renderer_amd/csrc/kernels.h
@@ -44,6 +44,7 @@
 void launch_tile8(const uint32_t* src, uint32_t w, uint32_t h, uint32_t* dst, hipStream_t s);
 void launch_mip_downsample8(const uint32_t* src, uint32_t sw, uint32_t sh, uint32_t* dst, uint32_t dw, uint32_t dh, uint32_t format, const float* lut,
                             const float* thr, hipStream_t s);
+void launch_bundle_interleave(const uint32_t* src, uint32_t w, uint32_t h, uint4* dst, uint32_t lane, hipStream_t s);
 
 struct BuildOptions {
   uint32_t builder = 0;
diff --git a/hala-renderer_amd/csrc/renderer.hip b/hala-renderer_amd/csrc/renderer.hip
--- a/hala-renderer_amd/csrc/renderer.hip
+++ b/hala-renderer_amd/csrc/renderer.hip
@@ -32,6 +32,10 @@
 constexpr size_t kLdsStageBudget = 40 * 1024;
 constexpr uint32_t kRefillThreshold = 24;
 constexpr int kStatRing = 16;
+#ifndef RT_BUNDLE_MIN_MAPS
+#define RT_BUNDLE_MIN_MAPS 2
+#endif
+constexpr uint32_t kBundleMinMaps = RT_BUNDLE_MIN_MAPS;
 constexpr uint32_t kMaxSampleBatch = 16;
 
 float h_sin_poly(float a) {
@@ -131,6 +135,15 @@
   DeviceArray<float> d_srgb_lut, d_srgb_thr;
   DeviceArray<TexDesc> d_textures;
   std::vector<TexDesc> host_textures;
+  struct BundleSource { uint32_t image[kBundleLanes], texture[kBundleLanes]; };
+  uint32_t texture_bundles_mode = 0;
+  bool bundles_on = false;
+  std::vector<BundleSource> bundle_sources;
+  std::vector<BundleDesc> host_bundles;
+  DeviceArray<uint4> d_bundle_arena;
+  DeviceArray<BundleDesc> d_bundles;
+  DeviceArray<uint32_t> d_material_bundle;
+  uint32_t bundled_materials = 0, unbundled_textured_materials = 0;
 
   BvhBuffers bvh{};
   struct Blas {
@@ -293,7 +306,9 @@
     sv.nodes = d_nodes.ptr; sv.tris = d_tris.ptr; sv.tris_any = any_invisible ? d_tris_any.ptr : d_tris.ptr; sv.tris_by_id = d_tris_by_id.ptr; sv.shade_tris = d_shade_tris.ptr;
     sv.inst_first_tri = d_inst_first_tri.ptr; sv.primitives = d_instances.ptr; sv.materials = d_materials.ptr; sv.material_kind = d_material_kind.ptr;
     sv.lights = d_lights.ptr; sv.cameras = d_cameras.ptr;
-    sv.textures = d_textures.ptr; sv.tex_arena = d_tex_arena.ptr; sv.tex_arena8 = d_tex_arena8.ptr; sv.tex_lut = d_srgb_lut.ptr; sv.texture_count = (uint32_t)host_textures.size(); sv.shade_sort = shade_sort ? 1u : 0u; sv.simple_materials = simple_materials ? 1u : 0u; sv.scatter_media = scatter_media ? 1u : 0u; sv.any_translucent = any_translucent ? 1u : 0u;
+    sv.textures = d_textures.ptr; sv.tex_arena = d_tex_arena.ptr; sv.tex_arena8 = d_tex_arena8.ptr; sv.tex_lut = d_srgb_lut.ptr; sv.texture_count = (uint32_t)host_textures.size();
+    if (!host_bundles.empty()) { sv.bundles = d_bundles.ptr; sv.bundle_arena = d_bundle_arena.ptr; sv.material_bundle = d_material_bundle.ptr; }
+    sv.shade_sort = shade_sort ? 1u : 0u; sv.simple_materials = simple_materials ? 1u : 0u; sv.scatter_media = scatter_media ? 1u : 0u; sv.any_translucent = any_translucent ? 1u : 0u;
     sv.env_pixels = reinterpret_cast<const float*>(d_env.ptr); sv.env_marginal = d_marginal.ptr; sv.env_conditional = d_conditional.ptr;
     sv.node_count = bvh.node_count; sv.tri_count = bvh.tri_count; sv.lds_nodes = lds_nodes; sv.lds_tris = lds_tris;
     sv.inst_refs = d_inst_refs.ptr; sv.inst_info = d_inst_info.ptr; sv.instance_count = (uint32_t)hs.instances.size(); sv.two_level = two_level ? 1u : 0u;
@@ -652,6 +667,88 @@
   return HALA_OK;
 }
 
+int update_texture_bundles(hala_rt_renderer* r, bool fresh) {
+  const HostScene& hs = r->hs;
+  const uint32_t nt = (uint32_t)r->host_textures.size();
+  if (fresh) {
+    r->bundles_on = r->texture_bundles_mode == 0u;
+    r->bundle_sources.clear(); r->host_bundles.clear();
+  }
+  std::vector<hala_rt_renderer::BundleSource> sources = r->bundle_sources;
+  std::vector<uint32_t> table(hs.gpu_materials.size(), kAbsent);
+  uint32_t bundled = 0, textured = 0;
+  for (size_t m = 0; m < hs.gpu_materials.size(); ++m) {
+    const hala_gpu_material& gm = hs.gpu_materials[m];
+    const uint32_t idx[kBundleLanes] = {gm.base_color_map_index, gm.normal_map_index, gm.metallic_roughness_map_index, gm.emission_map_index};
+    hala_rt_renderer::BundleSource src;
+    uint32_t maps = 0, w = 0, h = 0;
+    bool same = true;
+    for (uint32_t k = 0; k < kBundleLanes; ++k) {
+      src.image[k] = src.texture[k] = kAbsent;
+      if (idx[k] >= nt) continue;
+      const TexDesc& td = r->host_textures[idx[k]];
+      if (maps == 0) { w = td.width; h = td.height; }
+      same = same && td.format != kTexFloat && td.width == w && td.height == h;
+      src.image[k] = hs.texture_image[idx[k]]; src.texture[k] = idx[k];
+      ++maps;
+    }
+    if (maps == 0) continue;
+    ++textured;
+    if (!r->bundles_on || maps < kBundleMinMaps || !same) continue;
+    size_t b = 0;
+    while (b < sources.size() && memcmp(sources[b].image, src.image, sizeof(src.image)) != 0) ++b;
+    if (b == sources.size()) sources.push_back(src);
+    table[m] = (uint32_t)b;
+    ++bundled;
+  }
+  if (sources.size() != r->host_bundles.size()) {
+    std::vector<BundleDesc> descs(sources.size());
+    size_t lines = 0;
+    for (size_t b = 0; b < sources.size(); ++b) {
+      BundleDesc& bd = descs[b];
+      memset(&bd, 0, sizeof(bd));
+      for (uint32_t k = 0; k < kBundleLanes; ++k) {
+        if (sources[b].texture[k] == kAbsent) continue;
+        const TexDesc& td = r->host_textures[sources[b].texture[k]];
+        bd.width = td.width; bd.height = td.height; bd.mips = td.mips;
+        bd.formats |= td.format << (8u * k);
+      }
+      for (uint32_t l = 0; l < bd.mips; ++l) {
+        if (lines > 0xffffffffull) break;
+        bd.mip_offset[l] = (uint32_t)lines;
+        lines += bundle_level_lines(std::max(1u, bd.width >> l), std::max(1u, bd.height >> l));
+      }
+    }
+    bool ok = lines <= 0xffffffffull;
+    if (ok && r->d_bundle_arena.resize(lines * 4) != hipSuccess) { (void)hipGetLastError(); ok = false; }
+    if (!ok) {
+      r->bundles_on = false;
+      r->bundle_sources.clear(); r->host_bundles.clear();
+      r->d_bundle_arena.release();
+      std::fill(table.begin(), table.end(), kAbsent);
+      bundled = 0;
+    } else {
+      RT_HIP(hipMemsetAsync(r->d_bundle_arena.ptr, 0, lines * 64, r->stream));
+      for (size_t b = 0; b < sources.size(); ++b)
+        for (uint32_t k = 0; k < kBundleLanes; ++k) {
+          if (sources[b].texture[k] == kAbsent) continue;
+          const TexDesc& td = r->host_textures[sources[b].texture[k]];
+          for (uint32_t l = 0; l < td.mips; ++l)
+            launch_bundle_interleave(r->d_tex_arena8.ptr + td.mip_offset[l], std::max(1u, td.width >> l), std::max(1u, td.height >> l),
+                                     r->d_bundle_arena.ptr + ((size_t)descs[b].mip_offset[l] << 2), k, r->stream);
+        }
+      RT_HIP(r->d_bundles.upload(descs.data(), descs.size(), r->stream));
+      r->bundle_sources = sources; r->host_bundles = descs;
+    }
+  }
+  if (r->host_bundles.empty()) r->d_bundle_arena.release();
+  RT_HIP(r->d_material_bundle.upload(table.data(), table.size(), r->stream));
+  RT_HIP(hipStreamSynchronize(r->stream));
+  RT_HIP(hipGetLastError());
+  r->bundled_materials = bundled; r->unbundled_textured_materials = textured - bundled;
+  return HALA_OK;
+}
+
 int configure_traversal(hala_rt_renderer* r) {
   const size_t nb = (size_t)r->bvh.node_count * 64, tb = (size_t)r->bvh.tri_count * 48;
   r->staged = !r->two_level && nb + tb <= kLdsStageBudget;
@@ -1122,6 +1219,8 @@
   if (!r->has_scene) RT_FAIL("The scene in GPU is none!");
   if (r->hs.cameras.empty()) RT_FAIL("The scene has no camera.");
   if (r->hs.instances.empty()) RT_FAIL("The scene has no mesh primitive.");
+  RT_HIP(hipStreamSynchronize(r->stream));
+  if (update_texture_bundles(r, true) != HALA_OK) return HALA_ERR;
   if (build_bvh(r) != HALA_OK) return HALA_ERR;
   r->committed = true;
   r->crypto_tables = false;
@@ -1133,9 +1232,10 @@
 int hala_rt_set_build_options(hala_rt_renderer* r, const hala_rt_build_options* o) {
   if (!r) RT_FAIL("The renderer handle is null!");
   if (!o) RT_FAIL("The build options are null!");
-  if (o->builder > 3u || o->ploc_tail > 2u || o->instancing > 2u) RT_FAIL("Invalid build options.");
+  if (o->builder > 3u || o->ploc_tail > 2u || o->instancing > 2u || o->texture_bundles > 1u) RT_FAIL("Invalid build options.");
   for (uint32_t v : o->reserved) if (v != 0u) RT_FAIL("Invalid build options (reserved fields must be 0).");
   r->instancing_mode = o->instancing;
+  r->texture_bundles_mode = o->texture_bundles;
   r->bvh.opt.builder = o->builder; r->bvh.opt.ploc_tail = o->ploc_tail;
   r->bvh.opt.ploc_look_every = o->ploc_look_every; r->bvh.opt.collapse_look_every = o->collapse_look_every;
   return HALA_OK;
@@ -2039,6 +2139,17 @@
   if (mips) *mips = td.mips;
   return HALA_OK;
 }
+int hala_rt_texture_bundle_info(hala_rt_renderer* r, hala_texture_bundle_info* info) {
+  if (!r) RT_FAIL("The renderer handle is null!");
+  if (!info) RT_FAIL("Invalid argument.");
+  if (!r->committed) RT_FAIL("The top level acceleration structure is none!");
+  info->bundle_count = (uint32_t)r->host_bundles.size();
+  info->bundled_materials = r->bundled_materials;
+  info->unbundled_textured_materials = r->unbundled_textured_materials;
+  info->reserved = 0;
+  info->bundle_bytes = r->host_bundles.empty() ? 0ull : (unsigned long long)r->d_bundle_arena.count * 16ull;
+  return HALA_OK;
+}
 int hala_rt_read_texture_level(hala_rt_renderer* r, uint32_t texture, uint32_t level, float* dst_rgba32f) {
   if (ensure_device(r) != HALA_OK) return HALA_ERR;
   if (!r->has_scene || texture >= r->host_textures.size() || !dst_rgba32f) RT_FAIL("The texture does not exist.");
@@ -2404,6 +2515,7 @@
   const std::string e = r->hs.pack();
   if (!e.empty()) RT_FAIL(e);
   if (upload_packed(r, false) != HALA_OK) return HALA_ERR;
+  if (update_texture_bundles(r, false) != HALA_OK) return HALA_ERR;
   r->bvh.primitives = r->d_instances.ptr; r->bvh.inst_first_tri = r->d_inst_first_tri.ptr;
   const bool had_invisible = r->any_invisible;
   const std::vector<uint8_t> classes_before = r->material_any_class;
diff --git a/hala-renderer_amd/csrc/shading.h b/hala-renderer_amd/csrc/shading.h
--- a/hala-renderer_amd/csrc/shading.h
+++ b/hala-renderer_amd/csrc/shading.h
@@ -465,10 +465,13 @@
 }
 constexpr uint32_t kTexLutEntries = 512;
 template <typename LUT>
-RT_DI float4 tex8_fetch(LUT lut, const uint32_t* base, uint32_t format, int x, int y, int w) {
-  const uint32_t t = base[tex_tiled_index((uint32_t)x, (uint32_t)y, (uint32_t)w)];
+RT_DI float4 tex8_texel(LUT lut, uint32_t t, uint32_t format) {
   const uint32_t o = format == kTexSrgb8 ? 0u : 256u;
   return make_float4(lut[o + (t & 0xffu)], lut[o + ((t >> 8) & 0xffu)], lut[o + ((t >> 16) & 0xffu)], lut[256u + (t >> 24)]);
+}
+template <typename LUT>
+RT_DI float4 tex8_fetch(LUT lut, const uint32_t* base, uint32_t format, int x, int y, int w) {
+  return tex8_texel(lut, base[tex_tiled_index((uint32_t)x, (uint32_t)y, (uint32_t)w)], format);
 }
 template <typename LUT>
 RT_DI float4 tex_bilinear(const SceneView& sv, LUT lut, const TexDesc& td, uint32_t level, float u, float v) {
@@ -516,6 +519,51 @@
   const TexDesc& td = sv.textures[tex];
   return lod_base + 0.5f * log2_approx((float)td.width * (float)td.height);
 }
+struct BundleTap { uint4 t00, t10, t01, t11; float fx, fy; };
+RT_DI BundleTap bundle_fetch(const SceneView& sv, const BundleDesc& bd, uint32_t level, float u, float v) {
+  const int w = max((int)(bd.width >> level), 1), h = max((int)(bd.height >> level), 1);
+  const float x = u * (float)w - 0.5f, y = v * (float)h - 0.5f;
+  const float x0 = floorf(x), y0 = floorf(y);
+  const int ix0 = wrapi((int)x0, w), iy0 = wrapi((int)y0, h);
+  const int ix1 = wrap_next(ix0, w), iy1 = wrap_next(iy0, h);
+  const uint4* base = sv.bundle_arena + ((size_t)bd.mip_offset[level] << 2);
+  BundleTap k;
+  k.t00 = base[bundle_texel_index((uint32_t)ix0, (uint32_t)iy0, (uint32_t)w)]; k.t10 = base[bundle_texel_index((uint32_t)ix1, (uint32_t)iy0, (uint32_t)w)];
+  k.t01 = base[bundle_texel_index((uint32_t)ix0, (uint32_t)iy1, (uint32_t)w)]; k.t11 = base[bundle_texel_index((uint32_t)ix1, (uint32_t)iy1, (uint32_t)w)];
+  k.fx = x - x0; k.fy = y - y0;
+  return k;
+}
+template <int LANE>
+RT_DI uint32_t bundle_word(const uint4& t) { return LANE == 0 ? t.x : (LANE == 1 ? t.y : (LANE == 2 ? t.z : t.w)); }
+template <int LANE, typename LUT>
+RT_DI float4 bundle_bilinear(LUT lut, const BundleTap& k, uint32_t format) {
+  const float4 c00 = tex8_texel(lut, bundle_word<LANE>(k.t00), format), c10 = tex8_texel(lut, bundle_word<LANE>(k.t10), format);
+  const float4 c01 = tex8_texel(lut, bundle_word<LANE>(k.t01), format), c11 = tex8_texel(lut, bundle_word<LANE>(k.t11), format);
+  const float fx = k.fx, fy = k.fy, gx = 1.0f - fx, gy = 1.0f - fy;
+  float4 r;
+  r.x = (c00.x * gx + c10.x * fx) * gy + (c01.x * gx + c11.x * fx) * fy;
+  r.y = (c00.y * gx + c10.y * fx) * gy + (c01.y * gx + c11.y * fx) * fy;
+  r.z = (c00.z * gx + c10.z * fx) * gy + (c01.z * gx + c11.z * fx) * fy;
+  r.w = (c00.w * gx + c10.w * fx) * gy + (c01.w * gx + c11.w * fx) * fy;
+  return r;
+}
+struct BundleLod { uint32_t level; bool two; float fl; };
+RT_DI BundleLod bundle_lod(const BundleDesc& bd, float lod_base) {
+  float lod = lod_base + 0.5f * log2_approx((float)bd.width * (float)bd.height);
+  const float top = (float)(bd.mips - 1u);
+  lod = lod < 0.0f ? 0.0f : (lod > top ? top : lod);
+  const float l0 = floorf(lod);
+  BundleLod bl;
+  bl.fl = lod - l0;
+  bl.level = (uint32_t)l0;
+  bl.two = bl.fl > 0.0f && bl.level + 1u < bd.mips;
+  return bl;
+}
+RT_DI float4 bundle_mix(float4 a, const float4 b, float fl) {
+  const float g = 1.0f - fl;
+  a.x = a.x * g + b.x * fl; a.y = a.y * g + b.y * fl; a.z = a.z * g + b.z * fl; a.w = a.w * g + b.w * fl;
+  return a;
+}
 
 RT_DI uint32_t instance_of(const SceneView& sv, uint32_t gid) {
   uint32_t lo = 0, hi = sv.instance_count;
@@ -612,13 +660,12 @@
   sf.mat.base = ld3(m.base_color);
   sf.mat.emission = ld3(m.emission);
   sf.mat.ax = m.ax; sf.mat.ay = m.ay; sf.mat.type = SIMPLE ? 0u : m.type;
-  sf.mat.metallic = m.metallic; sf.mat.roughness = m.roughness; sf.mat.specular_tint = m.specular_tint;
-  sf.mat.sheen = m.sheen; sf.mat.sheen_tint = m.sheen_tint; sf.mat.clearcoat = m.clearcoat;
-  sf.mat.clearcoat_roughness = m.clearcoat_roughness; sf.mat.ior = m.ior;
-  sf.mat.trans = 0.0f; sf.mat.eta = m.ior; sf.mat.opacity = SIMPLE ? 1.0f : m.opacity;
+  sf.mat.metallic = m.metallic; sf.mat.roughness = m.roughness;
+  sf.mat.trans = 0.0f; sf.mat.opacity = SIMPLE ? 1.0f : m.opacity;
   const uint32_t nt = sv.texture_count;
   const bool has_base = !SIMPLE && m.base_color_map_index < nt, has_nrm = !SIMPLE && m.normal_map_index < nt;
   const bool has_mr = !SIMPLE && m.metallic_roughness_map_index < nt, has_em = !SIMPLE && m.emission_map_index < nt;
+  const uint32_t bundle = !SIMPLE && sv.material_bundle ? sv.material_bundle[material] : kAbsent;
   if (has_base || has_nrm || has_mr || has_em) {
     const float4 s4 = sp[4], s5 = sp[5], s6 = sp[6], s7 = sp[7];
     struct VA { float tex_coord[2]; };
@@ -633,17 +680,12 @@
     const float foot = t * pixel_spread / cosi;
     const float ratio = foot * foot * uv_area / world_area;
     const float lod_base = (ratio > 0.0f && ratio < 3.0e38f) ? 0.5f * log2_approx(ratio) : 0.0f;
-    if (has_base) {
-      const float4 s = tex_sample(sv, lut, m.base_color_map_index, tu, tv, tex_lod(sv, m.base_color_map_index, lod_base));
+    const auto apply_base = [&](const float4 s) {
       sf.mat.base = sf.mat.base * mk3(s.x, s.y, s.z);
       sf.mat.opacity = sf.mat.opacity * s.w;
-    }
-    if (has_em) {
-      const float4 s = tex_sample(sv, lut, m.emission_map_index, tu, tv, tex_lod(sv, m.emission_map_index, lod_base));
-      sf.mat.emission = sf.mat.emission * mk3(s.x, s.y, s.z);
-    }
-    if (has_mr) {
-      const float4 s = tex_sample(sv, lut, m.metallic_roughness_map_index, tu, tv, tex_lod(sv, m.metallic_roughness_map_index, lod_base));
+    };
+    const auto apply_emission = [&](const float4 s) { sf.mat.emission = sf.mat.emission * mk3(s.x, s.y, s.z); };
+    const auto apply_mr = [&](const float4 s) {
       sf.mat.metallic = sf.mat.metallic * s.z;
       if (m.type == 1u) {
         const float rl = sqrtf(m.roughness) * s.y;
@@ -653,10 +695,9 @@
         sf.mat.ax = maxf(0.001f, r2 / aspect);
         sf.mat.ay = maxf(0.001f, r2 * aspect);
       }
-    }
-    if (has_nrm) {
-      const float4 s = tex_sample(sv, lut, m.normal_map_index, tu, tv, tex_lod(sv, m.normal_map_index, lod_base));
-      const f3 tl = madd3(mk3(s7.x, s7.y, s7.z), v, madd3(mk3(s6.y, s6.z, s6.w), u, mk3(s5.z, s5.w, s6.x) * w0));
+    };
+    const auto local_tangent = [&]() { return madd3(mk3(s7.x, s7.y, s7.z), v, madd3(mk3(s6.y, s6.z, s6.w), u, mk3(s5.z, s5.w, s6.x) * w0)); };
+    const auto apply_normal = [&](const float4 s, const f3 tl) {
       f3 tw = transform_vector(md.transform, tl);
       tw = tw - sf.ns * dot3(sf.ns, tw);
       const float tl2 = dot3(tw, tw);
@@ -668,8 +709,43 @@
         const float nn2 = dot3(nn, nn);
         if (nn2 > 0.0f) sf.ns = nn * (1.0f / sqrtf(nn2));
       }
+    };
+    if (bundle != kAbsent) {
+      const BundleDesc& bd = sv.bundles[bundle];
+      const BundleLod bl = bundle_lod(bd, lod_base);
+      const uint32_t formats = bd.formats;
+      const f3 tl = local_tangent();
+      const uint32_t f_base = formats & 0xffu, f_nrm = (formats >> 8) & 0xffu, f_mr = (formats >> 16) & 0xffu, f_em = formats >> 24;
+      float4 c_base = make_float4(0.0f, 0.0f, 0.0f, 0.0f), c_nrm = c_base, c_mr = c_base, c_em = c_base;
+      {
+        const BundleTap k = bundle_fetch(sv, bd, bl.level, tu, tv);
+        if (has_base) c_base = bundle_bilinear<0>(lut, k, f_base);
+        if (has_nrm) c_nrm = bundle_bilinear<1>(lut, k, f_nrm);
+        if (has_mr) c_mr = bundle_bilinear<2>(lut, k, f_mr);
+        if (has_em) c_em = bundle_bilinear<3>(lut, k, f_em);
+      }
+      if (bl.two) {
+        const BundleTap k = bundle_fetch(sv, bd, bl.level + 1u, tu, tv);
+        if (has_base) c_base = bundle_mix(c_base, bundle_bilinear<0>(lut, k, f_base), bl.fl);
+        if (has_nrm) c_nrm = bundle_mix(c_nrm, bundle_bilinear<1>(lut, k, f_nrm), bl.fl);
+        if (has_mr) c_mr = bundle_mix(c_mr, bundle_bilinear<2>(lut, k, f_mr), bl.fl);
+        if (has_em) c_em = bundle_mix(c_em, bundle_bilinear<3>(lut, k, f_em), bl.fl);
+      }
+      if (has_base) apply_base(c_base);
+      if (has_em) apply_emission(c_em);
+      if (has_mr) apply_mr(c_mr);
+      if (has_nrm) apply_normal(c_nrm, tl);
+    } else {
+      if (has_base) apply_base(tex_sample(sv, lut, m.base_color_map_index, tu, tv, tex_lod(sv, m.base_color_map_index, lod_base)));
+      if (has_em) apply_emission(tex_sample(sv, lut, m.emission_map_index, tu, tv, tex_lod(sv, m.emission_map_index, lod_base)));
+      if (has_mr) apply_mr(tex_sample(sv, lut, m.metallic_roughness_map_index, tu, tv, tex_lod(sv, m.metallic_roughness_map_index, lod_base)));
+      if (has_nrm) apply_normal(tex_sample(sv, lut, m.normal_map_index, tu, tv, tex_lod(sv, m.normal_map_index, lod_base)), local_tangent());
     }
   }
+  sf.mat.specular_tint = m.specular_tint;
+  sf.mat.sheen = m.sheen; sf.mat.sheen_tint = m.sheen_tint; sf.mat.clearcoat = m.clearcoat;
+  sf.mat.clearcoat_roughness = m.clearcoat_roughness; sf.mat.ior = m.ior;
+  sf.mat.eta = m.ior;
   if (!SIMPLE && m.type == 1u) sf.mat.trans = m.specular_transmission * (1.0f - sf.mat.metallic);
   if (dot3(sf.ns, sf.ng) < 0.0f) sf.ng = -sf.ng;
   sf.absorb = splat3(1.0f); sf.glow = splat3(0.0f);
diff --git a/hala-renderer_amd/csrc/texture.hip b/hala-renderer_amd/csrc/texture.hip
--- a/hala-renderer_amd/csrc/texture.hip
+++ b/hala-renderer_amd/csrc/texture.hip
@@ -58,6 +58,15 @@
   for (int k = 0; k < 3; ++k) out |= (format == kTexSrgb8 ? tex8_encode_srgb(r4[k], thr) : tex8_encode_unorm(r4[k])) << (8 * k);
   dst[tex_tiled_index(x, y, dw)] = out;
 }
+__global__ void __launch_bounds__(256) k_bundle_interleave(const uint32_t* __restrict__ src, uint32_t w, uint32_t h, uint32_t* __restrict__ dst, uint32_t lane) {
+  const uint32_t i = blockIdx.x * blockDim.x + threadIdx.x;
+  if (i >= w * h) return;
+  const uint32_t y = i / w, x = i - y * w;
+  dst[(size_t)bundle_texel_index(x, y, w) * kBundleLanes + lane] = src[tex_tiled_index(x, y, w)];
+}
+void launch_bundle_interleave(const uint32_t* src, uint32_t w, uint32_t h, uint4* dst, uint32_t lane, hipStream_t s) {
+  hipLaunchKernelGGL(k_bundle_interleave, dim3((w * h + 255u) / 256u), dim3(256), 0, s, src, w, h, reinterpret_cast<uint32_t*>(dst), lane);
+}
 void launch_tile8(const uint32_t* src, uint32_t w, uint32_t h, uint32_t* dst, hipStream_t s) {
   hipLaunchKernelGGL(k_tile8, dim3((w * h + 255u) / 256u), dim3(256), 0, s, src, w, h, dst);
 }
diff --git a/hala-renderer_amd/renderer.py b/hala-renderer_amd/renderer.py
--- a/hala-renderer_amd/renderer.py
+++ b/hala-renderer_amd/renderer.py
@@ -95,9 +95,10 @@
 
     BUILDERS = {None: 0, "auto": 0, "sah": 1, "ploc": 2, "lbvh": 3}
 
-    def set_build_options(self, builder=None, ploc_tail=0, ploc_look_every=0, collapse_look_every=0, instancing=None):
+    def set_build_options(self, builder=None, ploc_tail=0, ploc_look_every=0, collapse_look_every=0, instancing=None, texture_bundles=None):
         o = A.BuildOptions(builder=self.BUILDERS[builder], ploc_tail=ploc_tail, ploc_look_every=ploc_look_every, collapse_look_every=collapse_look_every,
-                           instancing=0 if instancing is None else (2 if instancing else 1))
+                           instancing=0 if instancing is None else (2 if instancing else 1),
+                           texture_bundles=0 if texture_bundles is None or texture_bundles else 1)
         self._check(self._lib.hala_rt_set_build_options(self._h, C.byref(o)))
 
     def update(self, delta_time=0.0, width=None, height=None, ui_fn=None):
@@ -366,6 +367,11 @@
         self._check(self._lib.hala_rt_get_texture_info(self._h, C.c_uint32(texture), C.byref(w), C.byref(h), C.byref(m)))
         return w.value, h.value, m.value
 
+    def texture_bundle_info(self):
+        i = A.TextureBundleInfo()
+        self._check(self._lib.hala_rt_texture_bundle_info(self._h, C.byref(i)))
+        return i
+
     def read_texture_level(self, texture, level):
         w, h, _ = self.texture_info(texture)
         lw, lh = max(1, w >> level), max(1, h >> level)
diff --git a/include/halart.h b/include/halart.h
--- a/include/halart.h
+++ b/include/halart.h
@@ -258,7 +258,8 @@
   uint32_t ploc_look_every;
   uint32_t collapse_look_every;
   uint32_t instancing;
-  uint32_t reserved[3];
+  uint32_t texture_bundles;
+  uint32_t reserved[2];
 } hala_rt_build_options;
 int hala_rt_set_build_options(hala_rt_renderer* r, const hala_rt_build_options* options);
 
@@ -351,6 +352,14 @@
 
 int hala_rt_get_texture_info(hala_rt_renderer* r, uint32_t texture, uint32_t* width, uint32_t* height, uint32_t* mips);
 int hala_rt_read_texture_level(hala_rt_renderer* r, uint32_t texture, uint32_t level, float* dst_rgba32f);
+typedef struct hala_texture_bundle_info {
+  uint32_t bundle_count;
+  uint32_t bundled_materials;
+  uint32_t unbundled_textured_materials;
+  uint32_t reserved;
+  unsigned long long bundle_bytes;
+} hala_texture_bundle_info;
+int hala_rt_texture_bundle_info(hala_rt_renderer* r, hala_texture_bundle_info* info);
 int hala_rt_sample_texture_host(hala_rt_renderer* r, uint32_t texture, const float* uv_lod, uint32_t count, float* dst_rgba32f);
 
 int hala_rt_set_tile_shard(hala_rt_renderer* r, uint32_t rank, uint32_t world, uint32_t tile_size);
diff --git a/rust/hala-renderer-halart/src/lib.rs b/rust/hala-renderer-halart/src/lib.rs
--- a/rust/hala-renderer-halart/src/lib.rs
+++ b/rust/hala-renderer-halart/src/lib.rs
@@ -55,7 +55,7 @@
   #[repr(C)] #[derive(Default)] pub struct hala_rt_info { pub width: u32, pub height: u32 }
 
   #[repr(C)] #[derive(Default, Clone, Copy)]
-  pub struct hala_rt_build_options { pub builder: u32, pub ploc_tail: u32, pub ploc_look_every: u32, pub collapse_look_every: u32, pub instancing: u32, pub reserved: [u32; 3] }
+  pub struct hala_rt_build_options { pub builder: u32, pub ploc_tail: u32, pub ploc_look_every: u32, pub collapse_look_every: u32, pub instancing: u32, pub texture_bundles: u32, pub reserved: [u32; 2] }
   #[repr(C)] pub struct hala_scene { _private: [u8; 0] }
   #[repr(C)] pub struct hala_rtprog { _private: [u8; 0] }
   extern "C" {
```
